# gam0022/hanamaru-renderer

Hardware: AMD Instinct MI355X
Metric: Mpaths/sec at 1920x1080x1024spp (rtcamp6 scene); achieved GB/s in BVH traversal (higher is better)
Workload: dtype f32

## Files before the change

### hanamaru-renderer_amd/csrc/device_scene.h

```cpp
#pragma once
#include <math.h>
#include <stdint.h>

#if defined(__HIPCC__)
#define HD __host__ __device__ __forceinline__
#else
#define HD inline
#endif

namespace hr {

struct alignas(16) f4 { float x, y, z, w; };

struct alignas(16) Node {
    float nearx, neary, farx, fary;
    float nearz, farz;
    uint32_t a;
    uint32_t b;
};
HD void node_set_box(Node &n, const float *mn, const float *mx, int octant) {
    n.nearx = (octant & 1) ? mx[0] : mn[0]; n.farx = (octant & 1) ? mn[0] : mx[0];
    n.neary = (octant & 2) ? mx[1] : mn[1]; n.fary = (octant & 2) ? mn[1] : mx[1];
    n.nearz = (octant & 4) ? mx[2] : mn[2]; n.farz = (octant & 4) ? mn[2] : mx[2];
}
static const uint32_t NODE_END = 0x7fffffffu;
static const uint32_t LEAF_FLAG = 0x80000000u;
static const uint32_t LEAF_FIRST_BITS = 24u, LEAF_MAX_COUNT = 15u;
static const uint32_t MAX_PRIMS_PER_TYPE = 1u << LEAF_FIRST_BITS;
HD bool node_word_is_leaf(uint32_t a) { return a >= LEAF_FLAG; }
HD uint32_t leaf_word(uint32_t type, uint32_t count, uint32_t first) { return LEAF_FLAG | (type << 28) | (count << LEAF_FIRST_BITS) | first; }
HD uint32_t leaf_type(uint32_t w) { return (w >> 28) & 3u; }
HD uint32_t leaf_count(uint32_t w) { return (w >> LEAF_FIRST_BITS) & LEAF_MAX_COUNT; }
HD uint32_t leaf_first(uint32_t w) { return w & (MAX_PRIMS_PER_TYPE - 1u); }

struct alignas(16) QNode {
    uint32_t xy_near;
    uint32_t xy_far;
    uint32_t z_nf;
    uint32_t link;
};
HD uint32_t qnode_offset(int octant, uint32_t records_per_copy, uint32_t index) { return ((uint32_t)octant * records_per_copy + index) * 16u; }
HD uint32_t qnode_link(int octant, uint32_t records_per_copy, uint32_t successor_index) {
    return successor_index == NODE_END ? NODE_END : qnode_offset(octant, records_per_copy, successor_index);
}
HD void qframe_from_box(const float *root_mn, const float *root_mx, float *qmin, float *qstep) {
    for (int a = 0; a < 3; a++) {
        double ext = (double)root_mx[a] - (double)root_mn[a];
        if (!(ext > 1e-6)) ext = 1e-6;
        double gmin = (double)root_mn[a] - 1e-6 * ext;
        float fmin_ = (float)gmin;
        fmin_ -= (fmin_ < 0 ? -fmin_ : fmin_) * 1e-6f + 1e-30f;
        qmin[a] = fmin_;
        qstep[a] = (float)(ext * (1.0 + 4e-6) / 65532.0) * (1.0f + 1e-6f);
    }
}
HD uint32_t q_low(float v, float qmin, float qstep) {
    double q = floor(((double)v - (double)qmin) / (double)qstep - 0.05);
    return (uint32_t)(q < 0.0 ? 0.0 : (q > 65535.0 ? 65535.0 : q));
}
HD uint32_t q_high(float v, float qmin, float qstep) {
    double q = ceil(((double)v - (double)qmin) / (double)qstep + 0.05);
    return (uint32_t)(q < 0.0 ? 0.0 : (q > 65535.0 ? 65535.0 : q));
}
HD QNode qnode_make(const float *mn, const float *mx, int octant, const float *qmin, const float *qstep, uint32_t link) {
    uint32_t nearq[3], farq[3];
    for (int a = 0; a < 3; a++) {
        uint32_t lo = q_low(mn[a], qmin[a], qstep[a]), hi = q_high(mx[a], qmin[a], qstep[a]);
        nearq[a] = ((octant >> a) & 1) ? hi : lo;
        farq[a] = ((octant >> a) & 1) ? lo : hi;
    }
    QNode q;
    q.xy_near = nearq[0] | (nearq[1] << 16);
    q.xy_far = farq[0] | (farq[1] << 16);
    q.z_nf = nearq[2] | (farq[2] << 16);
    q.link = link;
    return q;
}
HD QNode qnode_sentinel(int octant) {
    QNode q;
    uint32_t nearq[3], farq[3];
    for (int a = 0; a < 3; a++) { nearq[a] = ((octant >> a) & 1) ? 0u : 65535u; farq[a] = ((octant >> a) & 1) ? 65535u : 0u; }
    q.xy_near = nearq[0] | (nearq[1] << 16);
    q.xy_far = farq[0] | (farq[1] << 16);
    q.z_nf = nearq[2] | (farq[2] << 16);
    q.link = NODE_END;
    return q;
}


struct alignas(16) Tri {
    float v0[3]; float e1x;
    float e1y, e1z, e2x, e2y;
    float e2z; int32_t element; uint32_t face; float pad1;
};

struct alignas(16) TriT {
    float n[3]; float ax;
    float ay, az, bx, by;
    float bz; float v0[3];
};
struct alignas(16) TriS { float n[3]; int32_t element; };
struct alignas(16) TriX { double n[3], v0[3]; };
HD void tri_derive(const Tri &t, TriT &tt, TriS &ts) {
    const double e1[3] = {t.e1x, t.e1y, t.e1z}, e2[3] = {t.e2x, t.e2y, t.e2z};
    const double n[3] = {e1[1] * e2[2] - e1[2] * e2[1], e1[2] * e2[0] - e1[0] * e2[2], e1[0] * e2[1] - e1[1] * e2[0]};
    const double nn = n[0] * n[0] + n[1] * n[1] + n[2] * n[2];
    const double inn = nn > 0.0 ? 1.0 / nn : 0.0, il = nn > 0.0 ? 1.0 / sqrt(nn) : 0.0;
    const double a[3] = {(e2[1] * n[2] - e2[2] * n[1]) * inn, (e2[2] * n[0] - e2[0] * n[2]) * inn, (e2[0] * n[1] - e2[1] * n[0]) * inn};
    const double b[3] = {(n[1] * e1[2] - n[2] * e1[1]) * inn, (n[2] * e1[0] - n[0] * e1[2]) * inn, (n[0] * e1[1] - n[1] * e1[0]) * inn};
    for (int k = 0; k < 3; k++) { tt.n[k] = (float)(n[k] * il); tt.v0[k] = t.v0[k]; ts.n[k] = (float)(n[k] * il); }
    tt.ax = (float)a[0]; tt.ay = (float)a[1]; tt.az = (float)a[2];
    tt.bx = (float)b[0]; tt.by = (float)b[1]; tt.bz = (float)b[2];
    ts.element = t.element;
}

struct alignas(16) Material {
    int32_t surface; float param; int32_t albedo_img, emission_img;
    float albedo[3]; int32_t roughness_img;
    float emission[3]; float roughness;
    int32_t nee_albedo_zero; int32_t pad[3];
};

struct ImageRef { uint32_t offset, width, height, pad; };

struct Emitter { float c[3]; float r; int32_t element; int32_t pad[3]; };

struct CameraF {
    float eye[3], right[3], up[3], forward[3], phr[3], phu[3];
    float lens_radius, focus_distance;
    int32_t lens_shape;
};

struct CameraD {
    double eye[3], right[3], up[3], forward[3], phr[3], phu[3];
    double lens_radius, focus_distance;
};

struct Scene {
    const QNode *qnodes;
    float qmin[3], qstep[3];
    const Node *nodes;
    const TriT *tris; const TriS *tri_shade;
    const uint32_t *tri_face;
    const f4 *spheres; const int32_t *sphere_elem;
    const f4 *sphere_lo;
    const f4 *cuboids;
    const f4 *cuboid_lo;
    const TriX *tri_exact;
    const Material *materials;
    const uint32_t *texels;
    const ImageRef *images;
    const Emitter *emitters;
    uint32_t num_nodes, num_tris, num_spheres, num_cuboids, num_elements, num_emitters;
    int32_t sky_image[6];
    float sky_intensity[3];
    const uint32_t *sky_quads;
    uint32_t sky_w, sky_h;
    CameraF cam;
    const CameraD *camd;
};

struct GovDev {
    unsigned long long t0[2][2], t1[2][2];
    unsigned long long prev_t0, prev_t1;
    uint32_t lvl[2][2];
    int32_t level;
    int32_t fixed;
    float known[5];
    uint32_t decisions, moves;
    uint32_t budget;
    uint32_t bud[2];
    uint32_t budget_lo, budget_hi, budget_step;
    uint32_t budget_moves;
    float thr_down, thr_up;
};
HD uint32_t gov_trace_mask(int32_t level) { return level >= 4 ? 0x1fu : level == 3 ? 0xfu : 0u; }
HD uint32_t gov_budget_next(uint32_t B, float ratio, uint32_t lo, uint32_t hi, uint32_t step, float down = 0.88f, float up = 0.97f) {
    if (!step) return B;
    if (ratio > up && B) return B + step > hi ? 0u : B + step;
    if (ratio < down) return !B ? hi : (B >= lo + step ? B - step : B);
    return B;
}
HD uint32_t gov_producer_prio(int32_t level, uint32_t init_prio) { return level <= 0 ? (init_prio | init_prio << 2) : level == 1 ? init_prio : 0u; }

struct RenderParams {
    uint32_t width, height;
    uint32_t tiles_x, tiles_y;
    uint32_t sampling_begin, stride, num_k;
    uint32_t adv_den;
    uint32_t leaf_den;
    uint32_t pad[3];
    uint32_t trace_boost;
    uint32_t node_unroll;
    uint32_t kchunk;
    uint32_t ovf_cap;
    uint32_t rr_start;
    uint32_t gov_slot;
    uint32_t nee_cull_off;
    uint32_t tail_div;
    uint32_t wg_budget;
    GovDev *gov;
    uint64_t rec_lo_off;
    uint32_t org_x, org_y, reg_w, reg_h;
    const uint32_t *tile_list;
    uint32_t tile_count;
};
HD uint32_t rp_reg_w(const RenderParams &rp) { return rp.reg_w ? rp.reg_w : rp.width; }
HD uint32_t rp_reg_h(const RenderParams &rp) { return rp.reg_h ? rp.reg_h : rp.height; }
HD bool rp_in_region(const RenderParams &rp, uint32_t px, uint32_t py) { return px < rp_reg_w(rp) && py < rp_reg_h(rp); }

HD void tile_lane_pixel(const RenderParams &rp, uint32_t tile, uint32_t j, uint32_t &px, uint32_t &py, uint32_t &sub) {
    uint32_t tx = tile % rp.tiles_x, ty = tile / rp.tiles_x;
    uint32_t pix = j >> 2;
    sub = j & 3u;
    px = tx * 4u + (pix & 3u);
    py = ty * 4u + (pix >> 2);
}
HD void tile_lane_frame_pixel(const RenderParams &rp, uint32_t tile, uint32_t j, uint32_t &px, uint32_t &py, uint32_t &sub) {
    tile_lane_pixel(rp, tile, j, px, py, sub);
    px += rp.org_x;
    py += rp.org_y;
}

static const int ISAAC_TAIL = 64;
static const int REC_FLOATS = 32;
static const int REC_DRAWS = 28;
static const int REC_HEAD = 28;
static const int LENS_FAST = 5;
static const int DRAWS_PER_PATH = 20;
static const uint32_t REC_ITEM_FLOATS = 64u * REC_FLOATS;
static const int SEG_B1 = 11, SEG_B2 = 21, SEG_NBLK = 11;
static const int SEGP_NBLK = 8, SEGP_PNBLK = 12, SEGP_PRE = 4, SEGP_XCOLS = 32, SEGP_AHEAD_END = 24;
HD bool segp_wants(uint32_t col, int block) {
    return block == 0 || block == 24 || (col < (uint32_t)SEGP_XCOLS ? block == 12 : block == 8 || block == 16);
}
HD uint32_t segp_slot(uint32_t col, int block) {
    if (col < (uint32_t)SEGP_XCOLS) return block == 0 ? col : block == 12 ? 32u + col : 64u + col;
    return 96u + (uint32_t)(block >> 3) * 8u + (col - (uint32_t)SEGP_XCOLS);
}
HD void segp_run(uint32_t slot, uint32_t &col, uint32_t &first, uint32_t &nblk) {
    if (slot < 64u) { col = slot & 31u; first = (slot >> 5) * (uint32_t)SEGP_PNBLK; nblk = (uint32_t)SEGP_PNBLK; }
    else if (slot < 96u) { col = slot - 64u; first = 24u; nblk = (uint32_t)SEGP_NBLK; }
    else { col = (uint32_t)SEGP_XCOLS + ((slot - 96u) & 7u); first = ((slot - 96u) >> 3) * (uint32_t)SEGP_NBLK; nblk = (uint32_t)SEGP_NBLK; }
}
HD uint32_t rec_slot(uint32_t lane_base, uint32_t slot) { return lane_base + (slot >> 2) * 256u + (slot & 3u); }

struct Counters {
    unsigned long long paths, rays, node_tests, tri_tests, sphere_tests, cuboid_tests, rng_overflow, shadow_culled;
    unsigned long long shade_calls, shade_lanes, box_passes, box_lanes, leaf_calls, leaf_lanes, outer_iters, pad2;
    unsigned long long phase_cycles[4];
    unsigned long long seed_phase[8];
};

}
```

### hanamaru-renderer_amd/csrc/hr_api.hip

```cpp
#include <hip/hip_runtime.h>

#include <cmath>
#include <cstdarg>
#include <cstdio>
#include <cstring>
#include <map>
#include <atomic>
#include <mutex>
#include <string>
#include <vector>

#include "bvh_build.h"
#include "device_scene.h"
#include "flatten.h"
#include "gpu_bvh.h"
#include "hanamaru_hip.h"
#include "hanamaru_hip_debug.h"
#include "hr_comm.h"
#include "isaac_core.h"
#include "post_core.h"
#include "pt_core.h"

using namespace hr;


static thread_local std::string g_err;
static int fail(int code, const char *fmt, ...) {
    char buf[1024];
    va_list ap;
    va_start(ap, fmt);
    vsnprintf(buf, sizeof buf, fmt, ap);
    va_end(ap);
    g_err = buf;
    return code;
}
#define HIP_TRY(expr)                                                                                         \
    do {                                                                                                      \
        hipError_t e_ = (expr);                                                                               \
        if (e_ != hipSuccess) return fail(HR_ERR_DEVICE, "%s failed: %s (%s:%d)", #expr, hipGetErrorString(e_), __FILE__, __LINE__); \
    } while (0)
#define HIP_TRY_AS(who, expr)                                                                                 \
    do {                                                                                                      \
        hipError_t e_ = (expr);                                                                               \
        if (e_ != hipSuccess) return fail(HR_ERR_DEVICE, "%s: %s", who, hipGetErrorString(e_));               \
    } while (0)
template <class T>
static int free_device(T *&p) {
    if (p) { HIP_TRY(hipFree(p)); p = nullptr; }
    return HR_OK;
}
struct CallScratch {
    std::vector<void *> blocks;
    CallScratch() = default;
    CallScratch(const CallScratch &) = delete;
    CallScratch &operator=(const CallScratch &) = delete;
    ~CallScratch() { for (void *q : blocks) (void)hipFree(q); }
    hipError_t alloc(void **out, size_t bytes) {
        const hipError_t e = hipMalloc(out, bytes);
        if (e == hipSuccess) blocks.push_back(*out);
        return e;
    }
};

#include "seed_kernels.h"
#include "trace_kernel.h"
#include "wf_kernels.h"
#include "post_kernels.h"
#include "kernel_variants.h"


struct EventPair { hipEvent_t a, b; };

enum : uint32_t { SRC_ACCUM = 1, SRC_MOMENTS = 2, SRC_COUNTS = 4, SRC_BUCKETS = 8, SRC_GUIDES = 16, SRC_SCENE = 32, SRC_TARGET = 64, SRC_NEW_D = 128 };
enum ImageId { GUIDE_IMAGE, D_IMAGE, R_IMAGE, RESTORED_IMAGE, SELECTED_IMAGE, N_IMAGES };

struct hr_ctx {
    int device = 0;
    int num_cus = 256;
    hipStream_t stream = nullptr, own_stream = nullptr, seed_stream = nullptr;
    std::vector<void *> scene_allocs;
    Scene dsc{};
    bool have_scene = false;
    uint64_t st_nodes = 0, st_tris = 0, st_spheres = 0, st_cuboids = 0;
    uint32_t num_images = 0;
    uint32_t W = 0, H = 0;
    uint32_t RX = 0, RY = 0, RW = 0, RH = 0;
    float *accum_own = nullptr, *accum = nullptr;
    float *post_tmp = nullptr;
    uint8_t *d_rgb8 = nullptr;
    bool moments_on = false;
    double *moments = nullptr, *noise_img = nullptr;
    uint64_t moments_n = 0;
    bool counts_on = false;
    uint32_t *counts = nullptr;
    float *guides = nullptr, *denoised = nullptr;
    uint32_t made_of[N_IMAGES] = {};
    uint32_t guide_bounces = 0;
    bool robust_on = false;
    uint32_t robust_k = 0;
    bool bucket_by_sampling = false;
    double *buckets = nullptr;
    uint64_t buckets_n = 0;
    float *robust = nullptr;
    uint8_t *robust_trim = nullptr;
    float *restored = nullptr;
    float *selected = nullptr;
    uint8_t *selected_levels = nullptr;
    double *robust_noise_img = nullptr;
    uint8_t *robust_noise_trim = nullptr;
    bool mask_on = false;
    std::vector<uint8_t> mask;
    uint32_t mask_active = 0;
    uint64_t mask_pixels = 0;
    uint32_t *d_tile_list = nullptr, *d_tile_flags = nullptr;
    uint32_t *d_select_out = nullptr;
    void *select_tmp = nullptr;
    size_t select_tmp_bytes = 0;
    hrcomm::Comm comm = nullptr;
    int comm_world = 0, comm_rank = 0;
    int comm_path = HR_COMM_NONE;
    uint64_t comm_group = 0;
    uint64_t allreduces = 0;
    std::vector<hr_ctx *> same_device_peers;
    float *accum_total = nullptr;
    bool total_valid = false;
    float *recs[2] = {nullptr, nullptr};
    uint32_t *ovf = nullptr;
    uint32_t ovf_cap = 0;
    u64 *ovf_win = nullptr;
    size_t draws_cap = 0;
    uint64_t rec_lo_off = 0;
    int draw_residuals = 1;
    u64 *ring = nullptr;
    int seed_split = 16;
    uint32_t init_prio = 1;
    hipEvent_t seed_done[2] = {nullptr, nullptr}, trace_done[2] = {nullptr, nullptr};
    bool seed_pending[2] = {false, false}, trace_pending[2] = {false, false};
    uint64_t batch_counter = 0;
    Counters *d_counters = nullptr;
    uint32_t *d_tile_counter = nullptr;
    bool counters = false;
    uint32_t batch = 0;
    uint32_t adv_den = 2, leaf_den = 2;
    int min_waves = 5;
    uint32_t trace_wgs = 6;
    uint32_t tail_div = 16;
    uint32_t trace_grid = 0, trace_budget = 0;
    uint32_t node_unroll = 2;
    uint32_t kchunk = 0;
    int trace_boost = -1;
    GovDev *gov = nullptr;
    bool quant_nodes = true;
    int max_leaf = 4;
    double split_ratio = -1.0;
    int bvh_builder = -1;
    int builder_in_use = 0;
    double bvh_build_ms = 0;
    uint64_t max_tail_bytes = 20ull << 30;
    int seed_mode = 2;
    int seed_prof = 0;
    int seed_prerun = 1;
    uint32_t seed_prio = 3;
    uint32_t nee_cull = 7;
    uint32_t rr_start = 0;
    uint32_t ploc_top = hr::lbvh::PLOC_TOP_CLUSTERS;
    int trace_mode = 0;
    int trace_mode_opt = -1;
    int precise_opt = -1;
    bool precise = false;
    bool wf_has_prec = false;
    WfQueues wf{};
    void *wf_block = nullptr;
    uint32_t wf_adv_den = 2, wf_trav_wgs = 8, wf_shade_wgs = 8;
    int debug_skip = 0;
    std::vector<EventPair> seed_events, trace_events, post_events, debug_events;
    double seed_ms = 0, trace_ms = 0, post_ms = 0, debug_ms = 0;
    uint64_t seed_launches = 0, trace_launches = 0, debug_launches = 0;
    uint64_t paths_rendered = 0;
    std::vector<std::pair<uint64_t, hipEvent_t>> markers;
    uint64_t next_ticket = 1;
};

static std::mutex g_bound_mu;
static std::map<const void *, std::pair<const hr_ctx *, size_t>> g_bound;
static void unbind_accumulator(hr_ctx *c) {
    std::lock_guard<std::mutex> lk(g_bound_mu);
    for (auto it = g_bound.begin(); it != g_bound.end();) it = it->second.first == c ? g_bound.erase(it) : std::next(it);
}
static void free_scene(hr_ctx *c) {
    for (void *p : c->scene_allocs) (void)hipFree(p);
    c->scene_allocs.clear();
    c->have_scene = false;
}
template <class T>
static int upload(hr_ctx *c, const std::vector<T> &v, const T **out) {
    void *d = nullptr;
    size_t bytes = std::max<size_t>(v.size() * sizeof(T), 16);
    HIP_TRY(hipMalloc(&d, bytes));
    c->scene_allocs.push_back(d);
    if (!v.empty()) HIP_TRY(hipMemcpy(d, v.data(), v.size() * sizeof(T), hipMemcpyHostToDevice));
    *out = reinterpret_cast<const T *>(d);
    return HR_OK;
}
static const int GOV_LEVELS = 5;
__global__ void governor_kernel(GovDev *g, uint32_t slot) {
    typedef unsigned long long u64t;
    const uint32_t other = slot ^ 1u;
    const u64t none = ~0ull;
    const u64t s0 = g->t0[0][slot], s1 = g->t1[0][slot], r0 = g->t0[1][slot], r1 = g->t1[1][slot];
    const bool have = s0 != none && s1 > s0 && r0 != none && r1 > r0;
    if (have && g->fixed < 0) {
        const u64t p0 = g->prev_t0, p1 = g->prev_t1;
        const u64t n0 = __hip_atomic_load(&g->t0[0][other], __ATOMIC_RELAXED, __HIP_MEMORY_SCOPE_AGENT), n1 = __hip_atomic_load(&g->t1[0][other], __ATOMIC_RELAXED, __HIP_MEMORY_SCOPE_AGENT);
        float ov_seed = 0.0f, ov_trace = 0.0f;
        if (p1 > p0) {
            const u64t lo = p0 > s0 ? p0 : s0, hi = p1 < s1 ? p1 : s1;
            if (hi > lo) ov_seed = (float)(hi - lo) / (float)(s1 - s0);
        }
        if (n0 != none && n0 < r1) {
            const u64t lo = n0 > r0 ? n0 : r0, hi = (n1 > n0 && n1 < r1) ? n1 : r1;
            if (hi > lo) ov_trace = (float)(hi - lo) / (float)(r1 - r0);
        }
        const int L = (int)g->lvl[0][slot];
        const float seed_t = (float)(s1 - s0), trace_t = (float)(r1 - r0), m = seed_t > trace_t ? seed_t : trace_t;
        const bool beside = ov_trace > 0.7f || trace_t > 1.25f * seed_t;
        const uint32_t B = g->bud[slot] ? g->bud[slot] - 1u : ~0u;
        const bool spare = trace_t < 0.7f * seed_t && ov_trace > 0.7f;
        if ((ov_seed > 0.7f || spare) && beside && L == (int)g->lvl[1][slot] && L >= 0 && L < GOV_LEVELS) {
            g->decisions++;
            bool budget_moved = false;
            if (L == 0 && g->level == 0 && B == g->budget && g->budget_step) {
                const uint32_t nb = gov_budget_next(B, trace_t / seed_t, g->budget_lo, g->budget_hi, g->budget_step, g->thr_down, g->thr_up);
                if (nb != B) {
                    budget_moved = true;
                    g->budget_moves++;
                    __hip_atomic_store(&g->budget, nb, __ATOMIC_RELAXED, __HIP_MEMORY_SCOPE_AGENT);
                    for (int k = 0; k < GOV_LEVELS; k++) g->known[k] = 0;
                }
            }
            if (!budget_moved && B == 0 && g->budget == 0) {
                g->known[L] = g->known[L] > 0 ? 0.5f * (g->known[L] + m) : m;
                if (L == g->level) {
                    int next = L;
                    if (trace_t > 1.015f * seed_t && L < GOV_LEVELS - 1 && g->known[L + 1] == 0) next = L + 1;
                    else if (seed_t > 1.015f * trace_t && L > 0 && g->known[L - 1] == 0) next = L - 1;
                    else
                        for (int k = 0; k < GOV_LEVELS; k++)
                            if (g->known[k] > 0 && g->known[k] < 0.995f * g->known[next]) next = k;
                    if (next != L) { g->moves++; __hip_atomic_store(&g->level, next, __ATOMIC_RELAXED, __HIP_MEMORY_SCOPE_AGENT); }
                }
            }
        }
    }
    if (r0 != none && r1 > r0) { g->prev_t0 = r0; g->prev_t1 = r1; }
    for (int k = 0; k < 2; k++) { g->t0[k][slot] = none; g->t1[k][slot] = 0; }
    g->bud[slot] = 0;
    if (g->fixed >= 0) __hip_atomic_store(&g->level, g->fixed, __ATOMIC_RELAXED, __HIP_MEMORY_SCOPE_AGENT);
}
static void resolve_modes(hr_ctx *c) {
    const bool has_scene = c->have_scene;
    const uint32_t tris = has_scene ? c->dsc.num_tris : 0u;
    c->precise = c->precise_opt == 1 || (c->precise_opt < 0 && has_scene && tris == 0u && !c->rr_start);
    c->trace_mode = c->trace_mode_opt >= 0 ? c->trace_mode_opt : (c->precise && tris > 0u ? 1 : 0);
}
static int govern_reset(hr_ctx *c) {
    resolve_modes(c);
    if (!c->gov) return HR_OK;
    GovDev h;
    memset(&h, 0, sizeof h);
    for (int k = 0; k < 2; k++)
        for (int sl = 0; sl < 2; sl++) h.t0[k][sl] = ~0ull;
    h.fixed = c->trace_boost;
    h.level = c->trace_boost >= 0 ? c->trace_boost : 0;
    if (c->trace_boost < 0) { h.budget_step = (uint32_t)c->num_cus / 4u; h.budget_lo = (uint32_t)c->num_cus * 5u / 2u; h.budget_hi = (uint32_t)c->num_cus * 7u / 2u; }
    h.thr_down = 0.88f; h.thr_up = 0.97f;
    if (c->trace_mode == 1 && !c->rr_start && c->trace_boost < 0) {
        h.budget_step = (uint32_t)c->num_cus / 2u; h.budget_lo = (uint32_t)c->num_cus * 3u; h.budget_hi = (uint32_t)c->num_cus * 7u;
        h.thr_down = 0.96f; h.thr_up = 1.02f;
    }
    HIP_TRY(hipMemcpy(c->gov, &h, sizeof h, hipMemcpyHostToDevice));
    return HR_OK;
}
static void changed(hr_ctx *c, uint32_t sources) {
    if (sources & SRC_ACCUM) {
        c->total_valid = false;
        for (hr_ctx *p : c->same_device_peers) p->total_valid = false;
    }
    for (uint32_t &made_of : c->made_of) if (made_of & sources) made_of = 0;
}
static int drain_events(hr_ctx *c) {
    auto sum = [](std::vector<EventPair> &ev, double &acc) -> hipError_t {
        hipError_t first = hipSuccess;
        for (auto &e : ev) {
            float ms = 0;
            hipError_t r = hipEventElapsedTime(&ms, e.a, e.b);
            if (r == hipSuccess) acc += ms;
            else if (first == hipSuccess) first = r;
            (void)hipEventDestroy(e.a);
            (void)hipEventDestroy(e.b);
        }
        ev.clear();
        return first;
    };
    HIP_TRY(sum(c->seed_events, c->seed_ms));
    HIP_TRY(sum(c->trace_events, c->trace_ms));
    HIP_TRY(sum(c->post_events, c->post_ms));
    HIP_TRY(sum(c->debug_events, c->debug_ms));
    return HR_OK;
}
static void retire_finished_launches(hr_ctx *c) {
    size_t n = 0;
    const size_t limit = std::min(c->seed_events.size(), c->trace_events.size());
    while (n < limit && hipEventQuery(c->seed_events[n].b) == hipSuccess && hipEventQuery(c->trace_events[n].b) == hipSuccess) n++;
    if (n > 2) n -= 2; else return;
    for (size_t i = 0; i < n; i++) {
        float sm = 0, tm = 0;
        if (hipEventElapsedTime(&sm, c->seed_events[i].a, c->seed_events[i].b) == hipSuccess) c->seed_ms += sm;
        if (hipEventElapsedTime(&tm, c->trace_events[i].a, c->trace_events[i].b) == hipSuccess) c->trace_ms += tm;
        (void)hipEventDestroy(c->seed_events[i].a); (void)hipEventDestroy(c->seed_events[i].b);
        (void)hipEventDestroy(c->trace_events[i].a); (void)hipEventDestroy(c->trace_events[i].b);
    }
    c->seed_events.erase(c->seed_events.begin(), c->seed_events.begin() + (long)n);
    c->trace_events.erase(c->trace_events.begin(), c->trace_events.begin() + (long)n);
}
static int sync_all(hr_ctx *c) {
    HIP_TRY(hipStreamSynchronize(c->seed_stream));
    HIP_TRY(hipStreamSynchronize(c->stream));
    c->trace_pending[0] = c->trace_pending[1] = false;
    c->seed_pending[0] = c->seed_pending[1] = false;
    for (auto &m : c->markers) (void)hipEventDestroy(m.second);
    c->markers.clear();
    return drain_events(c);
}
static void drop_pair(EventPair &ev) {
    if (ev.a) (void)hipEventDestroy(ev.a);
    if (ev.b) (void)hipEventDestroy(ev.b);
    ev = EventPair{nullptr, nullptr};
}
static hipError_t timed_begin(EventPair &ev, hipStream_t st) {
    ev = EventPair{nullptr, nullptr};
    hipError_t e = hipEventCreate(&ev.a);
    if (e == hipSuccess) e = hipEventCreate(&ev.b);
    if (e == hipSuccess) e = hipEventRecord(ev.a, st);
    if (e != hipSuccess) drop_pair(ev);
    return e;
}
static hipError_t timed_end(hipError_t launched, EventPair &ev, hipStream_t st, std::vector<EventPair> &list, uint64_t *launches = nullptr) {
    hipError_t e = launched;
    if (e == hipSuccess && ev.a) e = hipEventRecord(ev.b, st);
    if (e != hipSuccess || !ev.a) { drop_pair(ev); return e; }
    list.push_back(ev);
    if (launches) ++*launches;
    return hipSuccess;
}
struct CallEvents : EventPair {
    CallEvents() : EventPair{nullptr, nullptr} {}
    CallEvents(const CallEvents &) = delete;
    CallEvents &operator=(const CallEvents &) = delete;
    ~CallEvents() { drop_pair(*this); }
};

static void reset_same_device_peers(hr_ctx *c) {
    for (hr_ctx *p : c->same_device_peers) if (p != c) { p->same_device_peers.clear(); p->comm_world = 0; p->total_valid = false; p->comm_path = HR_COMM_NONE; p->allreduces = 0; }
}
static int free_mask_buffers(hr_ctx *c) {
    c->select_tmp_bytes = 0;
    for (uint32_t **p : {&c->d_tile_list, &c->d_tile_flags, &c->d_select_out}) { int rc = free_device(*p); if (rc) return rc; }
    return free_device(c->select_tmp);
}

enum PlaneLife { WITH_TARGET, WITH_OPTION, ON_FIRST_USE };
struct Plane {
    void **(*slot)(hr_ctx *);
    size_t elem;
    uint32_t comps;
    PlaneLife life;
    bool at_alloc, at_clear;
    const char *option = nullptr;
    bool hr_ctx::*on = nullptr;
    uint64_t hr_ctx::*n = nullptr;
    uint32_t hr_ctx::*per = nullptr;
};
#define PLANE_SLOT(member) [](hr_ctx *c) -> void ** { return (void **)&c->member; }
static const Plane ACCUM_OWN{PLANE_SLOT(accum_own), sizeof(float), 3, WITH_TARGET, true, true};
static const Plane POST_TMP{PLANE_SLOT(post_tmp), sizeof(float), 3, WITH_TARGET, false, false};
static const Plane RGB8{PLANE_SLOT(d_rgb8), sizeof(uint8_t), 3, WITH_TARGET, false, false};
static const Plane ACCUM_TOTAL{PLANE_SLOT(accum_total), sizeof(float), 3, ON_FIRST_USE, false, false};
static const Plane MOMENTS{PLANE_SLOT(moments), sizeof(double), 6, WITH_OPTION, true, true, "moments", &hr_ctx::moments_on, &hr_ctx::moments_n};
static const Plane NOISE_IMG{PLANE_SLOT(noise_img), sizeof(double), 1, ON_FIRST_USE, false, false};
static const Plane COUNTS{PLANE_SLOT(counts), sizeof(uint32_t), 1, WITH_OPTION, true, true, "sample_counts", &hr_ctx::counts_on};
static const Plane GUIDES{PLANE_SLOT(guides), sizeof(float), 8, ON_FIRST_USE, false, false};
static const Plane DENOISED{PLANE_SLOT(denoised), sizeof(float), 3, ON_FIRST_USE, false, false};
static const Plane BUCKETS{PLANE_SLOT(buckets), sizeof(double), 3, WITH_OPTION, true, true, "robust_buckets", &hr_ctx::robust_on, &hr_ctx::buckets_n, &hr_ctx::robust_k};
static const Plane ROBUST{PLANE_SLOT(robust), sizeof(float), 3, ON_FIRST_USE, false, false};
static const Plane ROBUST_TRIM{PLANE_SLOT(robust_trim), sizeof(uint8_t), 1, ON_FIRST_USE, false, false};
static const Plane ROBUST_NOISE_IMG{PLANE_SLOT(robust_noise_img), sizeof(double), 1, ON_FIRST_USE, false, false};
static const Plane ROBUST_NOISE_TRIM{PLANE_SLOT(robust_noise_trim), sizeof(uint8_t), 1, ON_FIRST_USE, false, false};
static const Plane RESTORED{PLANE_SLOT(restored), sizeof(float), 3, ON_FIRST_USE, false, false};
static const Plane SELECTED{PLANE_SLOT(selected), sizeof(float), 3, ON_FIRST_USE, false, false};
static const Plane SELECTED_LEVELS{PLANE_SLOT(selected_levels), sizeof(uint8_t), 1, ON_FIRST_USE, false, false};
#undef PLANE_SLOT
static const Plane *const PLANES[] = {&ACCUM_OWN, &POST_TMP, &RGB8, &ACCUM_TOTAL, &MOMENTS, &NOISE_IMG, &COUNTS, &GUIDES, &DENOISED, &BUCKETS, &ROBUST, &ROBUST_TRIM, &ROBUST_NOISE_IMG, &ROBUST_NOISE_TRIM, &RESTORED, &SELECTED, &SELECTED_LEVELS};

static size_t region_pixels(const hr_ctx *c) { return (size_t)c->RW * c->RH; }
static size_t plane_elems(const hr_ctx *c, const Plane &p) { return region_pixels(c) * p.comps * (p.per ? c->*p.per : 1u); }
static size_t plane_bytes(const hr_ctx *c, const Plane &p) { return plane_elems(c, p) * p.elem; }
static int plane_free(hr_ctx *c, const Plane &p) {
    if (p.n) c->*p.n = 0;
    return free_device(*p.slot(c));
}
static int plane_zero(hr_ctx *c, const Plane &p, hipStream_t st = nullptr, void *dev = nullptr) {
    if (!dev && !(dev = *p.slot(c))) return HR_OK;
    HIP_TRY(hipMemsetAsync(dev, 0, plane_bytes(c, p), st));
    if (!st) HIP_TRY(hipStreamSynchronize(nullptr));
    if (p.n) c->*p.n = 0;
    return HR_OK;
}
static int plane_alloc(hr_ctx *c, const Plane &p) {
    int rc = plane_free(c, p);
    if (rc) return rc;
    HIP_TRY(hipMalloc(p.slot(c), plane_bytes(c, p)));
    return p.at_alloc ? plane_zero(c, p) : HR_OK;
}
static int plane_read(hr_ctx *c, const Plane &p, const void *dev, void *host) {
    int rc = hr_synchronize(c);
    if (rc) return rc;
    HIP_TRY(hipMemcpy(host, dev, plane_bytes(c, p), hipMemcpyDeviceToHost));
    return HR_OK;
}
static int plane_write(hr_ctx *c, const Plane &p, void *dev, const void *host) {
    HIP_TRY(hipSetDevice(c->device));
    int rc = sync_all(c);
    if (rc) return rc;
    changed(c, dev == c->guides ? SRC_GUIDES : (dev == c->accum ? SRC_ACCUM : 0u) | SRC_MOMENTS | SRC_COUNTS | SRC_BUCKETS);
    HIP_TRY(hipMemcpy(dev, host, plane_bytes(c, p), hipMemcpyHostToDevice));
    return HR_OK;
}
static int plane_ready(hr_ctx *c, const Plane &p, const char *who) {
    if (!c) return fail(HR_ERR_INVALID, "%s: null ctx", who);
    if (!(c->*p.on) || !*p.slot(c)) return fail(HR_ERR_INVALID, "%s: option %s is off", who, p.option);
    return HR_OK;
}
static int option_plane_read(hr_ctx *c, const Plane &p, const char *who, void *host) {
    int rc = plane_ready(c, p, who);
    if (!rc && !host) rc = fail(HR_ERR_INVALID, "%s: null argument", who);
    return rc ? rc : plane_read(c, p, *p.slot(c), host);
}
static int option_plane_write(hr_ctx *c, const Plane &p, const char *who, const void *host) {
    int rc = plane_ready(c, p, who);
    if (!rc && !host) rc = fail(HR_ERR_INVALID, "%s: null argument", who);
    return rc ? rc : plane_write(c, p, *p.slot(c), host);
}

struct Image {
    const Plane *plane, *second;
    uint32_t stale_with;
    const Plane *option;
    const char *none;
};
static const Image IMAGES[N_IMAGES] = {
    {&GUIDES, nullptr, SRC_GUIDES | SRC_SCENE | SRC_TARGET, nullptr, "no guide planes (hr_render_guides or hr_write_guides first)"},
    {&DENOISED, nullptr, SRC_ACCUM | SRC_COUNTS | SRC_GUIDES | SRC_SCENE | SRC_TARGET | SRC_NEW_D, nullptr, "no denoised image (hr_denoise first; anything that changes its inputs invalidates it)"},
    {&ROBUST, &ROBUST_TRIM, SRC_COUNTS | SRC_BUCKETS | SRC_TARGET, &BUCKETS, "no robust image (hr_robust first; anything that changes its inputs invalidates it)"},
    {&RESTORED, nullptr, SRC_ACCUM | SRC_COUNTS | SRC_BUCKETS | SRC_GUIDES | SRC_SCENE | SRC_TARGET, nullptr, "no restored image (hr_robust_restore first; anything that changes its inputs invalidates it)"},
    {&SELECTED, &SELECTED_LEVELS, SRC_ACCUM | SRC_MOMENTS | SRC_COUNTS | SRC_BUCKETS | SRC_GUIDES | SRC_SCENE | SRC_TARGET, &BUCKETS,
     "no selected image (hr_denoise_select first; anything that changes its inputs invalidates it)"},
};
static bool image_valid(const hr_ctx *c, ImageId id) { return c->made_of[id] != 0; }
static void image_made(hr_ctx *c, ImageId id, uint32_t decided = 0) { c->made_of[id] = IMAGES[id].stale_with | decided; }
static int image_ready(hr_ctx *c, ImageId id, const char *who, const void *host) {
    const Image &im = IMAGES[id];
    int rc;
    if (im.option && (rc = plane_ready(c, *im.option, who))) return rc;
    if (!c || !host) return fail(HR_ERR_INVALID, "%s: null argument", who);
    if (!*im.plane->slot(c) || (im.second && !*im.second->slot(c)) || !image_valid(c, id)) return fail(HR_ERR_INVALID, "%s: %s", who, im.none);
    return HR_OK;
}
static int image_read(hr_ctx *c, ImageId id, const char *who, void *host, bool second = false) {
    const Plane &p = second ? *IMAGES[id].second : *IMAGES[id].plane;
    int rc = image_ready(c, id, who, host);
    return rc ? rc : plane_read(c, p, *p.slot(c), host);
}
static int guides_or_render(hr_ctx *c) { return image_valid(c, GUIDE_IMAGE) ? HR_OK : hr_render_guides(c); }
static int no_instantiation(const char *who, const char *kernel, uint32_t K) {
    return fail(HR_ERR_UNSUPPORTED, "%s: no %s instantiation for %u buckets (kernel_variants.h)", who, kernel, K);
// ... 375 lines not shown

int hr_bind_accumulator(hr_ctx *c, float *device_rgb) {
    if (!c) return fail(HR_ERR_INVALID, "hr_bind_accumulator: null ctx");
    if (!c->W) return fail(HR_ERR_NO_TARGET, "hr_bind_accumulator: hr_set_resolution not called");
    HIP_TRY(hipSetDevice(c->device));
    const size_t bytes = plane_bytes(c, ACCUM_OWN);
    if (device_rgb) {
        hipPointerAttribute_t at;
        if (hipPointerGetAttributes(&at, device_rgb) != hipSuccess || at.type != hipMemoryTypeDevice) {
            (void)hipGetLastError();
            return fail(HR_ERR_INVALID, "hr_bind_accumulator: %p is not device memory", (void *)device_rgb);
        }
        if (at.device != c->device) return fail(HR_ERR_INVALID, "hr_bind_accumulator: the buffer lives on device %d, the context on device %d", at.device, c->device);
        if ((uintptr_t)device_rgb % sizeof(float)) return fail(HR_ERR_INVALID, "hr_bind_accumulator: the buffer is not aligned for floats");
        void *base = nullptr;
        size_t size = 0;
        if (hipMemGetAddressRange((hipDeviceptr_t *)&base, &size, (hipDeviceptr_t)device_rgb) == hipSuccess) {
            if ((const char *)device_rgb + bytes > (const char *)base + size)
                return fail(HR_ERR_INVALID, "hr_bind_accumulator: the buffer is too small (%zu bytes from this address to the end of its allocation, %u x %u x 3 floats = %zu needed)",
                            (size_t)((const char *)base + size - (const char *)device_rgb), c->RW, c->RH, bytes);
        } else (void)hipGetLastError();
    }
    int rc = sync_all(c);
    if (rc) return rc;
    {
        std::lock_guard<std::mutex> lk(g_bound_mu);
        if (device_rgb)
            for (const auto &kv : g_bound) {
                const char *a = (const char *)kv.first, *b = (const char *)device_rgb;
                if (kv.second.first != c && a < b + bytes && b < a + kv.second.second)
                    return fail(HR_ERR_INVALID, "hr_bind_accumulator: this buffer is already bound to another context (one context per accumulator: the launch's radiance is added with plain loads and stores)");
            }
        for (auto it = g_bound.begin(); it != g_bound.end();) it = it->second.first == c ? g_bound.erase(it) : std::next(it);
        if (device_rgb) g_bound[device_rgb] = std::make_pair((const hr_ctx *)c, bytes);
    }
    c->accum = device_rgb ? device_rgb : c->accum_own;
    changed(c, SRC_ACCUM | SRC_MOMENTS | SRC_COUNTS | SRC_BUCKETS);
    return HR_OK;
}
void *hr_accumulator_device_ptr(hr_ctx *c) { return c ? c->accum : nullptr; }

int hr_set_stream(hr_ctx *c, void *s) {
    if (!c) return fail(HR_ERR_INVALID, "hr_set_stream: null ctx");
    HIP_TRY(hipSetDevice(c->device));
    int rc = sync_all(c);
    if (rc) return rc;
    c->stream = s ? (hipStream_t)s : c->own_stream;
    return HR_OK;
}

int hr_clear(hr_ctx *c) {
    if (!c) return fail(HR_ERR_INVALID, "hr_clear: null ctx");
    if (!c->accum) return fail(HR_ERR_NO_TARGET, "hr_clear: no accumulator (call hr_set_resolution)");
    HIP_TRY(hipSetDevice(c->device));
    int rc = sync_all(c);
    if (rc) return rc;
    changed(c, SRC_ACCUM | SRC_MOMENTS | SRC_COUNTS | SRC_BUCKETS);
    for (const Plane *p : PLANES)
        if (p->at_clear && (rc = plane_zero(c, *p, c->stream, p == &ACCUM_OWN ? c->accum : nullptr))) return rc;
    HIP_TRY(hipMemsetAsync(c->d_counters, 0, sizeof(Counters), c->stream));
    HIP_TRY(hipStreamSynchronize(c->stream));
    c->seed_ms = c->trace_ms = c->post_ms = c->debug_ms = 0;
    c->seed_launches = c->trace_launches = c->debug_launches = 0;
    c->paths_rendered = 0;
    return HR_OK;
}

static bool draws_twin(const hr_ctx *c) { return c->precise && c->seed_mode == 2 && c->draw_residuals; }
static uint64_t rec_lo_off(const hr_ctx *c) { return draws_twin(c) ? c->rec_lo_off : 0; }
static int ensure_draws(hr_ctx *c, size_t items) {
    const bool twin = draws_twin(c);
    if (items <= c->draws_cap && (!twin || c->rec_lo_off)) return HR_OK;
    int rc = sync_all(c);
    if (rc) return rc;
    items = std::max(items, c->draws_cap);
    c->draws_cap = 0;
    c->rec_lo_off = 0;
    const size_t floats = (items + SEED_SPARE_ITEMS) * REC_ITEM_FLOATS;
    for (int i = 0; i < 2; i++) {
        if (c->recs[i]) { HIP_TRY(hipFree(c->recs[i])); c->recs[i] = nullptr; }
        HIP_TRY(hipMalloc((void **)&c->recs[i], floats * (twin ? 2 : 1) * sizeof(float)));
    }
    c->draws_cap = items;
    c->rec_lo_off = twin ? floats : 0;
    return HR_OK;
}

static int ensure_ovf(hr_ctx *c, uint64_t paths_per_launch) {
    const uint64_t groups = (paths_per_launch + SEED_COLS - 1) / SEED_COLS;
    const uint64_t waves = 2 * std::min<uint64_t>(std::max<uint64_t>(groups, 1), (uint64_t)c->num_cus);
    const double expected = 4.7e-4 * (double)paths_per_launch / (double)waves;
    const uint64_t want = std::max<uint64_t>(SEED_OVF_MIN, ((uint64_t)(8.0 * expected) + 64 + 255) / 256 * 256);
    if (want <= c->ovf_cap) return HR_OK;
    int rc = sync_all(c);
    if (rc) return rc;
    if (c->ovf) { HIP_TRY(hipFree(c->ovf)); c->ovf = nullptr; }
    c->ovf_cap = 0;
    HIP_TRY(hipMalloc((void **)&c->ovf, (size_t)c->num_cus * 2 * want * sizeof(uint32_t)));
    c->ovf_cap = (uint32_t)want;
    return HR_OK;
}

static int ensure_wf(hr_ctx *c, uint64_t paths) {
    const uint64_t sub_paths = ((paths / 64u + WF_SUBQ - 1u) / WF_SUBQ) * 64u, sub_rays = sub_paths * (1ull + c->dsc.num_emitters);
    if (sub_paths <= c->wf.cap_paths && sub_rays <= c->wf.cap_rays && c->wf_block && (c->wf_has_prec || !c->precise)) return HR_OK;
    if (sub_rays * WF_SUBQ >= 0xffffffffull) return fail(HR_ERR_UNSUPPORTED, "split pipeline: %llu ray slots per launch exceed the 32-bit queue index (reduce option batch)", (unsigned long long)(sub_rays * WF_SUBQ));
    int rc = sync_all(c);
    if (rc) return rc;
    if (c->wf_block) { HIP_TRY(hipFree(c->wf_block)); c->wf_block = nullptr; }
    c->wf.cap_paths = c->wf.cap_rays = 0;
    const uint64_t rays = sub_rays * WF_SUBQ, pths = sub_paths * WF_SUBQ;
    const size_t ray_q = (size_t)rays * sizeof(f4), st_q = (size_t)pths * sizeof(f4), cnt = (WF_STEPS + 2) * WF_SUBQ * sizeof(WfCounts);
    const size_t total = cnt + 4 * ray_q + (size_t)rays * sizeof(WfHitRec) + (c->precise ? 10 : 6) * st_q;
    hipError_t e = hipMalloc(&c->wf_block, total);
    if (e != hipSuccess) { c->wf_block = nullptr; return fail(HR_ERR_DEVICE, "split pipeline: %.1f GiB of queues: %s", (double)total / (1ull << 30), hipGetErrorString(e)); }
    char *b = (char *)c->wf_block;
    c->wf.counts = (WfCounts *)b; b += cnt;
    for (int i = 0; i < 2; i++) { c->wf.ray_a[i] = (f4 *)b; b += ray_q; c->wf.ray_b[i] = (f4 *)b; b += ray_q; }
    c->wf.hits = (WfHitRec *)b; b += (size_t)rays * sizeof(WfHitRec);
    for (int i = 0; i < 2; i++) { c->wf.st_a[i] = (f4 *)b; b += st_q; c->wf.st_b[i] = (f4 *)b; b += st_q; c->wf.st_c[i] = (f4 *)b; b += st_q; }
    for (int i = 0; i < 2; i++) { c->wf.st_d[i] = c->wf.st_e[i] = c->wf.st_f[i] = nullptr; c->wf.tag[i] = nullptr; }
    if (c->precise) for (int i = 0; i < 2; i++) { c->wf.st_d[i] = (f4 *)b; b += st_q; c->wf.st_e[i] = (f4 *)b; b += st_q; }
    c->wf_has_prec = c->precise;
    c->wf.cap_paths = (uint32_t)sub_paths; c->wf.cap_rays = (uint32_t)sub_rays;
    return HR_OK;
}
static int launch_split(hr_ctx *c, const RenderParams &rp, int slot, std::vector<hipEvent_t> *marks = nullptr, uint32_t *plog = nullptr, const WfQueues *queues = nullptr) {
    const WfQueues wq = queues ? *queues : c->wf;
    hipStream_t st = c->stream;
    auto mark = [&]() -> hipError_t { if (!marks) return hipSuccess; hipEvent_t e; hipError_t r = hipEventCreate(&e); if (r != hipSuccess) return r; marks->push_back(e); return hipEventRecord(e, st); };
    const bool log = plog != nullptr;
    const WfStartFn start = select_wf_start_kernel(c->precise, rp.tile_list != nullptr);
    const WfTraverseFn traverse = select_wf_traverse_kernel(c->counters, c->dsc.qnodes != nullptr, log);
    const WfShadeFn shade = select_wf_shade_kernel(c->counters, c->precise, log);
    if (!start || !traverse || !shade) return fail(HR_ERR_UNSUPPORTED, "split pipeline: no kernel instantiation for these options (kernel_variants.h)");
    HIP_TRY(hipMemsetAsync(wq.counts, 0, (WF_STEPS + 2) * WF_SUBQ * sizeof(WfCounts), st));
    HIP_TRY(mark());
    auto grid_of = [&](uint32_t wgs_per_cu) { return dim3(std::max<uint32_t>(16u, (uint32_t)c->num_cus * wgs_per_cu / 16u * 16u)); };
    hipLaunchKernelGGL(start, grid_of(8u), dim3(256), 0, st, c->dsc, rp, c->recs[slot], wq);
    HIP_TRY(mark());
    RenderParams rt = rp;
    rt.adv_den = c->wf_adv_den;
    const dim3 gt = grid_of(c->wf_trav_wgs), gs = grid_of(c->wf_shade_wgs), b(256);
    for (uint32_t step = 1; step <= WF_STEPS; step++) {
        hipLaunchKernelGGL(traverse, gt, b, 0, st, c->dsc, rt, wq, step, c->d_counters);
        HIP_TRY(mark());
        hipLaunchKernelGGL(shade, gs, b, 0, st, c->dsc, rp, c->recs[slot], wq, step, c->d_counters, plog);
        HIP_TRY(mark());
    }
    HIP_TRY(hipGetLastError());
    return HR_OK;
}

static int launch_seed(hr_ctx *c, const RenderParams &rp, int slot, hipStream_t st) {
    const bool list = rp.tile_list != nullptr;
    uint64_t paths = (uint64_t)(list ? rp.tile_count : rp.tiles_x * rp.tiles_y) * rp.num_k * 64u;
    uint32_t grid = (uint32_t)std::min<uint64_t>((paths + SEED_COLS - 1) / SEED_COLS, (uint64_t)c->num_cus);
    const SeedVariant *v = select_seed_kernel(c->seed_mode, c->seed_split, c->seed_prof, rp.rec_lo_off != 0, list, c->seed_prerun != 0);
    if (!v) return fail(HR_ERR_UNSUPPORTED, "no seed kernel instantiation for seed_mode %d, seed_split %d, seed_prof %d%s (kernel_variants.h)", c->seed_mode, c->seed_split, c->seed_prof, list ? " under a tile mask" : "");
    const bool skip = (c->debug_skip & 2) != 0;
    if (!skip && v->ring && !c->ring) HIP_TRY(hipMalloc((void **)&c->ring, (size_t)c->num_cus * SEED_RING_WORDS_MAX * sizeof(u64)));
    EventPair ev;
    HIP_TRY(timed_begin(ev, st));
    hipError_t e = hipSuccess;
    if (!skip) {
        RenderParams krp = rp;
        int lens_shape = c->dsc.cam.lens_shape;
        void *args[7] = {&krp, &lens_shape, &c->ring, &c->recs[slot], &c->ovf, &c->ovf_win, &c->d_counters};
        if (!v->ring) std::copy(args + 3, args + 7, args + 2);
        e = hipLaunchKernel(v->fn, dim3(grid), dim3(v->threads), args, SEED_LDS_BYTES, st);
    }
    HIP_TRY(timed_end(e, ev, st, c->seed_events, &c->seed_launches));
    return HR_OK;
}

static void target_params(const hr_ctx *c, RenderParams &rp) {
    rp.width = c->W; rp.height = c->H;
    rp.org_x = c->RX; rp.org_y = c->RY; rp.reg_w = c->RW; rp.reg_h = c->RH;
    rp.tiles_x = (c->RW + 3) / 4; rp.tiles_y = (c->RH + 3) / 4;
}
static void knob_params(const hr_ctx *c, RenderParams &rp) {
    rp.adv_den = c->adv_den; rp.leaf_den = c->leaf_den;
    rp.node_unroll = c->node_unroll; rp.kchunk = c->kchunk;
    rp.nee_cull_off = ~c->nee_cull & 7u;
}
static uint32_t render_batch(const hr_ctx *c, uint32_t tiles, bool split) {
    uint64_t batch = c->batch;
    if (!batch) {
        const uint64_t per_sampling_paths = (uint64_t)tiles * 64u;
        batch = std::min<uint64_t>(64, std::max<uint64_t>(4, (33177600ull + per_sampling_paths - 1) / per_sampling_paths));
    }
    const uint64_t per_sampling = (uint64_t)tiles * REC_ITEM_FLOATS * sizeof(float) * (draws_twin(c) ? 2 : 1);
    batch = std::min(batch, std::max<uint64_t>(1, c->max_tail_bytes / std::max<uint64_t>(1, per_sampling)));
    if (split) {
        const uint64_t per_path = (1ull + c->dsc.num_emitters) * (4 * sizeof(f4) + sizeof(WfHitRec)) + (c->precise ? 10 : 6) * sizeof(f4);
        batch = std::min(batch, std::max<uint64_t>(1, c->max_tail_bytes / std::max<uint64_t>(1, (uint64_t)tiles * 64u * per_path)));
    }
    return (uint32_t)batch;
}
enum TraceSide { TRACE_NONE, TRACE_IN_FORCE, TRACE_SPLIT };
struct LaunchPlan {
    RenderParams rp;
    uint32_t tiles;
    uint32_t batch;
    bool split;
};
static int plan_launch(hr_ctx *c, uint32_t begin, uint32_t stride, uint32_t batch, TraceSide side, LaunchPlan &p) {
    p = LaunchPlan{};
    RenderParams &rp = p.rp;
    target_params(c, rp);
    knob_params(c, rp);
    rp.sampling_begin = begin; rp.stride = stride; rp.num_k = batch;
    rp.pad[0] = c->seed_prio;
    p.tiles = rp.tiles_x * rp.tiles_y;
    if (c->mask_on) { rp.tile_list = c->d_tile_list; rp.tile_count = c->mask_active; p.tiles = c->mask_active; }
    p.split = side == TRACE_SPLIT || (side == TRACE_IN_FORCE && c->trace_mode == 1 && !c->rr_start);
    p.batch = batch ? batch : render_batch(c, p.tiles, p.split);
    int rc = ensure_draws(c, (size_t)p.tiles * p.batch);
    if (rc) return rc;
    rp.rec_lo_off = rec_lo_off(c);
    if ((rc = ensure_ovf(c, (uint64_t)p.tiles * 64u * p.batch))) return rc;
    if (p.split && (rc = ensure_wf(c, (uint64_t)p.tiles * 64u * p.batch))) return rc;
    rp.ovf_cap = c->ovf_cap;
    return HR_OK;
}
static uint32_t trace_grid_size(const hr_ctx *c, uint32_t tiles, uint32_t nk, uint32_t fixed_grid) {
    const uint32_t kch = c->kchunk ? c->kchunk : TRACE_KCHUNK;
    const uint64_t units = (uint64_t)tiles * ((nk + kch - 1) / kch);
    return (uint32_t)std::min<uint64_t>(fixed_grid ? fixed_grid : (uint64_t)c->num_cus * c->trace_wgs, (units + TRACE_WAVES - 1) / TRACE_WAVES);
}

int hr_render(hr_ctx *c, uint32_t s_begin, uint32_t s_end, uint32_t stride) {
    if (!c || !stride) return fail(HR_ERR_INVALID, "hr_render: bad argument");
    if (!c->have_scene) return fail(HR_ERR_NO_SCENE, "hr_render: no scene uploaded");
    if (!c->accum || !c->W) return fail(HR_ERR_NO_TARGET, "hr_render: hr_set_resolution not called");
    if (s_end <= s_begin) return HR_OK;
    HIP_TRY(hipSetDevice(c->device));
    changed(c, SRC_ACCUM | SRC_MOMENTS | SRC_COUNTS | SRC_BUCKETS);
    if (c->precise_opt == 1 && c->rr_start) return fail(HR_ERR_UNSUPPORTED, "hr_render: russian_roulette and precise_shading exclude each other (the roulette estimator has no f64 instantiation)");
    const uint32_t total_k = (s_end - s_begin + stride - 1) / stride;
    const bool list = c->mask_on;
    if (list) {
        const char *what = c->counters ? "option counters" : c->rr_start ? "option russian_roulette" : c->min_waves != 5 ? "debug option min_waves" :
                           c->seed_mode != 2 ? "a seed_mode other than 2" : c->seed_prof ? "debug option seed_prof" : nullptr;
        if (what) return fail(HR_ERR_UNSUPPORTED, "hr_render: %s has no kernel form for a tile mask (hr_set_tile_mask(NULL) removes the mask)", what);
        if (!c->mask_active) {
            if (c->moments) c->moments_n += total_k;
            if (c->buckets) c->buckets_n += total_k;
            return HR_OK;
        }
    }
    LaunchPlan plan;
    int rc = plan_launch(c, s_begin, stride, 0, TRACE_IN_FORCE, plan);
    if (rc) return rc;
    RenderParams &rp = plan.rp;
    const uint32_t tiles = plan.tiles, batch = plan.batch;
    rp.rr_start = c->rr_start;
    rp.tail_div = c->tail_div;
    rp.pad[2] = (uint32_t)c->debug_skip;
    rp.wg_budget = c->trace_budget;
    const TraceFn trace = select_trace_kernel(c->counters, c->dsc.qnodes != nullptr, c->rr_start != 0, c->precise, c->min_waves, false, list);
    if (!trace) return fail(HR_ERR_UNSUPPORTED, "hr_render: no trace kernel instantiation for these options%s (kernel_variants.h)", list ? " under a tile mask" : "");
    const AccumulateFn accumulate = select_accumulate_kernel(c->moments != nullptr, c->counts != nullptr, list);
    if (!accumulate) return fail(HR_ERR_UNSUPPORTED, "hr_render: no accumulate kernel instantiation for these options (kernel_variants.h)");
    const BucketFn bucket = c->buckets ? select_bucket_kernel(c->counts != nullptr, list, c->bucket_by_sampling) : nullptr;
    if (c->buckets && !bucket) return fail(HR_ERR_UNSUPPORTED, "hr_render: no bucket kernel instantiation for these options (kernel_variants.h)");
    for (uint32_t done = 0; done < total_k; done += batch) {
        uint32_t nk = std::min(batch, total_k - done);
        rp.sampling_begin = s_begin + done * stride;
        rp.num_k = nk;
        int slot = (int)(c->batch_counter & 1);
        c->batch_counter++;
        rp.gov = c->gov; rp.gov_slot = (uint32_t)slot;
        rp.trace_boost = 0;
        rp.pad[1] = c->init_prio;
        hipStream_t sstream = c->seed_stream;
        if (c->trace_pending[slot]) HIP_TRY(hipStreamWaitEvent(sstream, c->trace_done[slot], 0));
        if ((rc = launch_seed(c, rp, slot, sstream))) return rc;
        HIP_TRY(hipEventRecord(c->seed_done[slot], sstream));
        c->seed_pending[slot] = true;
        HIP_TRY(hipStreamWaitEvent(c->stream, c->seed_done[slot], 0));
        EventPair ev;
        HIP_TRY(timed_begin(ev, c->stream));
        HIP_TRY(hipMemsetAsync(c->d_tile_counter + slot, 0, sizeof(uint32_t), c->stream));
        if (c->debug_skip & 16) {
        } else if (plan.split) {
            if ((rc = launch_split(c, rp, slot))) return rc;
        } else
            hipLaunchKernelGGL(trace, dim3(trace_grid_size(c, tiles, nk, c->trace_grid)), dim3(64 * TRACE_WAVES), 0, c->stream, c->dsc, rp, c->recs[slot], c->d_counters,
                               c->d_tile_counter + slot, (uint32_t *)nullptr);
        HIP_TRY(timed_end(hipGetLastError(), ev, c->stream, c->trace_events, &c->trace_launches));
        if (!(c->debug_skip & 16)) {
            if (bucket) {
                const unsigned long long start = c->bucket_by_sampling ? ((unsigned long long)rp.sampling_begin + c->robust_k - 1u) % c->robust_k : (unsigned long long)c->buckets_n;
                hipLaunchKernelGGL(bucket, dim3((tiles + 3) / 4), dim3(256), 0, c->stream, rp, c->recs[slot], c->buckets, c->counts, c->robust_k, start);
                HIP_TRY(hipGetLastError());
                c->buckets_n += nk;
            }
            hipLaunchKernelGGL(accumulate, dim3((tiles + 3) / 4), dim3(256), 0, c->stream, rp, c->recs[slot], c->accum, c->moments, c->counts);
            HIP_TRY(hipGetLastError());
            if (c->moments) c->moments_n += nk;
        }
        hipLaunchKernelGGL(governor_kernel, dim3(1), dim3(1), 0, c->stream, c->gov, (uint32_t)slot);
        HIP_TRY(hipGetLastError());
        HIP_TRY(hipEventRecord(c->trace_done[slot], c->stream));
        c->trace_pending[slot] = true;
        c->paths_rendered += (list ? c->mask_pixels : (uint64_t)region_pixels(c)) * 4 * nk;
        if (c->trace_events.size() >= 64 && c->seed_events.size() == c->trace_events.size()) retire_finished_launches(c);
        if (c->trace_events.size() > 4096) {
            if ((rc = sync_all(c))) return rc;
        }
    }
    return HR_OK;
}

template <class Fn, class... Args>
static int launch_tile_pass(hr_ctx *c, Fn fn, Args... args) {
    RenderParams rp{};
    target_params(c, rp);
    knob_params(c, rp);
    const uint32_t tiles = rp.tiles_x * rp.tiles_y;
    EventPair ev;
    HIP_TRY(timed_begin(ev, c->stream));
    hipLaunchKernelGGL(fn, dim3((tiles + TRACE_WAVES - 1) / TRACE_WAVES), dim3(64 * TRACE_WAVES), 0, c->stream, c->dsc, rp, args...);
    HIP_TRY(timed_end(hipGetLastError(), ev, c->stream, c->debug_events, &c->debug_launches));
    return HR_OK;
}

int hr_render_debug(hr_ctx *c, int mode) {
    if (!c || mode < 0 || mode > 3) return fail(HR_ERR_INVALID, "hr_render_debug: mode must be 0..3");
    int rc;
    if ((rc = debug_refusal(c, "hr_render_debug", A_SCENE)) || (rc = debug_refusal(c, "hr_render_debug", A_TARGET))) return rc;
    if (c->moments_on) return fail(HR_ERR_UNSUPPORTED, "hr_render_debug: not with option moments on (a debug sampling goes into the accumulator without per-sampling values)");
    if ((rc = debug_refusal(c, "hr_render_debug", NO_MASK))) return rc;
    if (c->counts_on) return fail(HR_ERR_UNSUPPORTED, "hr_render_debug: not with option sample_counts on (a debug sampling goes into the accumulator without being counted)");
    if (c->robust_on) return fail(HR_ERR_UNSUPPORTED, "hr_render_debug: not with option robust_buckets on (a debug sampling goes into the accumulator without per-sampling values)");
    HIP_TRY(hipSetDevice(c->device));
    changed(c, SRC_ACCUM);
    const DebugRenderFn fn = select_debug_render_kernel(c->counters, c->dsc.qnodes != nullptr);
    if (!fn) return fail(HR_ERR_UNSUPPORTED, "hr_render_debug: no kernel instantiation for these options (kernel_variants.h)");
    return launch_tile_pass(c, fn, mode, c->accum, c->d_counters);
}

int hr_synchronize(hr_ctx *c) {
    if (!c) return fail(HR_ERR_INVALID, "hr_synchronize: null ctx");
    HIP_TRY(hipSetDevice(c->device));
    int rc = sync_all(c);
    if (rc) return rc;
    Counters h;
    HIP_TRY(hipMemcpy(&h, c->d_counters, sizeof h, hipMemcpyDeviceToHost));
    if (h.rng_overflow) return fail(HR_ERR_RNG_WINDOW, "%llu paths needed more than %d ISAAC-64 outputs for the lens rejection loop (or the fix-up queue overflowed)", h.rng_overflow, ISAAC_TAIL);
    return HR_OK;
}

int hr_mark(hr_ctx *c, uint64_t *ticket) {
    if (!c || !ticket) return fail(HR_ERR_INVALID, "hr_mark: null argument");
    HIP_TRY(hipSetDevice(c->device));
    hipEvent_t ev = nullptr;
    HIP_TRY(hipEventCreateWithFlags(&ev, hipEventDisableTiming));
    hipError_t e = hipEventRecord(ev, c->stream);
    if (e != hipSuccess) { (void)hipEventDestroy(ev); return fail(HR_ERR_DEVICE, "hr_mark: %s", hipGetErrorString(e)); }
    *ticket = c->next_ticket++;
    c->markers.emplace_back(*ticket, ev);
    return HR_OK;
}
int hr_wait(hr_ctx *c, uint64_t ticket) {
    if (!c) return fail(HR_ERR_INVALID, "hr_wait: null ctx");
    HIP_TRY(hipSetDevice(c->device));
    size_t n = 0;
    while (n < c->markers.size() && c->markers[n].first <= ticket) n++;
    if (!n) return HR_OK;
    hipError_t e = hipEventSynchronize(c->markers[n - 1].second);
    for (size_t i = 0; i < n; i++) (void)hipEventDestroy(c->markers[i].second);
    c->markers.erase(c->markers.begin(), c->markers.begin() + (long)n);
    if (e != hipSuccess) return fail(HR_ERR_DEVICE, "hr_wait: %s", hipGetErrorString(e));
    return HR_OK;
}

int hr_read_accumulator(hr_ctx *c, float *host) {
    if (!c || !host) return fail(HR_ERR_INVALID, "hr_read_accumulator: null argument");
    if (!c->accum) return fail(HR_ERR_NO_TARGET, "hr_read_accumulator: no accumulator");
    return plane_read(c, ACCUM_OWN, c->total_valid ? c->accum_total : c->accum, host);
}
int hr_write_accumulator(hr_ctx *c, const float *host) {
    if (!c || !host) return fail(HR_ERR_INVALID, "hr_write_accumulator: null argument");
    if (!c->accum) return fail(HR_ERR_NO_TARGET, "hr_write_accumulator: no accumulator");
    return plane_write(c, ACCUM_OWN, c->accum, host);
}

#define NCCL_TRY(expr)                                                                                                    \
    do {                                                                                                                  \
        int r_ = (expr);                                                                                                  \
        if (r_ != 0) return fail(HR_ERR_DEVICE, "%s failed: %s", #expr, hrcomm::api().GetErrorString ? hrcomm::api().GetErrorString(r_) : "?"); \
    } while (0)

int hr_comm_get_unique_id(void *id_out) {
    if (!id_out) return fail(HR_ERR_INVALID, "hr_comm_get_unique_id: null argument");
    if (!hrcomm::load()) return fail(HR_ERR_UNSUPPORTED, "%s", hrcomm::api().error.c_str());
    hrcomm::UniqueId id;
    NCCL_TRY(hrcomm::api().GetUniqueId(&id));
    memcpy(id_out, &id, sizeof id);
    return HR_OK;
}
// ... 1017 lines not shown
};
static const OptionRow DEBUG_OPTIONS[] = {
    {"adv_den", &hr_ctx::adv_den, 1, 64, 0, "adv_den must be in [1,64]", 0},
    {"leaf_den", &hr_ctx::leaf_den, 1, 64, 0, "leaf_den must be in [1,64]", 0},
    {"min_waves", &hr_ctx::min_waves, 4, 6, 0, "min_waves must be in [4,6]", 0},
    {"kchunk", &hr_ctx::kchunk, 0, 64, 0, "kchunk must be in [1,64], or 0 for the default", 0},
    {"node_unroll", &hr_ctx::node_unroll, 1, 2, 1, "node_unroll must be 1 or 2", 0},
    {"tail_div", &hr_ctx::tail_div, 0, 2147483648.0, 0, "tail_div must be in [0,2^31] (0 = no finer tail)", 0},
    {"trace_grid", &hr_ctx::trace_grid, 0, 2147483648.0, 0, "trace_grid must be in [0,2^31] (0 = trace_wgs per CU)", 0},
    {"trace_budget", &hr_ctx::trace_budget, 0, 2147483648.0, 0, "trace_budget must be in [0,2^31] (0 = every workgroup stays)", 0},
    {"trace_wgs", &hr_ctx::trace_wgs, 1, 8, 0, "trace_wgs must be in [1,8]", 0},
    {"seed_prio", &hr_ctx::seed_prio, 0, 3, 0, "seed_prio must be in [0,3]", 0},
    {"init_prio", &hr_ctx::init_prio, 0, 3, 0, "init_prio must be in [0,3]", 0},
    {"seed_split", &hr_ctx::seed_split, 8, 28, 4, "seed_split must be 8, 12, 16, 20, 24 or 28", 0},
    {"seed_prof", &hr_ctx::seed_prof, 1, 0, 0, "", 0},
    {"seed_prerun", &hr_ctx::seed_prerun, 0, 1, 1, "seed_prerun must be 1 (pre-run window of the three-run seed kernel) or 0 (its three equal runs)", OPT_SYNC},
    {"ploc_top", &hr_ctx::ploc_top, 1, 1 << 16, 0, "ploc_top must be in [1,65536]", 0},
    {"trace_mode", &hr_ctx::trace_mode_opt, -1, 1, 1, "trace_mode must be -1 (automatic), 0 (megakernel) or 1 (split: traversal kernel + shading kernel)", OPT_SYNC | OPT_GOVERN},
    {"draw_residuals", &hr_ctx::draw_residuals, 0, 1, 1, "draw_residuals must be 0 or 1", 0},
    {"wf_adv_den", &hr_ctx::wf_adv_den, 0, 64, 0, "wf_adv_den must be in [0,64]", 0},
    {"wf_trav_wgs", &hr_ctx::wf_trav_wgs, 1, 16, 0, "wf_trav_wgs must be in [1,16]", 0},
    {"wf_shade_wgs", &hr_ctx::wf_shade_wgs, 1, 16, 0, "wf_shade_wgs must be in [1,16]", 0},
    {"debug_skip", &hr_ctx::debug_skip, 1, 0, 0, "", 0},
};
static int apply_option(hr_ctx *c, const OptionRow &r, double value) {
    if (r.lo <= r.hi) {
        bool ok = value >= r.lo && value <= r.hi;
        if (ok && r.step > 0) ok = std::fmod(value - r.lo, r.step) == 0.0;
        if (!ok) return fail(HR_ERR_INVALID, "%s", r.error);
    }
    if (r.flags & OPT_SYNC) { int rc = sync_all(c); if (rc) return rc; }
    if (r.field.b) c->*r.field.b = value != 0.0;
    else if (r.field.u) c->*r.field.u = (uint32_t)value;
    else c->*r.field.i = (int)value;
    return r.flags & OPT_GOVERN ? govern_reset(c) : HR_OK;
}

static int set_plane_option(hr_ctx *c, double value, const Plane &p, const Plane &other, int (*off_first)(hr_ctx *)) {
    if (value != 0 && value != 1) return fail(HR_ERR_INVALID, "%s must be 0 or 1", p.option);
    if (value == 1 && !c->W) return fail(HR_ERR_NO_TARGET, "%s: hr_set_resolution not called", p.option);
    int rc = sync_all(c);
    if (rc) return rc;
    if (value == 0 || !(c->*p.on)) changed(c, SRC_MOMENTS | SRC_COUNTS);
    if (value == 0) {
        c->*p.on = false;
        if ((rc = off_first(c))) return rc;
        return plane_free(c, p);
    }
    if (c->*p.on) return HR_OK;
    if ((rc = plane_alloc(c, p))) { (void)plane_free(c, p); return rc; }
    c->*p.on = true;
    return plane_zero(c, other);
}

static int set_robust_buckets(hr_ctx *c, double value) {
    if (value != 0 && !robust_valid_k(value)) return fail(HR_ERR_INVALID, "robust_buckets must be 0 (off) or an odd number of buckets in [3,15]");
    if (value != 0 && !c->W) return fail(HR_ERR_NO_TARGET, "robust_buckets: hr_set_resolution not called");
    if (c->robust_on && (uint32_t)value == c->robust_k) return HR_OK;
    changed(c, SRC_BUCKETS);
    int rc = sync_all(c);
    if (rc) return rc;
    c->robust_on = false;
    c->robust_k = 0;
    if ((rc = plane_free(c, BUCKETS)) || (rc = plane_free(c, ROBUST)) || (rc = plane_free(c, ROBUST_TRIM)) || (rc = plane_free(c, ROBUST_NOISE_IMG)) || (rc = plane_free(c, ROBUST_NOISE_TRIM)) || (rc = plane_free(c, RESTORED))) return rc;
    if (value == 0) return HR_OK;
    c->robust_k = (uint32_t)value;
    if ((rc = plane_alloc(c, BUCKETS))) { (void)plane_free(c, BUCKETS); c->robust_k = 0; return rc; }
    c->robust_on = true;
    if (c->counts_on) { changed(c, SRC_COUNTS | SRC_MOMENTS); if ((rc = plane_zero(c, COUNTS)) || (rc = plane_zero(c, MOMENTS))) return rc; }
    return HR_OK;
}

static bool set_sharding_option(hr_ctx *c, const std::string &key, double value, int &rc) {
    if (key != "bucket_by_sampling") return false;
    rc = HR_OK;
    if (value != 0 && value != 1) { rc = fail(HR_ERR_INVALID, "bucket_by_sampling must be 0 (a pixel's j-th sampling in bucket j mod K) or 1 (sampling s in bucket (s - 1) mod K)"); return true; }
    if ((value == 1) == c->bucket_by_sampling) return true;
    if ((rc = sync_all(c))) return true;
    c->bucket_by_sampling = value == 1;
    if (!c->robust_on) return true;
    changed(c, SRC_BUCKETS);
    if ((rc = plane_zero(c, BUCKETS))) return true;
    if (c->counts_on) { changed(c, SRC_COUNTS | SRC_MOMENTS); if ((rc = plane_zero(c, COUNTS))) return true; rc = plane_zero(c, MOMENTS); }
    return true;
}

static const char *const RR_EXCLUDES_PRECISE = "russian_roulette and precise_shading 1 exclude each other (the roulette estimator has no f64 instantiation)";
int hr_set_option(hr_ctx *c, const char *key, double value) {
    if (!c || !key) return fail(HR_ERR_INVALID, "hr_set_option: null argument");
    HIP_TRY(hipSetDevice(c->device));
    std::string k = key;
    if (k == "precise_shading" && value == 1 && c->rr_start) return fail(HR_ERR_UNSUPPORTED, "%s", RR_EXCLUDES_PRECISE);
    { int rc; if (set_sharding_option(c, k, value, rc)) return rc; }
    if (const OptionRow *row = find_row(PRODUCT_OPTIONS, [&](const OptionRow &r) { return k == r.key; })) return apply_option(c, *row, value);
    if (k == "moments") {
        const bool was_on = c->moments_on;
        const int rc = set_plane_option(c, value, MOMENTS, COUNTS, [](hr_ctx *x) { return plane_free(x, NOISE_IMG); });
        return !rc && value == 1 && !was_on && c->counts_on ? plane_zero(c, BUCKETS) : rc;
    }
    if (k == "sample_counts") {
        const bool was_on = c->counts_on;
        const int rc = set_plane_option(c, value, COUNTS, MOMENTS, remove_mask);
        return !rc && value == 1 && !was_on ? plane_zero(c, BUCKETS) : rc;
    }
    if (k == "robust_buckets") return set_robust_buckets(c, value);
    if (k == "guide_bounces") {
        if (!(value >= 0 && value <= 8) || value != std::floor(value)) return fail(HR_ERR_INVALID, "guide_bounces must be a whole number in [0,8]");
        if ((uint32_t)value == c->guide_bounces) return HR_OK;
        c->guide_bounces = (uint32_t)value;
        changed(c, SRC_GUIDES);
        return HR_OK;
    }
    if (k == "max_tail_gib") {
        if (value < 1 || value > 128) return fail(HR_ERR_INVALID, "max_tail_gib must be in [1,128]");
        c->max_tail_bytes = (uint64_t)value << 30;
        return HR_OK;
    }
    if (k == "split_ratio") {
        if ((value < 0 && value != -1) || value > 1000) return fail(HR_ERR_INVALID, "split_ratio must be -1 (automatic), 0 (off) or in (0,1000]");
        c->split_ratio = value;
        return HR_OK;
    }
    if (k == "rng_window") {
        if ((int)value != ISAAC_TAIL) return fail(HR_ERR_UNSUPPORTED, "rng_window is fixed at %d in this build", ISAAC_TAIL);
        return HR_OK;
    }
    if (k == "russian_roulette") {
        if (value != 0 && (value < 2 || value > 9)) return fail(HR_ERR_INVALID, "russian_roulette must be 0 (off) or the first iteration that plays, in [2,9]");
        if (value != 0 && c->precise_opt == 1) return fail(HR_ERR_UNSUPPORTED, "%s", RR_EXCLUDES_PRECISE);
        int rc = sync_all(c);
        if (rc) return rc;
        c->rr_start = (uint32_t)value;
        return govern_reset(c);
    }
    return fail(HR_ERR_INVALID, "unknown option '%s' (measurement knobs live behind hr_set_debug_option)", key);
}

int hr_set_debug_option(hr_ctx *c, const char *key, double value) {
    if (!c || !key) return fail(HR_ERR_INVALID, "hr_set_debug_option: null argument");
    HIP_TRY(hipSetDevice(c->device));
    std::string k = key;
    if (const OptionRow *row = find_row(DEBUG_OPTIONS, [&](const OptionRow &r) { return k == r.key; })) return apply_option(c, *row, value);
    if (k == "seed_mode") {
        if (value != 0 && value != 1 && value != 2 && value != 3 && value != 4) return fail(HR_ERR_INVALID, "seed_mode must be 4 (five-wave four-run kernel), 3 (phase-shifted four-run kernel), 2 (three-run kernel), 1 (producer / consumer kernel with a state ring) or 0 (fused kernel)");
#if !defined(HR_EXPERIMENTS)
        if (value >= 3) return fail(HR_ERR_UNSUPPORTED, "seed_mode %d is a measured experiment (slower than the default): build with `make EXPERIMENTS=1` to have it", (int)value);
#endif
        int rc = sync_all(c);
        if (rc) return rc;
        c->seed_mode = (int)value;
        return HR_OK;
    }
    if (k == "nee_cull") { c->nee_cull = (uint32_t)value & 7u; return HR_OK; }
    return fail(HR_ERR_INVALID, "unknown debug option '%s'", key);
}

int hr_debug_draws(hr_ctx *c, uint32_t sampling, uint32_t first_path, uint32_t num_paths, uint32_t window, uint64_t *host_out) {
    if (!c || !host_out || !num_paths) return fail(HR_ERR_INVALID, "hr_debug_draws: bad argument");
    int rc = debug_refusal(c, "hr_debug_draws", NO_REGION | NO_MASK | A_TARGET);
    if (rc) return rc;
    if (window == 0 || window > (uint32_t)ISAAC_TAIL) return fail(HR_ERR_INVALID, "window must be in [1,%d]", ISAAC_TAIL);
    if ((uint64_t)first_path + num_paths > (uint64_t)c->W * c->H * 4) return fail(HR_ERR_INVALID, "path range outside the image");
    HIP_TRY(hipSetDevice(c->device));
    CallScratch scratch;
    u64 *d = nullptr;
    HIP_TRY(scratch.alloc((void **)&d, (size_t)num_paths * window * 8));
    hipLaunchKernelGGL(seed_debug_kernel, dim3((num_paths + 63) / 64), dim3(64), 256 * 64 * 8, c->stream, c->W, c->H, sampling, first_path, num_paths,
                       (int)window, d);
    HIP_TRY_AS("hr_debug_draws", hipGetLastError());
    HIP_TRY_AS("hr_debug_draws", hipStreamSynchronize(c->stream));
    HIP_TRY_AS("hr_debug_draws", hipMemcpy(host_out, d, (size_t)num_paths * window * 8, hipMemcpyDeviceToHost));
    return HR_OK;
}

static int path_draws_out(hr_ctx *c, uint32_t sampling, float *host_out, bool residuals, const char *who) {
    if (!c || !host_out) return fail(HR_ERR_INVALID, "%s: bad argument", who);
    int rc = debug_refusal(c, who, NO_REGION | NO_MASK | A_TARGET);
    if (rc) return rc;
    if (!c->have_scene) return fail(HR_ERR_NO_SCENE, "%s: no scene (lens shape needed)", who);
    if (residuals && !draws_twin(c)) return fail(HR_ERR_UNSUPPORTED, "%s: no residuals are written (needs precise shading in force, seed_mode 2, draw_residuals 1)", who);
    HIP_TRY(hipSetDevice(c->device));
    if ((rc = sync_all(c))) return rc;
    LaunchPlan plan;
    if ((rc = plan_launch(c, sampling, 1, 1, TRACE_NONE, plan))) return rc;
    RenderParams &rp = plan.rp;
    const uint32_t tiles = plan.tiles;
    if (!residuals) rp.rec_lo_off = 0;
    rp.pad[0] = 0;
    if ((rc = launch_seed(c, rp, 0, c->stream))) return rc;
    std::vector<float> h((size_t)tiles * REC_ITEM_FLOATS), lo;
    HIP_TRY(hipStreamSynchronize(c->stream));
    HIP_TRY(hipMemcpy(h.data(), c->recs[0], h.size() * sizeof(float), hipMemcpyDeviceToHost));
    if (residuals) {
        lo.resize(h.size());
        HIP_TRY(hipMemcpy(lo.data(), c->recs[0] + rp.rec_lo_off, lo.size() * sizeof(float), hipMemcpyDeviceToHost));
    }
    for (uint32_t t = 0; t < tiles; t++)
        for (uint32_t j = 0; j < 64; j++) {
            uint32_t tx = t % rp.tiles_x, ty = t / rp.tiles_x, pix = j >> 2, sub = j & 3;
            uint32_t px = tx * 4 + (pix & 3), py = ty * 4 + (pix >> 2);
            if (px >= c->W || py >= c->H) continue;
            const float *rec = &h[(size_t)t * REC_ITEM_FLOATS];
            const uint32_t lb = j * 4u;
            uint32_t a = float_as_uint(rec[rec_slot(lb, REC_HEAD)]);
            float *o = &host_out[(((size_t)py * c->W + px) * 4 + sub) * DRAWS_PER_PATH];
            if (residuals) {
                const float *rl = &lo[(size_t)t * REC_ITEM_FLOATS];
                for (uint32_t d = 0; d < (uint32_t)DRAWS_PER_PATH; d++) o[d] = rl[rec_slot(lb, 2 * a + d)];
                continue;
            }
            o[0] = rec[rec_slot(lb, REC_HEAD + 1)];
            o[1] = rec[rec_slot(lb, REC_HEAD + 2)];
            for (uint32_t d = 2; d < (uint32_t)DRAWS_PER_PATH; d++) o[d] = rec[rec_slot(lb, 2 * a + d)];
        }
    return drain_events(c);
}
int hr_debug_path_draws(hr_ctx *c, uint32_t sampling, float *host_out) { return path_draws_out(c, sampling, host_out, false, "hr_debug_path_draws"); }
int hr_debug_path_draw_residuals(hr_ctx *c, uint32_t sampling, float *host_out) { return path_draws_out(c, sampling, host_out, true, "hr_debug_path_draw_residuals"); }

int hr_debug_path_log(hr_ctx *c, uint32_t sampling, uint32_t *host_out) {
    if (!c || !host_out) return fail(HR_ERR_INVALID, "hr_debug_path_log: bad argument");
    int rc = debug_refusal(c, "hr_debug_path_log", NO_REGION | NO_MASK | A_TARGET | A_SCENE);
    if (rc) return rc;
    HIP_TRY(hipSetDevice(c->device));
    if ((rc = sync_all(c))) return rc;
    LaunchPlan plan;
    if ((rc = plan_launch(c, sampling, 1, 1, TRACE_IN_FORCE, plan))) return rc;
    const RenderParams &rp = plan.rp;
    const bool split = plan.split;
    const TraceFn trace = select_trace_kernel(c->counters, c->dsc.qnodes != nullptr, c->rr_start != 0, c->precise, c->min_waves, true);
    if (!split && !trace) return fail(HR_ERR_UNSUPPORTED, "hr_debug_path_log: no trace kernel instantiation for these options (kernel_variants.h)");
    if ((rc = launch_seed(c, rp, 0, c->stream))) return rc;
    const size_t words = (size_t)c->W * c->H * 4u * 8u;
    CallScratch scratch;
    uint32_t *d_log = nullptr;
    HIP_TRY(scratch.alloc((void **)&d_log, words * sizeof(uint32_t)));
    HIP_TRY_AS("hr_debug_path_log", hipMemsetAsync(d_log, 0, words * sizeof(uint32_t), c->stream));
    if (split) {
        WfQueues wq = c->wf;
        const size_t st_q = (size_t)wq.cap_paths * WF_SUBQ * sizeof(f4), tg_q = (size_t)wq.cap_rays * WF_SUBQ * sizeof(uint32_t);
        char *b = nullptr;
        HIP_TRY_AS("hr_debug_path_log", scratch.alloc((void **)&b, 2 * st_q + 2 * tg_q));
        for (int i = 0; i < 2; i++) { wq.st_f[i] = (f4 *)b; b += st_q; }
        for (int i = 0; i < 2; i++) { wq.tag[i] = (uint32_t *)b; b += tg_q; }
        if ((rc = launch_split(c, rp, 0, nullptr, d_log, &wq))) return rc;
    } else {
        HIP_TRY_AS("hr_debug_path_log", hipMemsetAsync(c->d_tile_counter, 0, sizeof(uint32_t), c->stream));
        hipLaunchKernelGGL(trace, dim3(trace_grid_size(c, plan.tiles, 1, 0)), dim3(64 * TRACE_WAVES), 0, c->stream, c->dsc, rp, c->recs[0], c->d_counters, c->d_tile_counter, d_log);
        HIP_TRY_AS("hr_debug_path_log", hipGetLastError());
    }
    HIP_TRY_AS("hr_debug_path_log", hipStreamSynchronize(c->stream));
    HIP_TRY_AS("hr_debug_path_log", hipMemcpy(host_out, d_log, words * sizeof(uint32_t), hipMemcpyDeviceToHost));
    return drain_events(c);
}

int hr_debug_wf_profile(hr_ctx *c, uint32_t sampling, uint32_t num_k, double *ms_out, uint32_t *counts_out) {
    if (!c || !ms_out || !counts_out || !num_k) return fail(HR_ERR_INVALID, "hr_debug_wf_profile: bad argument");
    int rc = debug_refusal(c, "hr_debug_wf_profile", NO_REGION | NO_MASK | A_TARGET | A_SCENE);
    if (rc) return rc;
    HIP_TRY(hipSetDevice(c->device));
    if ((rc = sync_all(c))) return rc;
    LaunchPlan plan;
    if ((rc = plan_launch(c, sampling, 1, num_k, TRACE_SPLIT, plan))) return rc;
    RenderParams &rp = plan.rp;
    rp.kchunk = 0;
    if ((rc = launch_seed(c, rp, 0, c->stream))) return rc;
    std::vector<hipEvent_t> marks;
    rc = launch_split(c, rp, 0, &marks);
    hipError_t e = hipStreamSynchronize(c->stream);
    if (!rc && e == hipSuccess && marks.size() == 2u + 2u * WF_STEPS) {
        for (size_t i = 0; i + 1 < marks.size(); i++) { float ms = 0; (void)hipEventElapsedTime(&ms, marks[i], marks[i + 1]); ms_out[i] = ms; }
        std::vector<WfCounts> h((WF_STEPS + 2) * WF_SUBQ);
        e = hipMemcpy(h.data(), c->wf.counts, h.size() * sizeof(WfCounts), hipMemcpyDeviceToHost);
        for (uint32_t s = 0; s <= WF_STEPS; s++) {
            counts_out[2 * s] = counts_out[2 * s + 1] = 0;
            for (uint32_t k = 0; k < WF_SUBQ; k++) { counts_out[2 * s] += wf_rays(h[s * WF_SUBQ + k]); counts_out[2 * s + 1] += wf_paths(h[s * WF_SUBQ + k]); }
        }
    }
    for (hipEvent_t ev : marks) (void)hipEventDestroy(ev);
    if (rc) return rc;
    if (e != hipSuccess) return fail(HR_ERR_DEVICE, "hr_debug_wf_profile: %s", hipGetErrorString(e));
    return drain_events(c);
}

int hr_debug_intersect(hr_ctx *c, uint32_t n, const float *rays, float *out, int32_t *out_element) {
    if (!c || !rays || !out || !out_element || !n) return fail(HR_ERR_INVALID, "hr_debug_intersect: bad argument");
    int rc = debug_refusal(c, "hr_debug_intersect", NO_REGION | NO_MASK | A_SCENE);
    if (rc) return rc;
    HIP_TRY(hipSetDevice(c->device));
    CallScratch scratch;
    float *d_rays = nullptr, *d_out = nullptr;
    int32_t *d_el = nullptr;
    HIP_TRY_AS("hr_debug_intersect", scratch.alloc((void **)&d_rays, (size_t)n * 6 * 4));
    HIP_TRY_AS("hr_debug_intersect", scratch.alloc((void **)&d_out, (size_t)n * 8 * 4));
    HIP_TRY_AS("hr_debug_intersect", scratch.alloc((void **)&d_el, (size_t)n * 4));
    HIP_TRY_AS("hr_debug_intersect", hipMemcpy(d_rays, rays, (size_t)n * 6 * 4, hipMemcpyHostToDevice));
    hipLaunchKernelGGL(intersect_debug_kernel, dim3((n + 63) / 64), dim3(64), 0, c->stream, c->dsc, n, d_rays, d_out, d_el);
    HIP_TRY_AS("hr_debug_intersect", hipGetLastError());
    HIP_TRY_AS("hr_debug_intersect", hipStreamSynchronize(c->stream));
    HIP_TRY_AS("hr_debug_intersect", hipMemcpy(out, d_out, (size_t)n * 8 * 4, hipMemcpyDeviceToHost));
    HIP_TRY_AS("hr_debug_intersect", hipMemcpy(out_element, d_el, (size_t)n * 4, hipMemcpyDeviceToHost));
    return HR_OK;
}

int hr_debug_trace(hr_ctx *c, uint32_t n, const float *rays, const float *shadow_len, float *out, int32_t *out_element) {
    if (!c || !rays || !out || !out_element || !n) return fail(HR_ERR_INVALID, "hr_debug_trace: bad argument");
// ... 103 lines not shown
```

### hanamaru-renderer_amd/csrc/isaac_core.h

```cpp
#pragma once
#include "device_scene.h"

namespace hr {

typedef unsigned long long u64;

#if defined(__HIPCC__)
#define HR_NOUNROLL _Pragma("unroll 1")
#define HR_UNROLL _Pragma("unroll")
#else
#define HR_NOUNROLL
#define HR_UNROLL
#endif

#define HR_ISAAC_MIX(a, b, c, d, e, f, g, h) \
    a -= e; f ^= h >> 9;  h += a;            \
    b -= f; g ^= a << 9;  a += b;            \
    c -= g; h ^= b >> 23; b += c;            \
    d -= h; a ^= c << 15; c += d;            \
    e -= a; b ^= d >> 14; d += e;            \
    f -= b; c ^= e << 20; e += f;            \
    g -= c; d ^= f >> 17; f += g;            \
    h -= d; e ^= g << 14; g += h;

#if defined(__HIP_DEVICE_COMPILE__)
#include "isaac_mix_gfx950.h"
#define HR_ISAAC_MIXB_1(a, b, c, d, e, f, g, h) HR_ISAAC_MIX_R1(a, b, c, d, e, f, g, h)
#define HR_ISAAC_MIXB_2(a, b, c, d, e, f, g, h) HR_ISAAC_MIX_R2(a, b, c, d, e, f, g, h)
#else
#define HR_ISAAC_MIXB_1(a, b, c, d, e, f, g, h) HR_ISAAC_MIX(a, b, c, d, e, f, g, h)
#define HR_ISAAC_MIXB_2(a, b, c, d, e, f, g, h) HR_ISAAC_MIX(a, b, c, d, e, f, g, h)
#endif
#define HR_ISAAC_MIX_1(a, b, c, d, e, f, g, h) HR_ISAAC_MIX(a, b, c, d, e, f, g, h)
#define HR_ISAAC_MIX_2(a, b, c, d, e, f, g, h) HR_ISAAC_MIX(a, b, c, d, e, f, g, h)

struct IsaacWarm { u64 r[8]; };
HD IsaacWarm isaac_warm() {
    u64 a, b, c, d, e, f, g, h;
    a = b = c = d = e = f = g = h = 0x9e3779b97f4a7c13ULL;
    for (int i = 0; i < 4; i++) { HR_ISAAC_MIX(a, b, c, d, e, f, g, h) }
    IsaacWarm w;
    w.r[0] = a; w.r[1] = b; w.r[2] = c; w.r[3] = d; w.r[4] = e; w.r[5] = f; w.r[6] = g; w.r[7] = h;
    return w;
}

HD double isaac_to_f64(u64 v) {
    union { u64 u; double d; } cv;
    cv.u = 0x3FF0000000000000ULL | (v & 0x000FFFFFFFFFFFFFULL);
    return cv.d - 1.0;
}

template <class Out>
HD void isaac_init_final(Out &out, const IsaacWarm &w, u64 s0, u64 s1, u64 s2, u64 s3) {
    u64 A = w.r[0] + s0, B = w.r[1] + s1, C = w.r[2] + s2, D = w.r[3] + s3, E = w.r[4], F = w.r[5], G = w.r[6], H = w.r[7];
    HR_NOUNROLL
    for (int i = 0; i < 32; i++) { HR_ISAAC_MIX_2(A, B, C, D, E, F, G, H) }
    u64 a = w.r[0] + s0, b = w.r[1] + s1, c = w.r[2] + s2, d = w.r[3] + s3, e = w.r[4], f = w.r[5], g = w.r[6], h = w.r[7];
    HR_NOUNROLL
    for (int i = 0; i < 256; i += 8) {
        HR_ISAAC_MIX_1(a, b, c, d, e, f, g, h)
        A += a; B += b; C += c; D += d; E += e; F += f; G += g; H += h;
        HR_ISAAC_MIX_2(A, B, C, D, E, F, G, H)
        out.st8(i, A, B, C, D, E, F, G, H);
    }
}

template <int SPLIT, class Out>
HD void isaac_init_front(Out &out, const IsaacWarm &w, u64 s0, u64 s1, u64 s2, u64 s3) {
    u64 A = w.r[0] + s0, B = w.r[1] + s1, C = w.r[2] + s2, D = w.r[3] + s3, E = w.r[4], F = w.r[5], G = w.r[6], H = w.r[7];
    HR_NOUNROLL
    for (int i = 0; i < 32; i++) { HR_ISAAC_MIX_2(A, B, C, D, E, F, G, H) }
    u64 a = w.r[0] + s0, b = w.r[1] + s1, c = w.r[2] + s2, d = w.r[3] + s3, e = w.r[4], f = w.r[5], g = w.r[6], h = w.r[7];
    HR_NOUNROLL
    for (int i = 0; i < 8 * SPLIT; i += 8) {
        HR_ISAAC_MIX_1(a, b, c, d, e, f, g, h)
        A += a; B += b; C += c; D += d; E += e; F += f; G += g; H += h;
        HR_ISAAC_MIX_2(A, B, C, D, E, F, G, H)
        out.st8(i, A, B, C, D, E, F, G, H);
    }
    out.end2(0, a, b); out.end2(2, c, d); out.end2(4, e, f); out.end2(6, g, h);
    out.end2(8, A, B); out.end2(10, C, D); out.end2(12, E, F); out.end2(14, G, H);
}
template <int SPLIT, class Mem>
HD void isaac_init_back(Mem &mem, const u64 *st16) {
    u64 a = st16[0], b = st16[1], c = st16[2], d = st16[3], e = st16[4], f = st16[5], g = st16[6], h = st16[7];
    u64 A = st16[8], B = st16[9], C = st16[10], D = st16[11], E = st16[12], F = st16[13], G = st16[14], H = st16[15];
    HR_NOUNROLL
    for (int i = 8 * SPLIT; i < 256; i += 8) {
        HR_ISAAC_MIXB_1(a, b, c, d, e, f, g, h)
        A += a; B += b; C += c; D += d; E += e; F += f; G += g; H += h;
        HR_ISAAC_MIXB_2(A, B, C, D, E, F, G, H)
        mem.st(i, A); mem.st(i + 1, B); mem.st(i + 2, C); mem.st(i + 3, D);
        mem.st(i + 4, E); mem.st(i + 5, F); mem.st(i + 6, G); mem.st(i + 7, H);
    }
}

template <int B1, int B2, class Out>
HD void isaac_init_ahead(Out &out, const IsaacWarm &w, u64 s0, u64 s1, u64 s2, u64 s3) {
    static_assert(0 < B1 && B1 < B2 && B2 < 32, "segment boundaries");
    u64 A = w.r[0] + s0, B = w.r[1] + s1, C = w.r[2] + s2, D = w.r[3] + s3, E = w.r[4], F = w.r[5], G = w.r[6], H = w.r[7];
    HR_NOUNROLL
    for (int i = 0; i < 32; i++) { HR_ISAAC_MIX_2(A, B, C, D, E, F, G, H) }
    u64 a = w.r[0] + s0, b = w.r[1] + s1, c = w.r[2] + s2, d = w.r[3] + s3, e = w.r[4], f = w.r[5], g = w.r[6], h = w.r[7];
    out.state(0, a, b, c, d, e, f, g, h, A, B, C, D, E, F, G, H);
    HR_NOUNROLL
    for (int i = 0; i < B1; i++) {
        HR_ISAAC_MIX_1(a, b, c, d, e, f, g, h)
        A += a; B += b; C += c; D += d; E += e; F += f; G += g; H += h;
        HR_ISAAC_MIX_2(A, B, C, D, E, F, G, H)
    }
    out.state(1, a, b, c, d, e, f, g, h, A, B, C, D, E, F, G, H);
    HR_NOUNROLL
    for (int i = B1; i < B2; i++) {
        HR_ISAAC_MIX_1(a, b, c, d, e, f, g, h)
        A += a; B += b; C += c; D += d; E += e; F += f; G += g; H += h;
        HR_ISAAC_MIX_2(A, B, C, D, E, F, G, H)
    }
    out.state(2, a, b, c, d, e, f, g, h, A, B, C, D, E, F, G, H);
}
template <int NBLK, class Mem>
HD void isaac_init_run(Mem &mem, const u64 *st16) {
    u64 a = st16[0], b = st16[1], c = st16[2], d = st16[3], e = st16[4], f = st16[5], g = st16[6], h = st16[7];
    u64 A = st16[8], B = st16[9], C = st16[10], D = st16[11], E = st16[12], F = st16[13], G = st16[14], H = st16[15];
    HR_NOUNROLL
    for (int i = 0; i < 8 * NBLK; i += 8) {
        HR_ISAAC_MIXB_1(a, b, c, d, e, f, g, h)
        A += a; B += b; C += c; D += d; E += e; F += f; G += g; H += h;
        HR_ISAAC_MIXB_2(A, B, C, D, E, F, G, H)
        mem.st(i, A); mem.st(i + 1, B); mem.st(i + 2, C); mem.st(i + 3, D);
        mem.st(i + 4, E); mem.st(i + 5, F); mem.st(i + 6, G); mem.st(i + 7, H);
    }
}

template <class Out>
HD void isaac_init_ahead_pre(Out &out, const IsaacWarm &w, u64 s0, u64 s1, u64 s2, u64 s3) {
    u64 A = w.r[0] + s0, B = w.r[1] + s1, C = w.r[2] + s2, D = w.r[3] + s3, E = w.r[4], F = w.r[5], G = w.r[6], H = w.r[7];
    HR_NOUNROLL
    for (int i = 0; i < 32; i++) { HR_ISAAC_MIX_2(A, B, C, D, E, F, G, H) }
    u64 a = w.r[0] + s0, b = w.r[1] + s1, c = w.r[2] + s2, d = w.r[3] + s3, e = w.r[4], f = w.r[5], g = w.r[6], h = w.r[7];
    out.state(0, a, b, c, d, e, f, g, h, A, B, C, D, E, F, G, H);
#define HR_AHEAD_TO(from, to)                                                  \
    HR_NOUNROLL                                                                \
    for (int i = from; i < to; i++) {                                          \
        HR_ISAAC_MIX_1(a, b, c, d, e, f, g, h)                                 \
        A += a; B += b; C += c; D += d; E += e; F += f; G += g; H += h;        \
        HR_ISAAC_MIX_2(A, B, C, D, E, F, G, H)                                 \
    }                                                                          \
    if (out.wants(to)) out.state(to, a, b, c, d, e, f, g, h, A, B, C, D, E, F, G, H);
    HR_AHEAD_TO(0, 8)
    HR_AHEAD_TO(8, 12)
    HR_AHEAD_TO(12, 16)
    HR_AHEAD_TO(16, 24)
#undef HR_AHEAD_TO
}
template <int P>
HD void isaac_init_prerun(u64 *st16, u64 (*kept)[8]) {
    u64 a = st16[0], b = st16[1], c = st16[2], d = st16[3], e = st16[4], f = st16[5], g = st16[6], h = st16[7];
    u64 A = st16[8], B = st16[9], C = st16[10], D = st16[11], E = st16[12], F = st16[13], G = st16[14], H = st16[15];
    HR_UNROLL
    for (int p = 0; p < P; p++) {
        HR_ISAAC_MIX_1(a, b, c, d, e, f, g, h)
        A += a; B += b; C += c; D += d; E += e; F += f; G += g; H += h;
        HR_ISAAC_MIX_2(A, B, C, D, E, F, G, H)
        kept[p][0] = A; kept[p][1] = B; kept[p][2] = C; kept[p][3] = D; kept[p][4] = E; kept[p][5] = F; kept[p][6] = G; kept[p][7] = H;
    }
    st16[0] = a; st16[1] = b; st16[2] = c; st16[3] = d; st16[4] = e; st16[5] = f; st16[6] = g; st16[7] = h;
    st16[8] = A; st16[9] = B; st16[10] = C; st16[11] = D; st16[12] = E; st16[13] = F; st16[14] = G; st16[15] = H;
}

struct AheadRegs { u64 a, b, c, d, e, f, g, h, A, B, C, D, E, F, G, H; };
#define HR_AHEAD_BLOCK(r)                                                                           \
    HR_ISAAC_MIX_1(r.a, r.b, r.c, r.d, r.e, r.f, r.g, r.h)                                          \
    r.A += r.a; r.B += r.b; r.C += r.c; r.D += r.d; r.E += r.e; r.F += r.f; r.G += r.g; r.H += r.h; \
    HR_ISAAC_MIX_2(r.A, r.B, r.C, r.D, r.E, r.F, r.G, r.H)
template <int P1BLK, class Out>
HD void isaac_ahead_part1(Out &out, const IsaacWarm &w, u64 s0, u64 s1, u64 s2, u64 s3, AheadRegs &r) {
    r.A = w.r[0] + s0; r.B = w.r[1] + s1; r.C = w.r[2] + s2; r.D = w.r[3] + s3; r.E = w.r[4]; r.F = w.r[5]; r.G = w.r[6]; r.H = w.r[7];
    HR_NOUNROLL
    for (int i = 0; i < 32; i++) { HR_ISAAC_MIX_2(r.A, r.B, r.C, r.D, r.E, r.F, r.G, r.H) }
    r.a = w.r[0] + s0; r.b = w.r[1] + s1; r.c = w.r[2] + s2; r.d = w.r[3] + s3; r.e = w.r[4]; r.f = w.r[5]; r.g = w.r[6]; r.h = w.r[7];
    out.state(0, r.a, r.b, r.c, r.d, r.e, r.f, r.g, r.h, r.A, r.B, r.C, r.D, r.E, r.F, r.G, r.H);
    HR_NOUNROLL
    for (int i = 0; i < P1BLK; i++) { HR_AHEAD_BLOCK(r) }
}
template <int NRUN, int NBLK, int P1BLK, class Out>
HD void isaac_ahead_part2(Out &out, AheadRegs &r) {
    static_assert(NRUN * NBLK == 32 && P1BLK > 0 && P1BLK < NBLK, "runs tile the sweep; part 1 ends inside the first run");
    HR_NOUNROLL
    for (int i = P1BLK; i < NBLK; i++) { HR_AHEAD_BLOCK(r) }
    out.state(1, r.a, r.b, r.c, r.d, r.e, r.f, r.g, r.h, r.A, r.B, r.C, r.D, r.E, r.F, r.G, r.H);
    HR_NOUNROLL
    for (int k = 2; k < NRUN; k++) {
        HR_NOUNROLL
        for (int i = 0; i < NBLK; i++) { HR_AHEAD_BLOCK(r) }
        out.state(k, r.a, r.b, r.c, r.d, r.e, r.f, r.g, r.h, r.A, r.B, r.C, r.D, r.E, r.F, r.G, r.H);
    }
}

template <int TAILN, class Mem, class Tail>
HD void isaac_round(Mem &mem, Tail &tail);

template <int TAILN, class Mem, class Tail>
HD void isaac_seed_round(Mem &mem, const IsaacWarm &w, u64 s0, u64 s1, u64 s2, u64 s3, Tail &tail) {
    u64 a = w.r[0], b = w.r[1], c = w.r[2], d = w.r[3], e = w.r[4], f = w.r[5], g = w.r[6], h = w.r[7];
    a += s0; b += s1; c += s2; d += s3;
    HR_NOUNROLL
    for (int i = 0; i < 256; i += 8) {
        HR_ISAAC_MIX_1(a, b, c, d, e, f, g, h)
        mem.st(i, a); mem.st(i + 1, b); mem.st(i + 2, c); mem.st(i + 3, d);
        mem.st(i + 4, e); mem.st(i + 5, f); mem.st(i + 6, g); mem.st(i + 7, h);
    }
    HR_NOUNROLL
    for (int i = 0; i < 256; i += 8) {
        a += mem.ld(i); b += mem.ld(i + 1); c += mem.ld(i + 2); d += mem.ld(i + 3);
        e += mem.ld(i + 4); f += mem.ld(i + 5); g += mem.ld(i + 6); h += mem.ld(i + 7);
        HR_ISAAC_MIX_1(a, b, c, d, e, f, g, h)
        mem.st(i, a); mem.st(i + 1, b); mem.st(i + 2, c); mem.st(i + 3, d);
        mem.st(i + 4, e); mem.st(i + 5, f); mem.st(i + 6, g); mem.st(i + 7, h);
    }
    isaac_round<TAILN>(mem, tail);
}

#if defined(__HIP_DEVICE_COMPILE__)
#define HR_OPAQUE64(v) asm volatile("" : "+v"(v))
#define HR_OPAQUE32(p) asm volatile("" : "+v"(p))
#define HR_SCHED_FENCE() __builtin_amdgcn_sched_barrier(0)
#else
#define HR_OPAQUE64(v)
#define HR_OPAQUE32(p)
#define HR_SCHED_FENCE()
#endif

template <int TAILN, int NG, class Mem, class Tail>
HD void isaac_round_n(Mem *mem, Tail *tail) {
    static_assert(TAILN % 4 == 0 && TAILN >= 8 && TAILN <= 124, "tail steps");
    u64 aa[NG], x[NG], xn[NG], xnn[NG], m2v[NG], g1[NG], T[NG], g2[NG], xprev[NG];
    uint32_t p1[NG];
    HR_UNROLL for (int g = 0; g < NG; g++) {
        x[g] = mem[g].ld(0); xn[g] = mem[g].ld(1); xnn[g] = mem[g].ld(2); m2v[g] = mem[g].ld(128);
        g1[g] = mem[g].ld((int)((x[g] >> 3) & 255));
        aa[g] = ~(u64)0 + m2v[g];
        m2v[g] = mem[g].ld(129);
        T[g] = g1[g] + aa[g] + 1; g2[g] = 0; xprev[g] = 0;
        p1[g] = mem[g].off((int)((xn[g] >> 3) & 255));
    }
#define HR_ISAAC_STEP(N, MIXEXPR_NEXT, XN3_IDX, M2N_IDX, TAIL, TAILPREV)                                               \
    {                                                                                                                  \
        HR_UNROLL for (int g = 0; g < NG; g++) HR_OPAQUE32(p1[g]);                                                            \
        HR_SCHED_FENCE();                                                                                              \
        u64 g2n[NG];                                                                                                   \
        HR_UNROLL for (int g = 0; g < NG; g++) {                                                                       \
            u64 y = T[g] + g2[g];                                        \
            mem[g].st(N, y);                                                                                           \
            g1[g] = mem[g].ldo(p1[g]);                     \
            g2n[g] = mem[g].ld((int)((y >> 11) & 255));                                                                \
        }                                                                                                              \
        HR_SCHED_FENCE();                                                                                              \
        HR_UNROLL for (int g = 0; g < NG; g++) {                                                                       \
            if (TAILPREV) tail[g].put((N) - 1, g2[g] + xprev[g]);                                                      \
            g2[g] = g2n[g];                                                                                            \
            p1[g] = mem[g].off((int)((xnn[g] >> 3) & 255));                                                            \
            u64 xn3 = mem[g].ld(XN3_IDX);                                                                              \
            u64 m2n = mem[g].ld(M2N_IDX);                                                                              \
            const u64 A_ = aa[g];                                                                                      \
            aa[g] = (MIXEXPR_NEXT) + m2v[g];                                                              \
            T[g] = g1[g] + (aa[g] + x[g]);                                      \
            HR_OPAQUE64(T[g]);                                                                                         \
            xprev[g] = x[g]; x[g] = xn[g]; xn[g] = xnn[g]; xnn[g] = xn3; m2v[g] = m2n;                                 \
        }                                                                                                              \
    }
    HR_ISAAC_STEP(0, A_ ^ (A_ >> 5), 3, 130, false, false)
    HR_ISAAC_STEP(1, A_ ^ (A_ << 12), 4, 131, false, false)
    HR_ISAAC_STEP(2, A_ ^ (A_ >> 33), 5, 132, false, false)
    HR_ISAAC_STEP(3, ~(A_ ^ (A_ << 21)), 6, 133, false, false)
    HR_NOUNROLL
    for (int n = 4; n < 124; n += 4) {
        HR_ISAAC_STEP(n, A_ ^ (A_ >> 5), n + 3, n + 130, false, false)
        HR_ISAAC_STEP(n + 1, A_ ^ (A_ << 12), n + 4, n + 131, false, false)
        HR_ISAAC_STEP(n + 2, A_ ^ (A_ >> 33), n + 5, n + 132, false, false)
        HR_ISAAC_STEP(n + 3, ~(A_ ^ (A_ << 21)), n + 6, n + 133, false, false)
    }
    HR_ISAAC_STEP(124, A_ ^ (A_ >> 5), 127, 254, false, false)
    HR_ISAAC_STEP(125, A_ ^ (A_ << 12), 128, 255, false, false)
    HR_ISAAC_STEP(126, A_ ^ (A_ >> 33), 129, 0, false, false)
    HR_ISAAC_STEP(127, ~(A_ ^ (A_ << 21)), 130, 1, false, false)
    HR_NOUNROLL
    for (int n = 128; n < 256 - TAILN; n += 4) {
        HR_ISAAC_STEP(n, A_ ^ (A_ >> 5), n + 3, n - 126, false, false)
        HR_ISAAC_STEP(n + 1, A_ ^ (A_ << 12), n + 4, n - 125, false, false)
        HR_ISAAC_STEP(n + 2, A_ ^ (A_ >> 33), n + 5, n - 124, false, false)
        HR_ISAAC_STEP(n + 3, ~(A_ ^ (A_ << 21)), n + 6, n - 123, false, false)
    }
    HR_ISAAC_STEP(256 - TAILN, A_ ^ (A_ >> 5), 256 - TAILN + 3, 256 - TAILN - 126, true, false)
    HR_ISAAC_STEP(256 - TAILN + 1, A_ ^ (A_ << 12), 256 - TAILN + 4, 256 - TAILN - 125, true, true)
    HR_ISAAC_STEP(256 - TAILN + 2, A_ ^ (A_ >> 33), 256 - TAILN + 5, 256 - TAILN - 124, true, true)
    HR_ISAAC_STEP(256 - TAILN + 3, ~(A_ ^ (A_ << 21)), 256 - TAILN + 6, 256 - TAILN - 123, true, true)
    HR_NOUNROLL
    for (int n = 256 - TAILN + 4; n < 252; n += 4) {
        HR_ISAAC_STEP(n, A_ ^ (A_ >> 5), n + 3, n - 126, true, true)
        HR_ISAAC_STEP(n + 1, A_ ^ (A_ << 12), n + 4, n - 125, true, true)
        HR_ISAAC_STEP(n + 2, A_ ^ (A_ >> 33), n + 5, n - 124, true, true)
        HR_ISAAC_STEP(n + 3, ~(A_ ^ (A_ << 21)), n + 6, n - 123, true, true)
    }
    HR_ISAAC_STEP(252, A_ ^ (A_ >> 5), 255, 126, true, true)
    HR_ISAAC_STEP(253, A_ ^ (A_ << 12), 255, 127, true, true)
    HR_ISAAC_STEP(254, A_ ^ (A_ >> 33), 255, 127, true, true)
    HR_ISAAC_STEP(255, ~(A_ ^ (A_ << 21)), 255, 127, true, true)
    HR_UNROLL for (int g = 0; g < NG; g++) tail[g].put(255, g2[g] + xprev[g]);
#undef HR_ISAAC_STEP
}
struct NoRoundSync {
    static constexpr bool ON = false;
    static constexpr int N1 = 0, K1 = 0, N2 = 0, K2 = 0;
    HD void mid() const {}
};
template <class Mem, class Tail, class Sync = NoRoundSync>
HD void isaac_round_deep28(Mem &mem, Tail &tail, const Sync &sync = Sync()) {
    constexpr int TAILN = 28;
    u64 aa, x0, x1, x2, x3, m1, m2, g1, T, g2, xprev;
    uint32_t p1;
    x0 = mem.ld(0); x1 = mem.ld(1); x2 = mem.ld(2); x3 = mem.ld(3);
    g1 = mem.ld((int)((x0 >> 3) & 255));
    aa = ~(u64)0 + mem.ld(128);
    m1 = mem.ld(129); m2 = mem.ld(130);
    T = g1 + aa + 1; g2 = 0; xprev = 0;
    p1 = mem.off((int)((x1 >> 3) & 255));
#define DSTEP(N, R, MIXEXPR_NEXT, X4_IDX, M3_IDX, TAIL, TAILPREV)                                   \
    {                                                                                               \
        HR_OPAQUE32(p1);                                                                            \
        HR_SCHED_FENCE();                                                                           \
        u64 y = T + g2;                                                                             \
        mem.st((N) + (R), y);                                                                       \
        g1 = mem.ldo(p1);                                                                           \
        u64 g2n = mem.ld((int)((y >> 11) & 255));                                                   \
        HR_SCHED_FENCE();                                                                           \
        if (TAILPREV) tail.put((N) - 1, g2 + xprev);                                                \
        g2 = g2n;                                                                                   \
        p1 = mem.off((int)((x2 >> 3) & 255));                                                       \
        u64 x4 = mem.ld((X4_IDX) + (R));                                                            \
        u64 m3 = mem.ld(M3_IDX);                                                                    \
        const u64 A_ = aa;                                                                          \
        aa = (MIXEXPR_NEXT) + m1;                                                                   \
        T = g1 + (aa + x0);                                                                         \
        HR_OPAQUE64(T);                                                                             \
        xprev = x0; x0 = x1; x1 = x2; x2 = x3; x3 = x4; m1 = m2; m2 = m3;                           \
    }
#define DSTEP4(n, R, MO, TAIL, TP0)                                            \
    DSTEP((n), R, A_ ^ (A_ >> 5), (n) + 4, (n) + (MO), TAIL, TP0)              \
    DSTEP((n) + 1, R, A_ ^ (A_ << 12), (n) + 5, (n) + 1 + (MO), TAIL, TAIL)    \
    DSTEP((n) + 2, R, A_ ^ (A_ >> 33), (n) + 6, (n) + 2 + (MO), TAIL, TAIL)    \
    DSTEP((n) + 3, R, ~(A_ ^ (A_ << 21)), (n) + 7, (n) + 3 + (MO), TAIL, TAIL)
#define DSTEP20(n, R, MO, TAIL) DSTEP4(n, R, MO, TAIL, TAIL) DSTEP4((n) + 4, R, MO, TAIL, TAIL) DSTEP4((n) + 8, R, MO, TAIL, TAIL) DSTEP4((n) + 12, R, MO, TAIL, TAIL) DSTEP4((n) + 16, R, MO, TAIL, TAIL)
#define DHOOK(n, NN, KK, k) if (Sync::ON && Sync::KK == (k) && (n) == Sync::NN) sync.mid();
#define DSTEP20S(n, R, MO, NN, KK) DSTEP4(n, R, MO, false, false) DHOOK(n, NN, KK, 1) DSTEP4((n) + 4, R, MO, false, false) DHOOK(n, NN, KK, 2) DSTEP4((n) + 8, R, MO, false, false) DHOOK(n, NN, KK, 3) DSTEP4((n) + 12, R, MO, false, false) DHOOK(n, NN, KK, 4) DSTEP4((n) + 16, R, MO, false, false)
    DSTEP4(0, 0, 131, false, false)
    HR_NOUNROLL
    for (int n = 4; n < 124; n += 20) { DSTEP20S(n, 0, 131, N1, K1) }
    DSTEP(124, 0, A_ ^ (A_ >> 5), 128, 255, false, false)
    DSTEP(125, 0, A_ ^ (A_ << 12), 129, 0, false, false)
    DSTEP(126, 0, A_ ^ (A_ >> 33), 130, 1, false, false)
    DSTEP(127, 0, ~(A_ ^ (A_ << 21)), 131, 2, false, false)
    HR_NOUNROLL
    for (int n = 128; n < 256 - TAILN; n += 20) { DSTEP20S(n, 0, -125, N2, K2) }
    int tb = 128;
    HR_OPAQUE32(tb);
#define DTAILR (tb - 128)
    DSTEP4(256 - TAILN, DTAILR, -125, true, false)
    DSTEP20(256 - TAILN + 4, DTAILR, -125, true)
    DSTEP(252, DTAILR, A_ ^ (A_ >> 5), 255, 127, true, true)
    DSTEP(253, DTAILR, A_ ^ (A_ << 12), 255, 127, true, true)
    DSTEP(254, DTAILR, A_ ^ (A_ >> 33), 255, 127, true, true)
    DSTEP(255, DTAILR, ~(A_ ^ (A_ << 21)), 255, 127, true, true)
    tail.put(255, g2 + xprev);
    static_assert(256 - TAILN + 28 == 256, "the tail is 4 + 20 + 4 steps");
#undef DTAILR
#undef DSTEP
#undef DSTEP4
#undef DSTEP20
#undef DSTEP20S
#undef DHOOK
}
template <int TAILN, class Mem, class Tail>
HD void isaac_round(Mem &mem, Tail &tail) {
    if constexpr (TAILN == 28) isaac_round_deep28(mem, tail);
// ... 85 lines not shown
```

### hanamaru-renderer_amd/csrc/kernel_variants.h

```cpp
#pragma once

#define HR_VARIANT(kernel, ...) {__VA_ARGS__, kernel<__VA_ARGS__>}
template <class Row, size_t N, class Match>
static const Row *find_row(const Row (&table)[N], Match match) {
    for (const Row &r : table)
        if (match(r)) return &r;
    return nullptr;
}
template <class Row>
static auto fn_of(const Row *r) -> decltype(r->fn) { return r ? r->fn : nullptr; }

typedef void (*TraceFn)(Scene, RenderParams, float *, Counters *, uint32_t *, uint32_t *);
struct TraceVariant { bool cnt; int minw; bool qn, rr, log, prec, list; TraceFn fn; };
static const TraceVariant TRACE_VARIANTS[] = {
    HR_VARIANT(trace_kernel, false, 5, true, false, false, false, false), HR_VARIANT(trace_kernel, false, 5, false, false, false, false, false),
    HR_VARIANT(trace_kernel, false, 4, true, false, false, false, false), HR_VARIANT(trace_kernel, false, 6, true, false, false, false, false),
    HR_VARIANT(trace_kernel, true, 3, true, false, false, false, false), HR_VARIANT(trace_kernel, true, 3, false, false, false, false, false),
    HR_VARIANT(trace_kernel, false, 5, true, true, false, false, false), HR_VARIANT(trace_kernel, false, 5, false, true, false, false, false),
    HR_VARIANT(trace_kernel, true, 3, true, true, false, false, false), HR_VARIANT(trace_kernel, true, 3, false, true, false, false, false),
    HR_VARIANT(trace_kernel, false, 4, true, false, false, true, false), HR_VARIANT(trace_kernel, false, 4, false, false, false, true, false),
    HR_VARIANT(trace_kernel, false, 5, true, false, false, true, false), HR_VARIANT(trace_kernel, false, 3, true, false, false, true, false),
    HR_VARIANT(trace_kernel, true, 3, true, false, false, true, false), HR_VARIANT(trace_kernel, true, 3, false, false, false, true, false),
    HR_VARIANT(trace_kernel, false, 3, true, false, true, false, false), HR_VARIANT(trace_kernel, false, 3, false, false, true, false, false),
    HR_VARIANT(trace_kernel, false, 3, true, false, true, true, false), HR_VARIANT(trace_kernel, false, 3, false, false, true, true, false),
    HR_VARIANT(trace_kernel, false, 5, true, false, false, false, true), HR_VARIANT(trace_kernel, false, 5, false, false, false, false, true),
    HR_VARIANT(trace_kernel, false, 4, true, false, false, true, true), HR_VARIANT(trace_kernel, false, 4, false, false, false, true, true),
};
static TraceFn select_trace_kernel(bool counters, bool qn, bool rr, bool precise, int min_waves, bool log, bool list = false) {
    bool cnt = counters, prec = precise;
    int minw;
    if (log) { cnt = false; rr = false; minw = 3; }
    else if (rr) { prec = false; minw = cnt ? 3 : 5; }
    else if (cnt) minw = 3;
    else if (prec) minw = !qn ? 4 : min_waves == 6 ? 5 : min_waves == 4 ? 3 : 4;
    else minw = !qn ? 5 : min_waves == 4 ? 4 : min_waves == 6 ? 6 : 5;
    if (list && (cnt || rr || log || min_waves != 5)) return nullptr;
    return fn_of(find_row(TRACE_VARIANTS, [&](const TraceVariant &r) { return r.cnt == cnt && r.minw == minw && r.qn == qn && r.rr == rr && r.log == log && r.prec == prec && r.list == list; }));
}

typedef void (*WfStartFn)(Scene, RenderParams, float *, WfQueues);
struct WfStartVariant { bool prec, list; WfStartFn fn; };
static const WfStartVariant WF_START_VARIANTS[] = {HR_VARIANT(wf_start_kernel, false, false), HR_VARIANT(wf_start_kernel, true, false),
                                                   HR_VARIANT(wf_start_kernel, false, true), HR_VARIANT(wf_start_kernel, true, true)};
static WfStartFn select_wf_start_kernel(bool precise, bool list = false) {
    return fn_of(find_row(WF_START_VARIANTS, [&](const WfStartVariant &r) { return r.prec == precise && r.list == list; }));
}

typedef void (*WfTraverseFn)(Scene, RenderParams, WfQueues, uint32_t, Counters *);
struct WfTraverseVariant { bool cnt, qn; WfTraverseFn fn; };
static const WfTraverseVariant WF_TRAVERSE_VARIANTS[] = {HR_VARIANT(wf_traverse_kernel, false, true), HR_VARIANT(wf_traverse_kernel, false, false),
                                                         HR_VARIANT(wf_traverse_kernel, true, true), HR_VARIANT(wf_traverse_kernel, true, false)};
typedef void (*WfShadeFn)(Scene, RenderParams, float *, WfQueues, uint32_t, Counters *, uint32_t *);
struct WfShadeVariant { bool cnt, prec, log; WfShadeFn fn; };
static const WfShadeVariant WF_SHADE_VARIANTS[] = {HR_VARIANT(wf_shade_kernel, false, false, false), HR_VARIANT(wf_shade_kernel, false, true, false),
                                                   HR_VARIANT(wf_shade_kernel, true, false, false),  HR_VARIANT(wf_shade_kernel, true, true, false),
                                                   HR_VARIANT(wf_shade_kernel, false, false, true),  HR_VARIANT(wf_shade_kernel, false, true, true)};
static WfTraverseFn select_wf_traverse_kernel(bool counters, bool qn, bool log) {
    const bool cnt = counters && !log;
    return fn_of(find_row(WF_TRAVERSE_VARIANTS, [&](const WfTraverseVariant &r) { return r.cnt == cnt && r.qn == qn; }));
}
static WfShadeFn select_wf_shade_kernel(bool counters, bool precise, bool log) {
    const bool cnt = counters && !log;
    return fn_of(find_row(WF_SHADE_VARIANTS, [&](const WfShadeVariant &r) { return r.cnt == cnt && r.prec == precise && r.log == log; }));
}

typedef void (*DebugRenderFn)(Scene, RenderParams, int, float *, Counters *);
struct DebugRenderVariant { bool cnt, qn; DebugRenderFn fn; };
static const DebugRenderVariant DEBUG_RENDER_VARIANTS[] = {HR_VARIANT(debug_render_kernel, false, true), HR_VARIANT(debug_render_kernel, false, false),
                                                           HR_VARIANT(debug_render_kernel, true, true), HR_VARIANT(debug_render_kernel, true, false)};
static DebugRenderFn select_debug_render_kernel(bool counters, bool qn) {
    return fn_of(find_row(DEBUG_RENDER_VARIANTS, [&](const DebugRenderVariant &r) { return r.cnt == counters && r.qn == qn; }));
}
typedef void (*GuideRenderFn)(Scene, RenderParams, float *);
struct GuideRenderVariant { bool qn; GuideRenderFn fn; };
static const GuideRenderVariant GUIDE_RENDER_VARIANTS[] = {HR_VARIANT(guide_render_kernel, true), HR_VARIANT(guide_render_kernel, false)};
static GuideRenderFn select_guide_render_kernel(bool qn) {
    return fn_of(find_row(GUIDE_RENDER_VARIANTS, [&](const GuideRenderVariant &r) { return r.qn == qn; }));
}
typedef void (*GuideChainFn)(Scene, RenderParams, uint32_t, float *);
struct GuideChainVariant { bool qn; GuideChainFn fn; };
static const GuideChainVariant GUIDE_CHAIN_VARIANTS[] = {HR_VARIANT(guide_chain_kernel, true), HR_VARIANT(guide_chain_kernel, false)};
static GuideChainFn select_guide_chain_kernel(bool qn) {
    return fn_of(find_row(GUIDE_CHAIN_VARIANTS, [&](const GuideChainVariant &r) { return r.qn == qn; }));
}
typedef void (*GuideLensFn)(Scene, RenderParams, uint32_t, uint32_t, float *);
struct GuideLensVariant { bool qn; GuideLensFn fn; };
static const GuideLensVariant GUIDE_LENS_VARIANTS[] = {HR_VARIANT(guide_lens_kernel, true), HR_VARIANT(guide_lens_kernel, false)};
static GuideLensFn select_guide_lens_kernel(bool qn) {
    return fn_of(find_row(GUIDE_LENS_VARIANTS, [&](const GuideLensVariant &r) { return r.qn == qn; }));
}
typedef void (*TraceDebugFn)(Scene, RenderParams, uint32_t, const float *, const float *, float *, int32_t *, Counters *);
struct TraceDebugVariant { bool qn, cnt; TraceDebugFn fn; };
static const TraceDebugVariant TRACE_DEBUG_VARIANTS[] = {HR_VARIANT(trace_debug_kernel, true, false), HR_VARIANT(trace_debug_kernel, false, false),
                                                         HR_VARIANT(trace_debug_kernel, true, true), HR_VARIANT(trace_debug_kernel, false, true)};
static TraceDebugFn select_trace_debug_kernel(bool counters, bool qn) {
    return fn_of(find_row(TRACE_DEBUG_VARIANTS, [&](const TraceDebugVariant &r) { return r.cnt == counters && r.qn == qn; }));
}

struct SeedVariant { int mode, split, prof; bool lo; const void *fn; uint32_t threads; bool ring; bool list = false; bool pre = false; };
static const SeedVariant SEED_VARIANTS[] = {
    {0, 0, 0, false, (const void *)seed_isaac64_kernel, 64 * SEED_WAVES, false},
    {1, 8, 0, false, (const void *)seed_pc_kernel<8>, 256, true},
    {1, 12, 0, false, (const void *)seed_pc_kernel<12>, 256, true},
    {1, 16, 0, false, (const void *)seed_pc_kernel<16>, 256, true},
    {1, 20, 0, false, (const void *)seed_pc_kernel<20>, 256, true},
    {1, 24, 0, false, (const void *)seed_pc_kernel<24>, 256, true},
    {1, 28, 0, false, (const void *)seed_pc_kernel<28>, 256, true},
    {1, 16, 1, false, (const void *)seed_pc_kernel<16, true>, 256, true},
    {1, 20, 1, false, (const void *)seed_pc_kernel<20, true>, 256, true},
    {2, 0, 0, false, (const void *)seed_seg_kernel<false, false>, 256, true},
    {2, 0, 1, false, (const void *)seed_seg_kernel<true, false>, 256, true},
    {2, 0, 0, true, (const void *)seed_seg_kernel<false, true>, 256, true},
    {2, 0, 1, true, (const void *)seed_seg_kernel<true, true>, 256, true},
    {2, 0, 0, false, (const void *)seed_seg_kernel<false, false, true>, 256, true, true},
    {2, 0, 0, true, (const void *)seed_seg_kernel<false, true, true>, 256, true, true},
    {2, 0, 2, false, (const void *)seed_seg_kernel<2, false>, 256, true},
    {2, 0, 0, false, (const void *)seed_seg_kernel<false, false, false, true>, 256, true, false, true},
    {2, 0, 1, false, (const void *)seed_seg_kernel<true, false, false, true>, 256, true, false, true},
    {2, 0, 0, true, (const void *)seed_seg_kernel<false, true, false, true>, 256, true, false, true},
    {2, 0, 1, true, (const void *)seed_seg_kernel<true, true, false, true>, 256, true, false, true},
    {2, 0, 0, false, (const void *)seed_seg_kernel<false, false, true, true>, 256, true, true, true},
    {2, 0, 0, true, (const void *)seed_seg_kernel<false, true, true, true>, 256, true, true, true},
    {2, 0, 2, false, (const void *)seed_seg_kernel<2, false, false, true>, 256, true, false, true},
#if defined(HR_EXPERIMENTS)
    {3, 0, 0, false, (const void *)seed_ps_kernel<0>, 256, true},
    {3, 0, 1, false, (const void *)seed_ps_kernel<1>, 256, true},
    {3, 0, 2, false, (const void *)seed_ps_kernel<2>, 256, true},
    {3, 0, 3, false, (const void *)seed_ps_kernel<3>, 256, true},
    {4, 0, 0, false, (const void *)seed_w5_kernel<false>, 320, true},
    {4, 0, 1, false, (const void *)seed_w5_kernel<true>, 320, true},
#endif
};
static const SeedVariant *select_seed_kernel(int seed_mode, int seed_split, int seed_prof, bool twin, bool list = false, bool prerun = false) {
    int split = 0, prof = seed_prof ? 1 : 0;
    bool lo = false, pre = false;
    if (seed_mode == 2) { lo = twin; pre = prerun; if (seed_prof == 2) prof = 2; }
    else if (seed_mode == 1) split = prof ? (seed_split == 20 ? 20 : 16) : seed_split;
    else if (seed_mode == 3) prof = seed_prof >= 1 && seed_prof <= 3 ? seed_prof : 0;
    else if (seed_mode == 0) prof = 0;
    return find_row(SEED_VARIANTS, [&](const SeedVariant &r) { return r.mode == seed_mode && r.split == split && r.prof == prof && r.lo == lo && r.list == list && r.pre == pre; });
}

typedef void (*AccumulateFn)(RenderParams, const float *, float *, double *, uint32_t *);
struct AccumulateVariant { bool mom, cnts, list; AccumulateFn fn; };
static const AccumulateVariant ACCUMULATE_VARIANTS[] = {HR_VARIANT(accumulate_kernel, false, false, false), HR_VARIANT(accumulate_kernel, true, false, false),
                                                        HR_VARIANT(accumulate_kernel, false, true, false),  HR_VARIANT(accumulate_kernel, true, true, false),
                                                        HR_VARIANT(accumulate_kernel, false, true, true),   HR_VARIANT(accumulate_kernel, true, true, true)};
static AccumulateFn select_accumulate_kernel(bool moments, bool counts, bool list) {
    return fn_of(find_row(ACCUMULATE_VARIANTS, [&](const AccumulateVariant &r) { return r.mom == moments && r.cnts == counts && r.list == list; }));
}

typedef void (*BucketFn)(RenderParams, const float *, double *, const uint32_t *, uint32_t, unsigned long long);
struct BucketVariant {
    bool cnts, list, bys;
    BucketFn fn;
    constexpr BucketVariant(bool c, bool l, BucketFn f) : cnts(c), list(l), bys(false), fn(f) {}
    constexpr BucketVariant(bool c, bool l, bool b, BucketFn f) : cnts(c), list(l), bys(b), fn(f) {}
};
static const BucketVariant BUCKET_VARIANTS[] = {HR_VARIANT(bucket_kernel, false, false), HR_VARIANT(bucket_kernel, true, false), HR_VARIANT(bucket_kernel, true, true),
                                                HR_VARIANT(bucket_kernel, false, false, true), HR_VARIANT(bucket_kernel, true, false, true), HR_VARIANT(bucket_kernel, true, true, true)};
static BucketFn select_bucket_kernel(bool counts, bool list, bool by_sampling) {
    return fn_of(find_row(BUCKET_VARIANTS, [&](const BucketVariant &r) { return r.cnts == counts && r.list == list && r.bys == by_sampling; }));
}

typedef void (*RobustNoiseFn)(const double *, const uint32_t *, unsigned long long, size_t, double, double, double *, uint8_t *, double *);
struct RobustNoiseVariant { uint32_t k; bool stage; RobustNoiseFn fn; uint32_t lds() const { return stage ? 256u * 3u * k * (uint32_t)sizeof(double) : 0u; } };
static const RobustNoiseVariant ROBUST_NOISE_VARIANTS[] = {
    HR_VARIANT(robust_noise_kernel, 3, true),   HR_VARIANT(robust_noise_kernel, 5, true),   HR_VARIANT(robust_noise_kernel, 7, true),  HR_VARIANT(robust_noise_kernel, 9, true),
    HR_VARIANT(robust_noise_kernel, 11, true),  HR_VARIANT(robust_noise_kernel, 13, true),  HR_VARIANT(robust_noise_kernel, 15, true),
    HR_VARIANT(robust_noise_kernel, 3, false),  HR_VARIANT(robust_noise_kernel, 5, false),  HR_VARIANT(robust_noise_kernel, 7, false), HR_VARIANT(robust_noise_kernel, 9, false),
    HR_VARIANT(robust_noise_kernel, 11, false), HR_VARIANT(robust_noise_kernel, 13, false), HR_VARIANT(robust_noise_kernel, 15, false),
};
#if defined(HR_ROBUST_NOISE_PER_LANE)
static const bool ROBUST_NOISE_STAGED = false;
#else
static const bool ROBUST_NOISE_STAGED = true;
#endif
static const RobustNoiseVariant *select_robust_noise_kernel(uint32_t k, bool stage) {
    return find_row(ROBUST_NOISE_VARIANTS, [&](const RobustNoiseVariant &r) { return r.k == k && r.stage == stage; });
}

template <class Fn>
struct KRow { uint32_t k; Fn fn; uint32_t lds() const { return 256u * 3u * k * (uint32_t)sizeof(double); } };
typedef void (*RobustFn)(const double *, const uint32_t *, unsigned long long, float *, uint8_t *, size_t);
typedef KRow<RobustFn> RobustVariant;
static const RobustVariant ROBUST_VARIANTS[] = {
    HR_VARIANT(robust_kernel, 3),  HR_VARIANT(robust_kernel, 5),  HR_VARIANT(robust_kernel, 7),  HR_VARIANT(robust_kernel, 9),
    HR_VARIANT(robust_kernel, 11), HR_VARIANT(robust_kernel, 13), HR_VARIANT(robust_kernel, 15),
};
static const RobustVariant *select_robust_kernel(uint32_t k) {
    return find_row(ROBUST_VARIANTS, [&](const RobustVariant &r) { return r.k == k; });
}
typedef void (*RobustDenoiseInitFn)(const double *, const uint32_t *, unsigned long long, const float *, double *, size_t, int);
typedef KRow<RobustDenoiseInitFn> RobustDenoiseInitVariant;
static const RobustDenoiseInitVariant ROBUST_DENOISE_INIT_VARIANTS[] = {
    HR_VARIANT(robust_denoise_init_kernel, 3),  HR_VARIANT(robust_denoise_init_kernel, 5),  HR_VARIANT(robust_denoise_init_kernel, 7),
    HR_VARIANT(robust_denoise_init_kernel, 9),  HR_VARIANT(robust_denoise_init_kernel, 11), HR_VARIANT(robust_denoise_init_kernel, 13),
    HR_VARIANT(robust_denoise_init_kernel, 15),
};
static const RobustDenoiseInitVariant *select_robust_denoise_init_kernel(uint32_t k) {
    return find_row(ROBUST_DENOISE_INIT_VARIANTS, [&](const RobustDenoiseInitVariant &r) { return r.k == k; });
}

typedef void (*RestoreInitFn)(const double *, const uint32_t *, unsigned long long, double *, size_t);
typedef KRow<RestoreInitFn> RestoreInitVariant;
static const RestoreInitVariant RESTORE_INIT_VARIANTS[] = {
    HR_VARIANT(restore_init_kernel, 3),  HR_VARIANT(restore_init_kernel, 5),  HR_VARIANT(restore_init_kernel, 7),  HR_VARIANT(restore_init_kernel, 9),
    HR_VARIANT(restore_init_kernel, 11), HR_VARIANT(restore_init_kernel, 13), HR_VARIANT(restore_init_kernel, 15),
};
static const RestoreInitVariant *select_restore_init_kernel(uint32_t k) {
    return find_row(RESTORE_INIT_VARIANTS, [&](const RestoreInitVariant &r) { return r.k == k; });
}

typedef void (*SelectInitFn)(const double *, const uint32_t *, uint32_t, const float *, const double *, const float *, double *, double *, size_t, int);
typedef KRow<SelectInitFn> SelectInitVariant;
static const SelectInitVariant SELECT_INIT_VARIANTS[] = {
    HR_VARIANT(select_init_kernel, 3),  HR_VARIANT(select_init_kernel, 5),  HR_VARIANT(select_init_kernel, 7),  HR_VARIANT(select_init_kernel, 9),
    HR_VARIANT(select_init_kernel, 11), HR_VARIANT(select_init_kernel, 13), HR_VARIANT(select_init_kernel, 15),
};
static const SelectInitVariant *select_select_init_kernel(uint32_t k) {
    return find_row(SELECT_INIT_VARIANTS, [&](const SelectInitVariant &r) { return r.k == k; });
}
```

### hanamaru-renderer_amd/csrc/seed_kernels.h

```cpp
#pragma once
#include <hip/hip_runtime.h>

#include "adapt_core.h"
#include "device_scene.h"
#include "isaac_core.h"

using namespace hr;


__device__ __forceinline__ uint32_t lds_addr(const void *p) { return (uint32_t)(size_t)(const __attribute__((address_space(3))) void *)p; }
__device__ __forceinline__ u64 lds_load64(uint32_t a) { return *(const __attribute__((address_space(3))) u64 *)(size_t)a; }

static const int SEED_COLS = 80;
static const int SEED_WAVES = 2, SEED_LANES = SEED_COLS / SEED_WAVES;
__device__ __forceinline__ uint32_t seed_gov_begin(const RenderParams &rp, bool stamp) {
    if (!rp.gov) return rp.pad[1];
    const int32_t lvl = __hip_atomic_load(&rp.gov->level, __ATOMIC_RELAXED, __HIP_MEMORY_SCOPE_AGENT);
    if (stamp) {
        atomicMin(&rp.gov->t0[0][rp.gov_slot], (unsigned long long)__builtin_amdgcn_s_memrealtime());
        if (blockIdx.x == 0) rp.gov->lvl[0][rp.gov_slot] = (uint32_t)lvl;
    }
    return gov_producer_prio(lvl, rp.pad[1] & 3u);
}
__device__ __forceinline__ void seed_gov_end(const RenderParams &rp, bool stamp) {
// ... 226 lines not shown
        __syncthreads();
        HR_STAMP(3);
        if (it < n_groups) load_regs(r.G0 + it);
        RecStore rs(recs, pid);
        RecordTail<RecStore> lt(rs, lens_shape);
        if (lane < (uint32_t)SEED_LANES) {
            isaac_round<REC_DRAWS>(m, lt);
            lt.finish();
        }
        HR_STAMP(4);
        ovf_note(lane < (uint32_t)SEED_LANES && valid && lt.overflow(), pid, ovf_list, ovf_count, rp.ovf_cap);
        HR_STAMP(5);
        if (PROF) pc[7]++;
        __syncthreads();
        HR_STAMP(6);
    }
#undef HR_STAMP
    if (PROF && lane == 0)
        for (int i = 0; i < 8; i++) atomicAdd(&cnt->seed_phase[i], pc[i]);
    const bool lane_on = lane < (uint32_t)SEED_LANES;
    seed_fixup_wave(rp, lens_shape, m, colr, lane_on, ovf_list, ovf_count, win + (size_t)(blockIdx.x * 2u + half) * SEED_WIN_WORDS, recs, cnt);
}
template <int SEED_SPLIT>
__device__ __forceinline__ void seed_pc_producer(const RenderParams &rp, const PcRange &r, unsigned char *smem, uint32_t lane, uint32_t half) {
    typedef PcLayout<SEED_SPLIT> L;
    constexpr int CHUNKS = L::SHIP_ROWS * SEED_LANES * 8 / 1024;
    static_assert(CHUNKS % 2 == 0, "fill is unrolled by two");
    const IsaacWarm warm = isaac_warm();
    uint64_t frontier = r.first_path & ~63ull;
    const uint64_t n_groups = r.G1 - r.G0;
    for (uint64_t it = 0; it <= n_groups; it++) {
        if (it > 0) {
            if (!(rp.pad[2] & 8u)) {
                const uint64_t g = r.G0 + it - 1;
                const u64 *src = r.ring_wg + (g & (SEED_RING_GROUPS - 1)) * L::GROUP_WORDS + half * L::HALF_WORDS;
                const unsigned char *gsrc = reinterpret_cast<const unsigned char *>(src) + lane * 16u;
                unsigned char *ldst = smem + (size_t)half * SEED_LDS_HALF_BYTES;
#pragma unroll 5
                for (int q = 0; q < CHUNKS; q += 2, gsrc += 2048, ldst += 2048) {
                    const void __attribute__((address_space(1))) *gp = (const void __attribute__((address_space(1))) *)gsrc;
                    void __attribute__((address_space(3))) *lp = (void __attribute__((address_space(3))) *)ldst;
                    __builtin_amdgcn_global_load_lds(gp, lp, 16, 0, 2);
                    __builtin_amdgcn_global_load_lds(gp, lp, 16, 1024, 2);
                }
                __builtin_amdgcn_s_waitcnt(0);
            }
            __syncthreads();
        }
        const uint64_t need = (r.G0 + it + 2) * SEED_COLS;
        uint32_t n = 0;
        while (frontier < need && frontier < r.end_path) {
            if ((n & 1u) == half) {
                const uint64_t pid0 = frontier + lane;
                const bool on = pid0 >= r.first_path && pid0 < r.end_path && !(rp.pad[2] & 4u);
                const uint64_t ppid = pid0 >= r.first_path && pid0 < r.end_path ? pid0 : r.end_path - 1;
                const uint32_t item = (uint32_t)(ppid >> 6), j = (uint32_t)(ppid & 63u);
                uint32_t tile = item / rp.num_k, k = item - tile * rp.num_k;
                uint32_t px, py, sub;
                tile_lane_frame_pixel(rp, tile, j, px, py, sub);
                bool pvalid = px < rp.width && py < rp.height;
                u64 s, t;
                path_seed_words(rp.width, rp.height, pvalid ? px : 0u, pvalid ? py : 0u, sub, s, t);
                const uint64_t g = ppid / SEED_COLS;
                const uint32_t c80 = (uint32_t)(ppid - g * SEED_COLS);
                RingState<SEED_SPLIT> out(r.ring_wg + (g & (SEED_RING_GROUPS - 1)) * L::GROUP_WORDS + (c80 >= (uint32_t)SEED_LANES ? L::HALF_WORDS : 0), c80 % SEED_LANES, lane);
                if (on) isaac_init_front<SEED_SPLIT>(out, warm, 8700304ULL, (u64)(rp.sampling_begin + k * rp.stride), s, t);
            }
            frontier += 64;
            n++;
        }
        __builtin_amdgcn_s_waitcnt(0);
        __syncthreads();
    }
}
template <int SEED_SPLIT, bool PROF = false>
__global__ __launch_bounds__(256) void seed_pc_kernel(RenderParams rp, int lens_shape, u64 *__restrict__ ring, float *__restrict__ recs,
                                                      uint32_t *__restrict__ ovf, u64 *__restrict__ win, Counters *cnt) {
    extern __shared__ __align__(16) unsigned char smem[];
    const uint32_t lane = threadIdx.x & 63u, wave = threadIdx.x >> 6, half = wave & 1u;
    const bool consumer = wave < 2u;
    const uint32_t pprio = consumer ? 0u : seed_gov_begin(rp, wave == 2u && lane == 0u);
    const uint32_t prio = consumer ? rp.pad[0] : pprio & 3u;
    switch (prio) {
        case 0: break;
        case 1: __builtin_amdgcn_s_setprio(1); break;
        case 2: __builtin_amdgcn_s_setprio(2); break;
        default: __builtin_amdgcn_s_setprio(3); break;
    }
    PcRange r;
    r.paths = (uint64_t)rp.tiles_x * rp.tiles_y * rp.num_k * 64u;
    const uint64_t groups = (r.paths + SEED_COLS - 1) / SEED_COLS;
    r.G0 = groups * blockIdx.x / gridDim.x; r.G1 = groups * (blockIdx.x + 1) / gridDim.x;
    r.first_path = r.G0 * SEED_COLS; r.end_path = r.G1 * SEED_COLS < r.paths ? r.G1 * SEED_COLS : r.paths;
    r.ring_wg = ring + (size_t)blockIdx.x * SEED_RING_WORDS_MAX;
    if (consumer) seed_pc_consumer<SEED_SPLIT, PROF>(rp, lens_shape, r, smem, lane, half, recs, ovf, win, cnt);
    else {
        seed_pc_producer<SEED_SPLIT>(rp, r, smem, lane, half);
        seed_gov_end(rp, wave == 2u && lane == 0u);
    }
}

struct SegLayout {
    static const size_t STATE_WORDS = (size_t)16 * SEED_LANES;
    static const size_t HALF_WORDS = 3 * STATE_WORDS;
    static const size_t GROUP_WORDS = 2 * HALF_WORDS;
};
static_assert(SEED_RING_GROUPS * SegLayout::GROUP_WORDS <= SEED_RING_WORDS_MAX, "the ring allocation of the producer / consumer kernel holds it");
struct SegStateOut {
    u64 *base;
    __device__ __forceinline__ void state(int k, u64 a, u64 b, u64 c, u64 d, u64 e, u64 f, u64 g, u64 h, u64 A, u64 B, u64 C, u64 D, u64 E, u64 F, u64 G, u64 H) {
        typedef u64 u64x2 __attribute__((ext_vector_type(2)));
        u64x2 *dst = reinterpret_cast<u64x2 *>(base + (size_t)k * SegLayout::STATE_WORDS);
        const u64x2 q[8] = {{a, b}, {c, d}, {e, f}, {g, h}, {A, B}, {C, D}, {E, F}, {G, H}};
#pragma unroll
        for (int j = 0; j < 8; j++) asm volatile("global_store_dwordx4 %0, %1, off sc1\n\ts_nop 1" : : "v"(dst + j * SEED_LANES), "v"(q[j]) : "memory");
    }
};
struct SegLane {
    uint32_t col, run;
    bool on;
};
__device__ __forceinline__ SegLane seg_lane(bool consumer, uint32_t lane) {
    SegLane l;
    if (lane < (uint32_t)SEED_LANES) { l.col = lane; l.run = consumer ? 2u : 0u; l.on = true; }
    else if (consumer) { l.col = lane - (uint32_t)SEED_LANES; l.run = 1u; l.on = true; }
    else { l.col = lane - 16u; l.run = 1u; l.on = lane < 56u; if (!l.on) l.col = (uint32_t)SEED_LANES - 1u; }
    return l;
}
struct SegRegs {
    typedef u64 u64x2_t __attribute__((ext_vector_type(2)));
    u64x2_t v[8];
    __device__ __forceinline__ void load(const u64 *ring_wg, uint64_t g, uint32_t half, const SegLane &l) {
        const u64 *regs = ring_wg + (g & (SEED_RING_GROUPS - 1)) * SegLayout::GROUP_WORDS + half * SegLayout::HALF_WORDS + (size_t)l.run * SegLayout::STATE_WORDS + (size_t)l.col * 2u;
#pragma unroll
        for (int q = 0; q < 8; q++) v[q] = __builtin_nontemporal_load(reinterpret_cast<const u64x2_t *>(regs + q * (2 * SEED_LANES)));
    }
    __device__ __forceinline__ void run(unsigned char *lds_half, const SegLane &l) const {
        u64 st16[16];
#pragma unroll
        for (int q = 0; q < 8; q++) { st16[2 * q] = v[q].x; st16[2 * q + 1] = v[q].y; }
        const uint32_t first = l.run == 0u ? 0u : l.run == 1u ? (uint32_t)SEG_B1 : (uint32_t)SEG_B2;
        LdsHalfMem m{reinterpret_cast<u64 *>(lds_half) + l.col + (size_t)first * 8u * SEED_LANES};
        if (l.on) isaac_init_run<SEG_NBLK>(m, st16);
    }
};
struct SegpLayout {
    static const size_t WAVE_WORDS = (size_t)16 * 64;
    static const size_t HALF_WORDS = 2 * WAVE_WORDS;
    static const size_t GROUP_WORDS = 2 * HALF_WORDS;
};
static_assert(SEED_RING_GROUPS * SegpLayout::GROUP_WORDS <= SEED_RING_WORDS_MAX, "the ring allocation of the producer / consumer kernel holds it");
static_assert(2 * SEGP_XCOLS == 64 && SEGP_XCOLS + 4 * (SEED_LANES - SEGP_XCOLS) == 64, "64 producer runs and 64 consumer runs per half");
static_assert(SEGP_PNBLK == SEGP_PRE + SEGP_NBLK && 2 * SEGP_PNBLK + SEGP_NBLK == 32 && 4 * SEGP_NBLK == 32 && SEGP_AHEAD_END == 32 - SEGP_NBLK, "the runs tile the sweep");
struct SegpStateOut {
    u64 *half;
    uint32_t col;
    __device__ __forceinline__ bool wants(int block) const { return segp_wants(col, block); }
    __device__ __forceinline__ void state(int block, u64 a, u64 b, u64 c, u64 d, u64 e, u64 f, u64 g, u64 h, u64 A, u64 B, u64 C, u64 D, u64 E, u64 F, u64 G, u64 H) {
        typedef u64 u64x2 __attribute__((ext_vector_type(2)));
        const uint32_t s = segp_slot(col, block);
        u64x2 *dst = reinterpret_cast<u64x2 *>(half + (size_t)(s >> 6) * SegpLayout::WAVE_WORDS + (size_t)(s & 63u) * 2u);
        const u64x2 q[8] = {{a, b}, {c, d}, {e, f}, {g, h}, {A, B}, {C, D}, {E, F}, {G, H}};
#pragma unroll
        for (int j = 0; j < 8; j++) asm volatile("global_store_dwordx4 %0, %1, off sc1\n\ts_nop 1" : : "v"(dst + j * 64), "v"(q[j]) : "memory");
    }
};
struct SegpLane {
    uint32_t slot, col, first;
};
__device__ __forceinline__ SegpLane segp_lane(bool consumer, uint32_t lane) {
    SegpLane l;
    uint32_t nblk;
    l.slot = (consumer ? 64u : 0u) + lane;
    segp_run(l.slot, l.col, l.first, nblk);
    return l;
}
struct SegpRegs {
    typedef u64 u64x2_t __attribute__((ext_vector_type(2)));
    u64x2_t v[8];
    __device__ __forceinline__ void load(const u64 *ring_wg, uint64_t g, uint32_t half, const SegpLane &l) {
        const u64 *regs = ring_wg + (g & (SEED_RING_GROUPS - 1)) * SegpLayout::GROUP_WORDS + half * SegpLayout::HALF_WORDS + (size_t)(l.slot >> 6) * SegpLayout::WAVE_WORDS + (size_t)(l.slot & 63u) * 2u;
#pragma unroll
        for (int q = 0; q < 8; q++) v[q] = __builtin_nontemporal_load(reinterpret_cast<const u64x2_t *>(regs + q * 128));
    }
    __device__ __forceinline__ void run(unsigned char *lds_half, const SegpLane &l) const {
        u64 st16[16];
#pragma unroll
        for (int q = 0; q < 8; q++) { st16[2 * q] = v[q].x; st16[2 * q + 1] = v[q].y; }
        LdsHalfMem m{reinterpret_cast<u64 *>(lds_half) + l.col + (size_t)l.first * 8u * SEED_LANES};
        isaac_init_run<SEGP_NBLK>(m, st16);
    }
    __device__ __forceinline__ void prerun(u64 (*kept)[8]) {
        u64 st16[16];
#pragma unroll
        for (int q = 0; q < 8; q++) { st16[2 * q] = v[q].x; st16[2 * q + 1] = v[q].y; }
        isaac_init_prerun<SEGP_PRE>(st16, kept);
#pragma unroll
        for (int q = 0; q < 8; q++) { v[q].x = st16[2 * q]; v[q].y = st16[2 * q + 1]; }
    }
    __device__ __forceinline__ void finish(unsigned char *lds_half, const SegpLane &l, const u64 (*kept)[8]) const {
        LdsHalfMem k{reinterpret_cast<u64 *>(lds_half) + l.col + (size_t)l.first * 8u * SEED_LANES};
#pragma unroll
        for (int p = 0; p < SEGP_PRE; p++)
#pragma unroll
            for (int j = 0; j < 8; j++) k.st(p * 8 + j, kept[p][j]);
        u64 st16[16];
#pragma unroll
        for (int q = 0; q < 8; q++) { st16[2 * q] = v[q].x; st16[2 * q + 1] = v[q].y; }
        LdsHalfMem m{k.col + (size_t)SEGP_PRE * 8u * SEED_LANES};
        isaac_init_run<SEGP_NBLK>(m, st16);
    }
};
template <bool PRE> struct SegForm { typedef SegLane Lane; typedef SegRegs Regs; static __device__ __forceinline__ Lane lane(bool consumer, uint32_t l) { return seg_lane(consumer, l); } };
template <> struct SegForm<true> { typedef SegpLane Lane; typedef SegpRegs Regs; static __device__ __forceinline__ Lane lane(bool consumer, uint32_t l) { return segp_lane(consumer, l); } };
template <bool PROF, bool LO, bool LIST, bool PRE>
__device__ __forceinline__ void seed_seg_consumer(const RenderParams &rp, int lens_shape, const PcRange &r, unsigned char *smem, uint32_t lane, uint32_t half,
                                                  float *__restrict__ recs, uint32_t *__restrict__ ovf, u64 *__restrict__ win, Counters *cnt) {
    uint32_t *ovf_list = ovf + (size_t)(blockIdx.x * 2u + half) * rp.ovf_cap;
    uint32_t ovf_count = 0;
    unsigned long long pc[8] = {0, 0, 0, 0, 0, 0, 0, 0}, tm = 0;
#define HR_STAMP(i) do { if (PROF) { unsigned long long now_ = __builtin_readcyclecounter(); pc[i] += now_ - tm; tm = now_; } } while (0)
    const typename SegForm<PRE>::Lane sl = SegForm<PRE>::lane(true, lane);
    typename SegForm<PRE>::Regs regs;
    const uint32_t colr = lane < (uint32_t)SEED_LANES ? lane : 0u;
    unsigned char *lds_half = smem + (size_t)half * SEED_LDS_HALF_BYTES;
    LdsHalfMem m{reinterpret_cast<u64 *>(lds_half) + colr};
    const uint64_t n_groups = r.G1 - r.G0;
    if (PRE) __syncthreads();
    __syncthreads();
    for (uint64_t it = 1; it <= n_groups; it++) {
        if (PROF) tm = __builtin_readcyclecounter();
        const uint64_t g = r.G0 + it - 1;
        if (it == 1) regs.load(r.ring_wg, g, half, sl);
        const uint64_t pid = g * SEED_COLS + half * SEED_LANES + colr;
        const bool in_range = pid < r.paths;
        const uint32_t item = (uint32_t)((in_range ? pid : r.paths - 1) >> 6), j = (uint32_t)((in_range ? pid : r.paths - 1) & 63u);
        uint32_t tile = item / rp.num_k;
        uint32_t px, py, sub;
        tile_lane_frame_pixel(rp, launch_tile<LIST>(rp, tile), j, px, py, sub);
        const bool valid = in_range && px < rp.width && py < rp.height;
        HR_STAMP(0);
        if (PROF) { __builtin_amdgcn_s_waitcnt(0x0F70); HR_STAMP(1); }
        regs.run(lds_half, sl);
        HR_STAMP(2);
        __syncthreads();
        HR_STAMP(3);
        if (it < n_groups) regs.load(r.ring_wg, r.G0 + it, half, sl);
        RecStore rs(recs, pid, rp.rec_lo_off);
        RecordTail<RecStore, LO> lt(rs, lens_shape);
        if (lane < (uint32_t)SEED_LANES) {
            isaac_round<REC_DRAWS>(m, lt);
            lt.finish();
        }
        HR_STAMP(4);
        ovf_note(lane < (uint32_t)SEED_LANES && valid && lt.overflow(), pid, ovf_list, ovf_count, rp.ovf_cap);
        HR_STAMP(5);
        if (PROF) pc[7]++;
        __syncthreads();
        HR_STAMP(6);
    }
#undef HR_STAMP
    if (PROF && lane == 0)
        for (int i = 0; i < 8; i++) atomicAdd(&cnt->seed_phase[i], pc[i]);
    const bool lane_on = lane < (uint32_t)SEED_LANES;
    seed_fixup_wave<LdsHalfMem, LO, LIST>(rp, lens_shape, m, colr, lane_on, ovf_list, ovf_count, win + (size_t)(blockIdx.x * 2u + half) * SEED_WIN_WORDS, recs, cnt);
}
static const uint32_t SEG_PROF_FIT = 563u * SEGP_PRE;
template <bool LIST, bool PRE, bool PROF>
__device__ __forceinline__ void seed_seg_producer(const RenderParams &rp, const PcRange &r, unsigned char *smem, uint32_t lane, uint32_t half, const uint32_t pprio, Counters *cnt) {
    const IsaacWarm warm = isaac_warm();
    const typename SegForm<PRE>::Lane sl = SegForm<PRE>::lane(false, lane);
    typename SegForm<PRE>::Regs regs;
    u64 kept[PRE ? SEGP_PRE : 1][8];
    uint32_t pc[8] = {0, 0, 0, 0, 0, 0, 0, 0}, tm = 0, chunks = 0;
#define HR_NOW() __builtin_amdgcn_readfirstlane((uint32_t)__builtin_readcyclecounter())
#define HR_STAMP(i) do { if (PROF) { const uint32_t now_ = HR_NOW(); pc[i] = __builtin_amdgcn_readfirstlane(pc[i] + (now_ - tm)); tm = now_; } } while (0)
    unsigned char *lds_half = smem + (size_t)half * SEED_LDS_HALF_BYTES;
    const uint64_t n_groups = r.G1 - r.G0;
    uint64_t frontier = r.first_path & ~63ull;
    auto ahead = [&](uint64_t upto) {
        const uint64_t need = upto * SEED_COLS;
        for (; frontier < need && frontier < r.end_path; frontier += 64) {
            if (((frontier >> 6) & 1u) != half) continue;
            const uint64_t pid0 = frontier + lane;
            const bool on = pid0 >= r.first_path && pid0 < r.end_path && !(rp.pad[2] & 4u);
            const uint64_t ppid = pid0 >= r.first_path && pid0 < r.end_path ? pid0 : r.end_path - 1;
            const uint32_t item = (uint32_t)(ppid >> 6), j = (uint32_t)(ppid & 63u);
            uint32_t tile = item / rp.num_k, k = item - tile * rp.num_k;
            uint32_t px, py, sub;
            tile_lane_frame_pixel(rp, launch_tile<LIST>(rp, tile), j, px, py, sub);
            bool pvalid = px < rp.width && py < rp.height;
            u64 s, t;
            path_seed_words(rp.width, rp.height, pvalid ? px : 0u, pvalid ? py : 0u, sub, s, t);
            const uint64_t g = ppid / SEED_COLS;
            const uint32_t c80 = (uint32_t)(ppid - g * SEED_COLS), hh = c80 >= (uint32_t)SEED_LANES ? 1u : 0u;
            if constexpr (PRE) {
                SegpStateOut out{r.ring_wg + (g & (SEED_RING_GROUPS - 1)) * SegpLayout::GROUP_WORDS + hh * SegpLayout::HALF_WORDS, c80 - hh * (uint32_t)SEED_LANES};
                if (on) isaac_init_ahead_pre(out, warm, 8700304ULL, (u64)(rp.sampling_begin + k * rp.stride), s, t);
            } else {
                SegStateOut out{r.ring_wg + (g & (SEED_RING_GROUPS - 1)) * SegLayout::GROUP_WORDS + hh * SegLayout::HALF_WORDS + (size_t)(c80 - hh * (uint32_t)SEED_LANES) * 2u};
                if (on) isaac_init_ahead<SEG_B1, SEG_B2>(out, warm, 8700304ULL, (u64)(rp.sampling_begin + k * rp.stride), s, t);
            }
            if (PROF) chunks = __builtin_amdgcn_readfirstlane(chunks + 1u);
        }
        __builtin_amdgcn_s_waitcnt(0);
    };
    ahead(r.G0 + 2);
    if constexpr (PRE) {
        __syncthreads();
        regs.load(r.ring_wg, r.G0, half, sl);
        regs.prerun(kept);
        __syncthreads();
    } else {
        __syncthreads();
        if (n_groups >= 1) regs.load(r.ring_wg, r.G0, half, sl);
    }
    for (uint64_t it = 1; it <= n_groups; it++) {
        if (PROF) { tm = HR_NOW(); chunks = 0; }
        if constexpr (PRE) regs.finish(lds_half, sl, kept);
        else regs.run(lds_half, sl);
        HR_STAMP(0);
        __syncthreads();
        HR_STAMP(1);
        if (it < n_groups) regs.load(r.ring_wg, r.G0 + it, half, sl);
        if (((pprio >> 2) & 3u) != (pprio & 3u)) {
            const uint32_t pr = (it & 1u) ? (pprio >> 2) & 3u : pprio & 3u;
            if (pr == 0u) __builtin_amdgcn_s_setprio(0); else if (pr == 1u) __builtin_amdgcn_s_setprio(1); else if (pr == 2u) __builtin_amdgcn_s_setprio(2); else __builtin_amdgcn_s_setprio(3);
        }
        ahead(r.G0 + it + 2);
        if constexpr (PRE) regs.prerun(kept);
        HR_STAMP(2);
        __syncthreads();
        if (PROF) {
            const uint32_t now_ = HR_NOW(), wait = now_ - tm;
            tm = now_;
            const bool busy = chunks != 0;
            pc[3] = __builtin_amdgcn_readfirstlane(pc[3] + (busy ? wait : 0u));
            pc[4] = __builtin_amdgcn_readfirstlane(pc[4] + (busy ? 0u : wait));
            pc[5] = __builtin_amdgcn_readfirstlane(pc[5] + (busy ? 1u : 0u));
            pc[6] = __builtin_amdgcn_readfirstlane(pc[6] + (busy && wait < SEG_PROF_FIT ? 1u : 0u));
            pc[7] = __builtin_amdgcn_readfirstlane(pc[7] + 1u);
        }
    }
#undef HR_STAMP
#undef HR_NOW
    if (PROF && lane == 0)
        for (int i = 0; i < 8; i++) atomicAdd(&cnt->seed_phase[i], (unsigned long long)pc[i]);
}
template <int PROF = 0, bool LO = false, bool LIST = false, bool PRE = false>
__global__ __launch_bounds__(256) void seed_seg_kernel(RenderParams rp, int lens_shape, u64 *__restrict__ ring, float *__restrict__ recs,
                                                       uint32_t *__restrict__ ovf, u64 *__restrict__ win, Counters *cnt) {
    extern __shared__ __align__(16) unsigned char smem[];
    const uint32_t lane = threadIdx.x & 63u, wave = threadIdx.x >> 6, half = wave & 1u;
    const bool consumer = wave < 2u;
    const uint32_t pprio = consumer ? 0u : seed_gov_begin(rp, wave == 2u && lane == 0u);
    const uint32_t prio = consumer ? rp.pad[0] : pprio & 3u;
    switch (prio) {
        case 0: break;
        case 1: __builtin_amdgcn_s_setprio(1); break;
        case 2: __builtin_amdgcn_s_setprio(2); break;
        default: __builtin_amdgcn_s_setprio(3); break;
    }
    PcRange r;
    r.paths = (uint64_t)launch_tiles<LIST>(rp) * rp.num_k * 64u;
    const uint64_t groups = (r.paths + SEED_COLS - 1) / SEED_COLS;
    r.G0 = groups * blockIdx.x / gridDim.x; r.G1 = groups * (blockIdx.x + 1) / gridDim.x;
    r.first_path = r.G0 * SEED_COLS; r.end_path = r.G1 * SEED_COLS < r.paths ? r.G1 * SEED_COLS : r.paths;
    r.ring_wg = ring + (size_t)blockIdx.x * SEED_RING_WORDS_MAX;
    if (consumer) seed_seg_consumer<PROF == 1, LO, LIST, PRE>(rp, lens_shape, r, smem, lane, half, recs, ovf, win, cnt);
    else {
        seed_seg_producer<LIST, PRE, PROF == 2>(rp, r, smem, lane, half, pprio, cnt);
        seed_gov_end(rp, wave == 2u && lane == 0u);
    }
}

#if defined(HR_EXPERIMENTS)
static const int PS_NRUN = 4, PS_NBLK = 8, PS_P1BLK = 4;
struct PsLayout {
    static const size_t STATE_WORDS = (size_t)16 * SEED_LANES;
    static const size_t HALF_WORDS = PS_NRUN * STATE_WORDS;
    static const size_t GROUP_WORDS = 2 * HALF_WORDS;
};
static_assert(SEED_RING_GROUPS * PsLayout::GROUP_WORDS <= SEED_RING_WORDS_MAX, "the ring allocation of the producer / consumer kernel holds it");
struct PsStateOut {
    u64 *base;
    __device__ __forceinline__ void state(int k, u64 a, u64 b, u64 c, u64 d, u64 e, u64 f, u64 g, u64 h, u64 A, u64 B, u64 C, u64 D, u64 E, u64 F, u64 G, u64 H) {
        typedef u64 u64x2 __attribute__((ext_vector_type(2)));
        u64x2 *dst = reinterpret_cast<u64x2 *>(base + (size_t)k * PsLayout::STATE_WORDS);
        const u64x2 q[8] = {{a, b}, {c, d}, {e, f}, {g, h}, {A, B}, {C, D}, {E, F}, {G, H}};
#pragma unroll
        for (int j = 0; j < 8; j++) asm volatile("global_store_dwordx4 %0, %1, off sc1\n\ts_nop 1" : : "v"(dst + j * SEED_LANES), "v"(q[j]) : "memory");
    }
};
struct PsLane { uint32_t col, run; bool on; };
__device__ __forceinline__ PsLane ps_lane(uint32_t slot, uint32_t lane) {
    const uint32_t L = slot * 64u + lane;
    PsLane l;
    l.on = L < (uint32_t)(PS_NRUN * SEED_LANES);
    const uint32_t Lc = l.on ? L : 0u;
    l.run = Lc / (uint32_t)SEED_LANES; l.col = Lc - l.run * (uint32_t)SEED_LANES;
    return l;
}
struct PsRegs {
    typedef u64 u64x2_t __attribute__((ext_vector_type(2)));
    u64x2_t v[8];
    __device__ __forceinline__ void load(const u64 *ring_wg, uint64_t g, uint32_t half, const PsLane &l) {
        const u64 *regs = ring_wg + (g & (SEED_RING_GROUPS - 1)) * PsLayout::GROUP_WORDS + half * PsLayout::HALF_WORDS + (size_t)l.run * PsLayout::STATE_WORDS + (size_t)l.col * 2u;
#pragma unroll
        for (int q = 0; q < 8; q++) v[q] = __builtin_nontemporal_load(reinterpret_cast<const u64x2_t *>(regs + q * (2 * SEED_LANES)));
    }
    __device__ __forceinline__ void run(unsigned char *lds_half, const PsLane &l) const {
        u64 st16[16];
#pragma unroll
        for (int q = 0; q < 8; q++) { st16[2 * q] = v[q].x; st16[2 * q + 1] = v[q].y; }
        LdsHalfMem m{reinterpret_cast<u64 *>(lds_half) + l.col + (size_t)(l.run * (uint32_t)PS_NBLK) * 8u * SEED_LANES};
        if (l.on) isaac_init_run<PS_NBLK>(m, st16);
    }
};
template <bool PROF>
struct PsRoundSync {
    static constexpr bool ON = true;
    static constexpr int N1 = 104, K1 = 2, N2 = 148, K2 = 2;
    unsigned long long *pc, *tm; mutable int k;
    __device__ __forceinline__ void mid() const {
        if (PROF) { unsigned long long now = __builtin_readcyclecounter(); pc[3 + 2 * k] += now - *tm; *tm = now; }
        __builtin_amdgcn_s_barrier();
        if (PROF) { unsigned long long now = __builtin_readcyclecounter(); pc[4 + 2 * k] += now - *tm; *tm = now; k++; }
    }
};
template <int PROF>
__device__ __forceinline__ void seed_ps_consumer(const RenderParams &rp, int lens_shape, const PcRange &r, unsigned char *smem, uint32_t lane, uint32_t half,
                                                 float *__restrict__ recs, uint32_t *__restrict__ ovf, u64 *__restrict__ win, Counters *cnt) {
    uint32_t *ovf_list = ovf + (size_t)(blockIdx.x * 2u + half) * rp.ovf_cap;
    uint32_t ovf_count = 0;
    const PsLane sl = ps_lane(0u, lane);
    PsRegs regs;
    constexpr bool P = PROF != 0;
    unsigned long long pc[8] = {0, 0, 0, 0, 0, 0, 0, 0}, tm = 0;
#define HR_STAMP(i) do { if (P) { unsigned long long now_ = __builtin_readcyclecounter(); pc[i] += now_ - tm; tm = now_; } } while (0)
    const uint32_t colr = lane < (uint32_t)SEED_LANES ? lane : 0u;
    unsigned char *lds_half = smem + (size_t)half * SEED_LDS_HALF_BYTES;
    LdsHalfMem m{reinterpret_cast<u64 *>(lds_half) + colr};
    const uint64_t n_groups = r.G1 - r.G0;
    __syncthreads();
    if (n_groups >= 1) regs.load(r.ring_wg, r.G0, half, sl);
    if (half == 1u && n_groups >= 1) { __builtin_amdgcn_s_barrier(); __builtin_amdgcn_s_barrier(); }
    for (uint64_t it = 1; it <= n_groups; it++) {
        const uint64_t g = r.G0 + it - 1;
        const uint64_t pid = g * SEED_COLS + half * SEED_LANES + colr;
        const bool in_range = pid < r.paths;
        const uint32_t item = (uint32_t)((in_range ? pid : r.paths - 1) >> 6), j = (uint32_t)((in_range ? pid : r.paths - 1) & 63u);
        uint32_t tile = item / rp.num_k;
        uint32_t px, py, sub;
        tile_lane_frame_pixel(rp, tile, j, px, py, sub);
        const bool valid = in_range && px < rp.width && py < rp.height;
        if (P) tm = __builtin_readcyclecounter();
        __syncthreads();
        HR_STAMP(0);
        regs.run(lds_half, sl);
        HR_STAMP(1);
        __syncthreads();
        HR_STAMP(2);
        if (it < n_groups) regs.load(r.ring_wg, r.G0 + it, half, sl);
        RecStore rs(recs, pid);
        RecordTail<RecStore> lt(rs, lens_shape);
        if (lane < (uint32_t)SEED_LANES) {
            isaac_round_deep28(m, lt, PsRoundSync<P>{pc, &tm, 0});
            lt.finish();
        }
        ovf_note(lane < (uint32_t)SEED_LANES && valid && lt.overflow(), pid, ovf_list, ovf_count, rp.ovf_cap);
        HR_STAMP(7);
    }
    if (half == 0u && n_groups >= 1) { __builtin_amdgcn_s_barrier(); __builtin_amdgcn_s_barrier(); }
#undef HR_STAMP
    if (P && lane == 0 && half + 1u == (uint32_t)PROF)
        for (int i = 0; i < 8; i++) atomicAdd(&cnt->seed_phase[i], pc[i]);
    const bool lane_on = lane < (uint32_t)SEED_LANES;
    seed_fixup_wave(rp, lens_shape, m, colr, lane_on, ovf_list, ovf_count, win + (size_t)(blockIdx.x * 2u + half) * SEED_WIN_WORDS, recs, cnt);
}
template <int PROF>
__device__ __forceinline__ void seed_ps_producer(const RenderParams &rp, const PcRange &r, unsigned char *smem, uint32_t lane, uint32_t half, Counters *cnt) {
    constexpr bool P = PROF == 3;
    unsigned long long pc[8] = {0, 0, 0, 0, 0, 0, 0, 0}, tm = 0;
#define HR_STAMP(i) do { if (P) { unsigned long long now_ = __builtin_readcyclecounter(); pc[i] += now_ - tm; tm = now_; } } while (0)
    const IsaacWarm warm = isaac_warm();
    const PsLane sl = ps_lane(1u + half, lane);
    PsRegs regs;
    const uint64_t n_groups = r.G1 - r.G0;
    uint64_t frontier = r.first_path & ~63ull;
    AheadRegs job;
    PsStateOut job_out{nullptr};
    bool job_on = false, job_open = false;
    auto part1 = [&](uint64_t upto) -> bool {
        const uint64_t need = upto * SEED_COLS;
        for (; frontier < need && frontier < r.end_path; frontier += 64) {
            if (((frontier >> 6) & 1u) != half) continue;
            const uint64_t pid0 = frontier + lane;
            job_on = pid0 >= r.first_path && pid0 < r.end_path && !(rp.pad[2] & 4u);
            const uint64_t ppid = pid0 >= r.first_path && pid0 < r.end_path ? pid0 : r.end_path - 1;
            const uint32_t item = (uint32_t)(ppid >> 6), j = (uint32_t)(ppid & 63u);
            uint32_t tile = item / rp.num_k, k = item - tile * rp.num_k;
            uint32_t px, py, sub;
            tile_lane_frame_pixel(rp, tile, j, px, py, sub);
            bool pvalid = px < rp.width && py < rp.height;
            u64 s, t;
            path_seed_words(rp.width, rp.height, pvalid ? px : 0u, pvalid ? py : 0u, sub, s, t);
            const uint64_t g = ppid / SEED_COLS;
            const uint32_t c80 = (uint32_t)(ppid - g * SEED_COLS), hh = c80 >= (uint32_t)SEED_LANES ? 1u : 0u;
            job_out.base = r.ring_wg + (g & (SEED_RING_GROUPS - 1)) * PsLayout::GROUP_WORDS + hh * PsLayout::HALF_WORDS + (size_t)(c80 - hh * (uint32_t)SEED_LANES) * 2u;
            if (job_on) isaac_ahead_part1<PS_P1BLK>(job_out, warm, 8700304ULL, (u64)(rp.sampling_begin + k * rp.stride), s, t, job);
            frontier += 64;
            return true;
        }
        return false;
    };
    auto part2 = [&]() {
        if (job_on) isaac_ahead_part2<PS_NRUN, PS_NBLK, PS_P1BLK>(job_out, job);
        __builtin_amdgcn_s_waitcnt(0);
    };
    while (part1(r.G0 + 2)) part2();
    __syncthreads();
    if (P) tm = __builtin_readcyclecounter();
    for (uint64_t it = 1; it <= n_groups; it++) {
        const uint64_t g = r.G0 + it - 1;
        for (uint32_t hw = 0; hw < 2u; hw++) {
            regs.load(r.ring_wg, g, hw, sl);
            HR_STAMP(hw ? 3 : 7);
// ... 255 lines not shown
```

Baseline: 1430.

## Add wide seed producer/consumer form with governor-capped trace budget

Adds a second segmentation of the ISAAC seed pre-run (SegpCut<true>) that hands out 16/4-block runs with more pre-run columns. It instantiates wide seed kernels with a 112-VGPR ceiling, and the consumer now loads the ring after the ahead step. A host-side rule latches the wide form on when the governor's trace budget sits at or below 3x CUs, and the governor gains a budget cap that clamps budget growth while the wide form is active. The aim is to raise seed throughput when trace leaves registers free, at the cost of capping trace workgroups and adding a device-to-host governor readback on each sync.

```diff
diff --git a/hanamaru-renderer_amd/csrc/device_scene.h b/hanamaru-renderer_amd/csrc/device_scene.h
--- a/hanamaru-renderer_amd/csrc/device_scene.h
+++ b/hanamaru-renderer_amd/csrc/device_scene.h
@@ -173,6 +173,7 @@
     uint32_t budget_lo, budget_hi, budget_step;
     uint32_t budget_moves;
     float thr_down, thr_up;
+    uint32_t budget_cap, cap_hits;
 };
 HD uint32_t gov_trace_mask(int32_t level) { return level >= 4 ? 0x1fu : level == 3 ? 0xfu : 0u; }
 HD uint32_t gov_budget_next(uint32_t B, float ratio, uint32_t lo, uint32_t hi, uint32_t step, float down = 0.88f, float up = 0.97f) {
@@ -230,19 +231,41 @@
 static const int DRAWS_PER_PATH = 20;
 static const uint32_t REC_ITEM_FLOATS = 64u * REC_FLOATS;
 static const int SEG_B1 = 11, SEG_B2 = 21, SEG_NBLK = 11;
-static const int SEGP_NBLK = 8, SEGP_PNBLK = 12, SEGP_PRE = 4, SEGP_XCOLS = 32, SEGP_AHEAD_END = 24;
-HD bool segp_wants(uint32_t col, int block) {
-    return block == 0 || block == 24 || (col < (uint32_t)SEGP_XCOLS ? block == 12 : block == 8 || block == 16);
-}
-HD uint32_t segp_slot(uint32_t col, int block) {
-    if (col < (uint32_t)SEGP_XCOLS) return block == 0 ? col : block == 12 ? 32u + col : 64u + col;
-    return 96u + (uint32_t)(block >> 3) * 8u + (col - (uint32_t)SEGP_XCOLS);
-}
-HD void segp_run(uint32_t slot, uint32_t &col, uint32_t &first, uint32_t &nblk) {
-    if (slot < 64u) { col = slot & 31u; first = (slot >> 5) * (uint32_t)SEGP_PNBLK; nblk = (uint32_t)SEGP_PNBLK; }
-    else if (slot < 96u) { col = slot - 64u; first = 24u; nblk = (uint32_t)SEGP_NBLK; }
-    else { col = (uint32_t)SEGP_XCOLS + ((slot - 96u) & 7u); first = ((slot - 96u) >> 3) * (uint32_t)SEGP_NBLK; nblk = (uint32_t)SEGP_NBLK; }
-}
+template <bool WIDE> struct SegpCut;
+template <> struct SegpCut<false> {
+    static const int NBLK = 8, PNBLK = 12, PRE = 4, XCOLS = 32, AHEAD_END = 24;
+    static HD bool wants(uint32_t col, int block) {
+        return block == 0 || block == 24 || (col < (uint32_t)XCOLS ? block == 12 : block == 8 || block == 16);
+    }
+    static HD uint32_t slot(uint32_t col, int block) {
+        if (col < (uint32_t)XCOLS) return block == 0 ? col : block == 12 ? 32u + col : 64u + col;
+        return 96u + (uint32_t)(block >> 3) * 8u + (col - (uint32_t)XCOLS);
+    }
+    static HD void run(uint32_t slot, uint32_t &col, uint32_t &first, uint32_t &nblk) {
+        if (slot < 64u) { col = slot & 31u; first = (slot >> 5) * (uint32_t)PNBLK; nblk = (uint32_t)PNBLK; }
+        else if (slot < 96u) { col = slot - 64u; first = 24u; nblk = (uint32_t)NBLK; }
+        else { col = (uint32_t)XCOLS + ((slot - 96u) & 7u); first = ((slot - 96u) >> 3) * (uint32_t)NBLK; nblk = (uint32_t)NBLK; }
+    }
+};
+template <> struct SegpCut<true> {
+    static const int NBLK = 4, PNBLK = 16, PRE = 10, XCOLS = 24, AHEAD_END = 28, STEP = 4;
+    static HD bool wants(uint32_t col, int block) {
+        return block == 0 || block == 16 || (col >= (uint32_t)XCOLS && (block == 20 || block == 24 || block == 28));
+    }
+    static HD uint32_t slot(uint32_t col, int block) {
+        if (col < (uint32_t)XCOLS) return block == 0 ? col : (uint32_t)XCOLS + col;
+        return block == 0 ? 2u * (uint32_t)XCOLS + (col - (uint32_t)XCOLS) : 64u + (uint32_t)((block - 16) >> 2) * 16u + (col - (uint32_t)XCOLS);
+    }
+    static HD void run(uint32_t slot, uint32_t &col, uint32_t &first, uint32_t &nblk) {
+        if (slot < 2u * (uint32_t)XCOLS) { col = slot % (uint32_t)XCOLS; first = (slot / (uint32_t)XCOLS) * (uint32_t)PNBLK; nblk = (uint32_t)PNBLK; }
+        else if (slot < 64u) { col = slot - (uint32_t)XCOLS; first = 0u; nblk = (uint32_t)PNBLK; }
+        else { col = (uint32_t)XCOLS + ((slot - 64u) & 15u); first = 16u + ((slot - 64u) >> 4) * (uint32_t)NBLK; nblk = (uint32_t)NBLK; }
+    }
+};
+static const int SEGP_NBLK = SegpCut<false>::NBLK, SEGP_PNBLK = SegpCut<false>::PNBLK, SEGP_PRE = SegpCut<false>::PRE, SEGP_XCOLS = SegpCut<false>::XCOLS, SEGP_AHEAD_END = SegpCut<false>::AHEAD_END;
+HD bool segp_wants(uint32_t col, int block) { return SegpCut<false>::wants(col, block); }
+HD uint32_t segp_slot(uint32_t col, int block) { return SegpCut<false>::slot(col, block); }
+HD void segp_run(uint32_t slot, uint32_t &col, uint32_t &first, uint32_t &nblk) { SegpCut<false>::run(slot, col, first, nblk); }
 HD uint32_t rec_slot(uint32_t lane_base, uint32_t slot) { return lane_base + (slot >> 2) * 256u + (slot & 3u); }
 
 struct Counters {
diff --git a/hanamaru-renderer_amd/csrc/hr_api.hip b/hanamaru-renderer_amd/csrc/hr_api.hip
--- a/hanamaru-renderer_amd/csrc/hr_api.hip
+++ b/hanamaru-renderer_amd/csrc/hr_api.hip
@@ -160,6 +160,12 @@
     int seed_mode = 2;
     int seed_prof = 0;
     int seed_prerun = 1;
+    int seed_wide = 0;
+    bool wide_latched = false;
+    uint32_t wide_over = 0;
+    uint32_t wide_seen_decisions = 0, wide_seen_hits = 0;
+    bool gov_wide = false;
+    bool last_seed_wide = false;
     uint32_t seed_prio = 3;
     uint32_t nee_cull = 7;
     uint32_t rr_start = 0;
@@ -230,7 +236,8 @@
             g->decisions++;
             bool budget_moved = false;
             if (L == 0 && g->level == 0 && B == g->budget && g->budget_step) {
-                const uint32_t nb = gov_budget_next(B, trace_t / seed_t, g->budget_lo, g->budget_hi, g->budget_step, g->thr_down, g->thr_up);
+                uint32_t nb = gov_budget_next(B, trace_t / seed_t, g->budget_lo, g->budget_hi, g->budget_step, g->thr_down, g->thr_up);
+                if (g->budget_cap && (nb == 0u || nb > g->budget_cap)) { nb = g->budget_cap; g->cap_hits++; }
                 if (nb != B) {
                     budget_moved = true;
                     g->budget_moves++;
@@ -263,8 +270,13 @@
     c->precise = c->precise_opt == 1 || (c->precise_opt < 0 && has_scene && tris == 0u && !c->rr_start);
     c->trace_mode = c->trace_mode_opt >= 0 ? c->trace_mode_opt : (c->precise && tris > 0u ? 1 : 0);
 }
+static bool seed_wide_supported(const hr_ctx *c) { return c->seed_mode == 2 && c->seed_prerun != 0 && !c->counters && !c->rr_start; }
+static bool seed_wide_in_force(const hr_ctx *c) { return seed_wide_supported(c) && (c->seed_wide == 1 || (c->seed_wide < 0 && c->wide_latched)); }
 static int govern_reset(hr_ctx *c) {
     resolve_modes(c);
+    c->gov_wide = seed_wide_in_force(c);
+    c->wide_seen_decisions = c->wide_seen_hits = 0;
+    c->wide_over = 0;
     if (!c->gov) return HR_OK;
     GovDev h;
     memset(&h, 0, sizeof h);
@@ -277,6 +289,9 @@
     if (c->trace_mode == 1 && !c->rr_start && c->trace_boost < 0) {
         h.budget_step = (uint32_t)c->num_cus / 2u; h.budget_lo = (uint32_t)c->num_cus * 3u; h.budget_hi = (uint32_t)c->num_cus * 7u;
         h.thr_down = 0.96f; h.thr_up = 1.02f;
+    } else if (c->gov_wide && c->trace_boost < 0) {
+        h.budget_cap = h.budget = (uint32_t)c->num_cus * 3u;
+        h.budget_hi = std::min(h.budget_hi, h.budget_cap);
     }
     HIP_TRY(hipMemcpy(c->gov, &h, sizeof h, hipMemcpyHostToDevice));
     return HR_OK;
@@ -323,6 +338,25 @@
     c->seed_events.erase(c->seed_events.begin(), c->seed_events.begin() + (long)n);
     c->trace_events.erase(c->trace_events.begin(), c->trace_events.begin() + (long)n);
 }
+static int seed_wide_rule(hr_ctx *c) {
+    if (c->seed_wide >= 0 || !c->gov || c->trace_boost >= 0) return HR_OK;
+    GovDev h;
+    HIP_TRY(hipMemcpy(&h, c->gov, sizeof h, hipMemcpyDeviceToHost));
+    if (h.decisions == c->wide_seen_decisions) return HR_OK;
+    c->wide_seen_decisions = h.decisions;
+    const bool fits = !c->precise && c->trace_mode == 0 && c->min_waves == 5;
+    bool want;
+    if (!fits) want = false;
+    else if (!c->wide_latched) want = h.budget != 0u && h.budget <= (uint32_t)c->num_cus * 3u;
+    else {
+        c->wide_over = h.cap_hits != c->wide_seen_hits ? c->wide_over + 1u : 0u;
+        c->wide_seen_hits = h.cap_hits;
+        want = c->wide_over < 2u;
+    }
+    if (want == c->wide_latched) return HR_OK;
+    c->wide_latched = want;
+    return seed_wide_in_force(c) != c->gov_wide ? govern_reset(c) : HR_OK;
+}
 static int sync_all(hr_ctx *c) {
     HIP_TRY(hipStreamSynchronize(c->seed_stream));
     HIP_TRY(hipStreamSynchronize(c->stream));
@@ -330,7 +364,8 @@
     c->seed_pending[0] = c->seed_pending[1] = false;
     for (auto &m : c->markers) (void)hipEventDestroy(m.second);
     c->markers.clear();
-    return drain_events(c);
+    int rc = drain_events(c);
+    return rc ? rc : seed_wide_rule(c);
 }
 static void drop_pair(EventPair &ev) {
     if (ev.a) (void)hipEventDestroy(ev.a);
@@ -1012,12 +1047,18 @@
     return HR_OK;
 }
 
+static const char *seed_wide_refusal(const hr_ctx *c) {
+    if (c->seed_wide != 1) return nullptr;
+    return c->counters ? "option counters" : c->rr_start ? "option russian_roulette" : c->seed_mode != 2 ? "a seed_mode other than 2" : !c->seed_prerun ? "seed_prerun 0" : nullptr;
+}
 static int launch_seed(hr_ctx *c, const RenderParams &rp, int slot, hipStream_t st) {
     const bool list = rp.tile_list != nullptr;
     uint64_t paths = (uint64_t)(list ? rp.tile_count : rp.tiles_x * rp.tiles_y) * rp.num_k * 64u;
     uint32_t grid = (uint32_t)std::min<uint64_t>((paths + SEED_COLS - 1) / SEED_COLS, (uint64_t)c->num_cus);
-    const SeedVariant *v = select_seed_kernel(c->seed_mode, c->seed_split, c->seed_prof, rp.rec_lo_off != 0, list, c->seed_prerun != 0);
+    if (const char *why = seed_wide_refusal(c)) return fail(HR_ERR_UNSUPPORTED, "debug option seed_wide 1: the wide seed rows have no form for %s", why);
+    const SeedVariant *v = select_seed_kernel(c->seed_mode, c->seed_split, c->seed_prof, rp.rec_lo_off != 0, list, c->seed_prerun != 0, seed_wide_in_force(c));
     if (!v) return fail(HR_ERR_UNSUPPORTED, "no seed kernel instantiation for seed_mode %d, seed_split %d, seed_prof %d%s (kernel_variants.h)", c->seed_mode, c->seed_split, c->seed_prof, list ? " under a tile mask" : "");
+    c->last_seed_wide = v->wide;
     const bool skip = (c->debug_skip & 2) != 0;
     if (!skip && v->ring && !c->ring) HIP_TRY(hipMalloc((void **)&c->ring, (size_t)c->num_cus * SEED_RING_WORDS_MAX * sizeof(u64)));
     EventPair ev;
@@ -1109,6 +1150,12 @@
             if (c->buckets) c->buckets_n += total_k;
             return HR_OK;
         }
+    }
+    if (const char *why = seed_wide_refusal(c)) return fail(HR_ERR_UNSUPPORTED, "hr_render: debug option seed_wide 1: the wide seed rows have no form for %s", why);
+    if (seed_wide_in_force(c) != c->gov_wide) {
+        int grc = sync_all(c);
+        if (!grc && seed_wide_in_force(c) != c->gov_wide) grc = govern_reset(c);
+        if (grc) return grc;
     }
     LaunchPlan plan;
     int rc = plan_launch(c, s_begin, stride, 0, TRACE_IN_FORCE, plan);
@@ -2432,6 +2479,17 @@
         return HR_OK;
     }
     if (k == "nee_cull") { c->nee_cull = (uint32_t)value & 7u; return HR_OK; }
+    if (!strcmp(key, "seed_wide")) {
+        if (value != -1 && value != 0 && value != 1) return fail(HR_ERR_INVALID, "seed_wide must be -1 (the wide row of the pre-run form while the governor leaves its registers free), 0 (never) or 1 (always)");
+        int rc = sync_all(c);
+        if (rc) return rc;
+        c->seed_wide = (int)value;
+        return govern_reset(c);
+    }
+    if (!strcmp(key, "seed_wide_ran")) {
+        if (value != 0 && value != 1) return fail(HR_ERR_INVALID, "seed_wide_ran asks about form 1 (wide) or 0 (narrow)");
+        return c->last_seed_wide == (value == 1) ? HR_OK : fail(HR_ERR_UNSUPPORTED, "the last seed kernel launched took the %s form", c->last_seed_wide ? "wide" : "narrow");
+    }
     return fail(HR_ERR_INVALID, "unknown debug option '%s'", key);
 }
 
diff --git a/hanamaru-renderer_amd/csrc/isaac_core.h b/hanamaru-renderer_amd/csrc/isaac_core.h
--- a/hanamaru-renderer_amd/csrc/isaac_core.h
+++ b/hanamaru-renderer_amd/csrc/isaac_core.h
@@ -11,6 +11,16 @@
 #else
 #define HR_NOUNROLL
 #define HR_UNROLL
+#endif
+
+#if defined(__HIP_DEVICE_COMPILE__)
+#define HR_OPAQUE64(v) asm volatile("" : "+v"(v))
+#define HR_OPAQUE32(p) asm volatile("" : "+v"(p))
+#define HR_SCHED_FENCE() __builtin_amdgcn_sched_barrier(0)
+#else
+#define HR_OPAQUE64(v)
+#define HR_OPAQUE32(p)
+#define HR_SCHED_FENCE()
 #endif
 
 #define HR_ISAAC_MIX(a, b, c, d, e, f, g, h) \
@@ -132,7 +142,7 @@
     }
 }
 
-template <class Out>
+template <bool WIDE = false, class Out>
 HD void isaac_init_ahead_pre(Out &out, const IsaacWarm &w, u64 s0, u64 s1, u64 s2, u64 s3) {
     u64 A = w.r[0] + s0, B = w.r[1] + s1, C = w.r[2] + s2, D = w.r[3] + s3, E = w.r[4], F = w.r[5], G = w.r[6], H = w.r[7];
     HR_NOUNROLL
@@ -147,10 +157,18 @@
         HR_ISAAC_MIX_2(A, B, C, D, E, F, G, H)                                 \
     }                                                                          \
     if (out.wants(to)) out.state(to, a, b, c, d, e, f, g, h, A, B, C, D, E, F, G, H);
-    HR_AHEAD_TO(0, 8)
-    HR_AHEAD_TO(8, 12)
-    HR_AHEAD_TO(12, 16)
-    HR_AHEAD_TO(16, 24)
+    if constexpr (WIDE) {
+        static_assert(SegpCut<true>::AHEAD_END == 28 && SegpCut<true>::STEP == 4, "the hand-outs below");
+        HR_AHEAD_TO(0, 16)
+        HR_AHEAD_TO(16, 20)
+        HR_AHEAD_TO(20, 24)
+        HR_AHEAD_TO(24, 28)
+    } else {
+        HR_AHEAD_TO(0, 8)
+        HR_AHEAD_TO(8, 12)
+        HR_AHEAD_TO(12, 16)
+        HR_AHEAD_TO(16, 24)
+    }
 #undef HR_AHEAD_TO
 }
 template <int P>
@@ -163,6 +181,7 @@
         A += a; B += b; C += c; D += d; E += e; F += f; G += g; H += h;
         HR_ISAAC_MIX_2(A, B, C, D, E, F, G, H)
         kept[p][0] = A; kept[p][1] = B; kept[p][2] = C; kept[p][3] = D; kept[p][4] = E; kept[p][5] = F; kept[p][6] = G; kept[p][7] = H;
+        if (P > 4) { HR_SCHED_FENCE(); }
     }
     st16[0] = a; st16[1] = b; st16[2] = c; st16[3] = d; st16[4] = e; st16[5] = f; st16[6] = g; st16[7] = h;
     st16[8] = A; st16[9] = B; st16[10] = C; st16[11] = D; st16[12] = E; st16[13] = F; st16[14] = G; st16[15] = H;
@@ -221,15 +240,6 @@
     isaac_round<TAILN>(mem, tail);
 }
 
-#if defined(__HIP_DEVICE_COMPILE__)
-#define HR_OPAQUE64(v) asm volatile("" : "+v"(v))
-#define HR_OPAQUE32(p) asm volatile("" : "+v"(p))
-#define HR_SCHED_FENCE() __builtin_amdgcn_sched_barrier(0)
-#else
-#define HR_OPAQUE64(v)
-#define HR_OPAQUE32(p)
-#define HR_SCHED_FENCE()
-#endif
 
 template <int TAILN, int NG, class Mem, class Tail>
 HD void isaac_round_n(Mem *mem, Tail *tail) {
diff --git a/hanamaru-renderer_amd/csrc/kernel_variants.h b/hanamaru-renderer_amd/csrc/kernel_variants.h
--- a/hanamaru-renderer_amd/csrc/kernel_variants.h
+++ b/hanamaru-renderer_amd/csrc/kernel_variants.h
@@ -97,7 +97,7 @@
     return fn_of(find_row(TRACE_DEBUG_VARIANTS, [&](const TraceDebugVariant &r) { return r.cnt == counters && r.qn == qn; }));
 }
 
-struct SeedVariant { int mode, split, prof; bool lo; const void *fn; uint32_t threads; bool ring; bool list = false; bool pre = false; };
+struct SeedVariant { int mode, split, prof; bool lo; const void *fn; uint32_t threads; bool ring; bool list = false; bool pre = false; bool wide = false; };
 static const SeedVariant SEED_VARIANTS[] = {
     {0, 0, 0, false, (const void *)seed_isaac64_kernel, 64 * SEED_WAVES, false},
     {1, 8, 0, false, (const void *)seed_pc_kernel<8>, 256, true},
@@ -122,6 +122,13 @@
     {2, 0, 0, false, (const void *)seed_seg_kernel<false, false, true, true>, 256, true, true, true},
     {2, 0, 0, true, (const void *)seed_seg_kernel<false, true, true, true>, 256, true, true, true},
     {2, 0, 2, false, (const void *)seed_seg_kernel<2, false, false, true>, 256, true, false, true},
+    {2, 0, 0, false, (const void *)seed_seg_kernel<false, false, false, true, true>, 256, true, false, true, true},
+    {2, 0, 1, false, (const void *)seed_seg_kernel<true, false, false, true, true>, 256, true, false, true, true},
+    {2, 0, 0, true, (const void *)seed_seg_kernel<false, true, false, true, true>, 256, true, false, true, true},
+    {2, 0, 1, true, (const void *)seed_seg_kernel<true, true, false, true, true>, 256, true, false, true, true},
+    {2, 0, 0, false, (const void *)seed_seg_kernel<false, false, true, true, true>, 256, true, true, true, true},
+    {2, 0, 0, true, (const void *)seed_seg_kernel<false, true, true, true, true>, 256, true, true, true, true},
+    {2, 0, 2, false, (const void *)seed_seg_kernel<2, false, false, true, true>, 256, true, false, true, true},
 #if defined(HR_EXPERIMENTS)
     {3, 0, 0, false, (const void *)seed_ps_kernel<0>, 256, true},
     {3, 0, 1, false, (const void *)seed_ps_kernel<1>, 256, true},
@@ -131,14 +138,15 @@
     {4, 0, 1, false, (const void *)seed_w5_kernel<true>, 320, true},
 #endif
 };
-static const SeedVariant *select_seed_kernel(int seed_mode, int seed_split, int seed_prof, bool twin, bool list = false, bool prerun = false) {
+static const SeedVariant *select_seed_kernel(int seed_mode, int seed_split, int seed_prof, bool twin, bool list = false, bool prerun = false, bool wide = false) {
     int split = 0, prof = seed_prof ? 1 : 0;
     bool lo = false, pre = false;
     if (seed_mode == 2) { lo = twin; pre = prerun; if (seed_prof == 2) prof = 2; }
     else if (seed_mode == 1) split = prof ? (seed_split == 20 ? 20 : 16) : seed_split;
     else if (seed_mode == 3) prof = seed_prof >= 1 && seed_prof <= 3 ? seed_prof : 0;
     else if (seed_mode == 0) prof = 0;
-    return find_row(SEED_VARIANTS, [&](const SeedVariant &r) { return r.mode == seed_mode && r.split == split && r.prof == prof && r.lo == lo && r.list == list && r.pre == pre; });
+    wide = wide && pre;
+    return find_row(SEED_VARIANTS, [&](const SeedVariant &r) { return r.mode == seed_mode && r.split == split && r.prof == prof && r.lo == lo && r.list == list && r.pre == pre && r.wide == wide; });
 }
 
 typedef void (*AccumulateFn)(RenderParams, const float *, float *, double *, uint32_t *);
diff --git a/hanamaru-renderer_amd/csrc/seed_kernels.h b/hanamaru-renderer_amd/csrc/seed_kernels.h
--- a/hanamaru-renderer_amd/csrc/seed_kernels.h
+++ b/hanamaru-renderer_amd/csrc/seed_kernels.h
@@ -402,13 +402,18 @@
 static_assert(SEED_RING_GROUPS * SegpLayout::GROUP_WORDS <= SEED_RING_WORDS_MAX, "the ring allocation of the producer / consumer kernel holds it");
 static_assert(2 * SEGP_XCOLS == 64 && SEGP_XCOLS + 4 * (SEED_LANES - SEGP_XCOLS) == 64, "64 producer runs and 64 consumer runs per half");
 static_assert(SEGP_PNBLK == SEGP_PRE + SEGP_NBLK && 2 * SEGP_PNBLK + SEGP_NBLK == 32 && 4 * SEGP_NBLK == 32 && SEGP_AHEAD_END == 32 - SEGP_NBLK, "the runs tile the sweep");
+typedef SegpCut<true> SegwCut;
+static_assert(2 * SegwCut::XCOLS + (SEED_LANES - SegwCut::XCOLS) == 64 && 4 * (SEED_LANES - SegwCut::XCOLS) == 64, "64 producer runs and 64 consumer runs per half");
+static_assert(2 * SegwCut::PNBLK == 32 && SegwCut::PNBLK + 4 * SegwCut::NBLK == 32 && SegwCut::AHEAD_END == 32 - SegwCut::NBLK && SegwCut::PRE < SegwCut::PNBLK, "the runs tile the sweep");
+static_assert(SegwCut::PNBLK % SegwCut::STEP == 0 && SegwCut::NBLK == SegwCut::STEP, "entry blocks are multiples of the step");
+template <bool WIDE>
 struct SegpStateOut {
     u64 *half;
     uint32_t col;
-    __device__ __forceinline__ bool wants(int block) const { return segp_wants(col, block); }
+    __device__ __forceinline__ bool wants(int block) const { return SegpCut<WIDE>::wants(col, block); }
     __device__ __forceinline__ void state(int block, u64 a, u64 b, u64 c, u64 d, u64 e, u64 f, u64 g, u64 h, u64 A, u64 B, u64 C, u64 D, u64 E, u64 F, u64 G, u64 H) {
         typedef u64 u64x2 __attribute__((ext_vector_type(2)));
-        const uint32_t s = segp_slot(col, block);
+        const uint32_t s = SegpCut<WIDE>::slot(col, block);
         u64x2 *dst = reinterpret_cast<u64x2 *>(half + (size_t)(s >> 6) * SegpLayout::WAVE_WORDS + (size_t)(s & 63u) * 2u);
         const u64x2 q[8] = {{a, b}, {c, d}, {e, f}, {g, h}, {A, B}, {C, D}, {E, F}, {G, H}};
 #pragma unroll
@@ -418,14 +423,17 @@
 struct SegpLane {
     uint32_t slot, col, first;
 };
+template <bool WIDE>
 __device__ __forceinline__ SegpLane segp_lane(bool consumer, uint32_t lane) {
     SegpLane l;
     uint32_t nblk;
     l.slot = (consumer ? 64u : 0u) + lane;
-    segp_run(l.slot, l.col, l.first, nblk);
+    SegpCut<WIDE>::run(l.slot, l.col, l.first, nblk);
     return l;
 }
+template <bool WIDE>
 struct SegpRegs {
+    typedef SegpCut<WIDE> Cut;
     typedef u64 u64x2_t __attribute__((ext_vector_type(2)));
     u64x2_t v[8];
     __device__ __forceinline__ void load(const u64 *ring_wg, uint64_t g, uint32_t half, const SegpLane &l) {
@@ -438,44 +446,46 @@
 #pragma unroll
         for (int q = 0; q < 8; q++) { st16[2 * q] = v[q].x; st16[2 * q + 1] = v[q].y; }
         LdsHalfMem m{reinterpret_cast<u64 *>(lds_half) + l.col + (size_t)l.first * 8u * SEED_LANES};
-        isaac_init_run<SEGP_NBLK>(m, st16);
+        isaac_init_run<Cut::NBLK>(m, st16);
     }
     __device__ __forceinline__ void prerun(u64 (*kept)[8]) {
         u64 st16[16];
 #pragma unroll
         for (int q = 0; q < 8; q++) { st16[2 * q] = v[q].x; st16[2 * q + 1] = v[q].y; }
-        isaac_init_prerun<SEGP_PRE>(st16, kept);
+        isaac_init_prerun<Cut::PRE>(st16, kept);
 #pragma unroll
         for (int q = 0; q < 8; q++) { v[q].x = st16[2 * q]; v[q].y = st16[2 * q + 1]; }
     }
     __device__ __forceinline__ void finish(unsigned char *lds_half, const SegpLane &l, const u64 (*kept)[8]) const {
         LdsHalfMem k{reinterpret_cast<u64 *>(lds_half) + l.col + (size_t)l.first * 8u * SEED_LANES};
 #pragma unroll
-        for (int p = 0; p < SEGP_PRE; p++)
+        for (int p = 0; p < Cut::PRE; p++)
 #pragma unroll
             for (int j = 0; j < 8; j++) k.st(p * 8 + j, kept[p][j]);
+        if (WIDE) HR_SCHED_FENCE();
         u64 st16[16];
 #pragma unroll
         for (int q = 0; q < 8; q++) { st16[2 * q] = v[q].x; st16[2 * q + 1] = v[q].y; }
-        LdsHalfMem m{k.col + (size_t)SEGP_PRE * 8u * SEED_LANES};
-        isaac_init_run<SEGP_NBLK>(m, st16);
-    }
-};
-template <bool PRE> struct SegForm { typedef SegLane Lane; typedef SegRegs Regs; static __device__ __forceinline__ Lane lane(bool consumer, uint32_t l) { return seg_lane(consumer, l); } };
-template <> struct SegForm<true> { typedef SegpLane Lane; typedef SegpRegs Regs; static __device__ __forceinline__ Lane lane(bool consumer, uint32_t l) { return segp_lane(consumer, l); } };
-template <bool PROF, bool LO, bool LIST, bool PRE>
+        LdsHalfMem m{k.col + (size_t)Cut::PRE * 8u * SEED_LANES};
+        isaac_init_run<Cut::PNBLK - Cut::PRE>(m, st16);
+    }
+};
+template <bool PRE, bool WIDE> struct SegForm { typedef SegLane Lane; typedef SegRegs Regs; static __device__ __forceinline__ Lane lane(bool consumer, uint32_t l) { return seg_lane(consumer, l); } };
+template <bool WIDE> struct SegForm<true, WIDE> { typedef SegpLane Lane; typedef SegpRegs<WIDE> Regs; static __device__ __forceinline__ Lane lane(bool consumer, uint32_t l) { return segp_lane<WIDE>(consumer, l); } };
+template <bool PROF, bool LO, bool LIST, bool PRE, bool WIDE>
 __device__ __forceinline__ void seed_seg_consumer(const RenderParams &rp, int lens_shape, const PcRange &r, unsigned char *smem, uint32_t lane, uint32_t half,
                                                   float *__restrict__ recs, uint32_t *__restrict__ ovf, u64 *__restrict__ win, Counters *cnt) {
     uint32_t *ovf_list = ovf + (size_t)(blockIdx.x * 2u + half) * rp.ovf_cap;
     uint32_t ovf_count = 0;
     unsigned long long pc[8] = {0, 0, 0, 0, 0, 0, 0, 0}, tm = 0;
 #define HR_STAMP(i) do { if (PROF) { unsigned long long now_ = __builtin_readcyclecounter(); pc[i] += now_ - tm; tm = now_; } } while (0)
-    const typename SegForm<PRE>::Lane sl = SegForm<PRE>::lane(true, lane);
-    typename SegForm<PRE>::Regs regs;
+    const typename SegForm<PRE, WIDE>::Lane sl = SegForm<PRE, WIDE>::lane(true, lane);
+    typename SegForm<PRE, WIDE>::Regs regs;
     const uint32_t colr = lane < (uint32_t)SEED_LANES ? lane : 0u;
     unsigned char *lds_half = smem + (size_t)half * SEED_LDS_HALF_BYTES;
     LdsHalfMem m{reinterpret_cast<u64 *>(lds_half) + colr};
     const uint64_t n_groups = r.G1 - r.G0;
+    if (WIDE) { __syncthreads(); __syncthreads(); }
     if (PRE) __syncthreads();
     __syncthreads();
     for (uint64_t it = 1; it <= n_groups; it++) {
@@ -516,12 +526,63 @@
     seed_fixup_wave<LdsHalfMem, LO, LIST>(rp, lens_shape, m, colr, lane_on, ovf_list, ovf_count, win + (size_t)(blockIdx.x * 2u + half) * SEED_WIN_WORDS, recs, cnt);
 }
 static const uint32_t SEG_PROF_FIT = 563u * SEGP_PRE;
-template <bool LIST, bool PRE, bool PROF>
+static const uint32_t SEG_PROF_LATE = 64u;
+template <bool LIST>
+__device__ __forceinline__ void segw_ahead(const RenderParams &rp, const PcRange &r, const IsaacWarm &warm, uint32_t lane, uint32_t half, uint64_t g1, bool do1, uint64_t g2, bool do2) {
+    typedef u64 u64x2_t __attribute__((ext_vector_type(2)));
+    if ((!do1 && !do2) || (rp.pad[2] & 4u)) return;
+    const bool s1 = lane < (uint32_t)SEED_LANES, s2 = !s1 && lane < (uint32_t)(SEED_LANES + SEED_LANES - SegwCut::XCOLS);
+    const uint32_t col1 = s1 ? lane : 0u, col2 = (uint32_t)SegwCut::XCOLS + (s2 ? lane - (uint32_t)SEED_LANES : 0u);
+    SegpStateOut<true> out1{r.ring_wg + (g1 & (SEED_RING_GROUPS - 1)) * SegpLayout::GROUP_WORDS + half * SegpLayout::HALF_WORDS, col1};
+    SegpStateOut<true> out2{r.ring_wg + (g2 & (SEED_RING_GROUPS - 1)) * SegpLayout::GROUP_WORDS + half * SegpLayout::HALF_WORDS, col2};
+    AheadRegs q;
+    q.a = q.b = q.c = q.d = q.e = q.f = q.g = q.h = q.A = q.B = q.C = q.D = q.E = q.F = q.G = q.H = 0;
+    if (do1) {
+        const uint64_t pid = g1 * SEED_COLS + half * (uint32_t)SEED_LANES + col1;
+        const uint64_t ppid = pid < r.end_path ? pid : r.end_path - 1;
+        const uint32_t item = (uint32_t)(ppid >> 6), j = (uint32_t)(ppid & 63u);
+        uint32_t tile = item / rp.num_k, k = item - tile * rp.num_k;
+        uint32_t px, py, sub;
+        tile_lane_frame_pixel(rp, launch_tile<LIST>(rp, tile), j, px, py, sub);
+        bool pvalid = px < rp.width && py < rp.height;
+        u64 s, t;
+        path_seed_words(rp.width, rp.height, pvalid ? px : 0u, pvalid ? py : 0u, sub, s, t);
+        const u64 s0 = 8700304ULL, sk = (u64)(rp.sampling_begin + k * rp.stride);
+        q.A = warm.r[0] + s0; q.B = warm.r[1] + sk; q.C = warm.r[2] + s; q.D = warm.r[3] + t; q.E = warm.r[4]; q.F = warm.r[5]; q.G = warm.r[6]; q.H = warm.r[7];
+        HR_NOUNROLL
+        for (int i = 0; i < 32; i++) { HR_ISAAC_MIX_2(q.A, q.B, q.C, q.D, q.E, q.F, q.G, q.H) }
+        q.a = warm.r[0] + s0; q.b = warm.r[1] + sk; q.c = warm.r[2] + s; q.d = warm.r[3] + t; q.e = warm.r[4]; q.f = warm.r[5]; q.g = warm.r[6]; q.h = warm.r[7];
+        if (s1) out1.state(0, q.a, q.b, q.c, q.d, q.e, q.f, q.g, q.h, q.A, q.B, q.C, q.D, q.E, q.F, q.G, q.H);
+    }
+    if (do2) {
+        const uint32_t sl = SegwCut::slot(col2, 16);
+        const u64 *regs = out2.half + (size_t)(sl >> 6) * SegpLayout::WAVE_WORDS + (size_t)(sl & 63u) * 2u;
+        u64x2_t v[8];
+#pragma unroll
+        for (int p = 0; p < 8; p++) v[p] = __builtin_nontemporal_load(reinterpret_cast<const u64x2_t *>(regs + p * 128));
+        if (s2) {
+            q.a = v[0].x; q.b = v[0].y; q.c = v[1].x; q.d = v[1].y; q.e = v[2].x; q.f = v[2].y; q.g = v[3].x; q.h = v[3].y;
+            q.A = v[4].x; q.B = v[4].y; q.C = v[5].x; q.D = v[5].y; q.E = v[6].x; q.F = v[6].y; q.G = v[7].x; q.H = v[7].y;
+        }
+    }
+    static_assert(SegwCut::PNBLK == 4 * SegwCut::STEP && SegwCut::AHEAD_END - SegwCut::PNBLK == 3 * SegwCut::STEP, "stage 1 sweeps four steps, stage 2 three of them");
+    HR_NOUNROLL
+    for (int st = 0; st < (do1 ? 4 : 3); st++) {
+        HR_NOUNROLL
+        for (int i = 0; i < SegwCut::STEP; i++) { HR_AHEAD_BLOCK(q) }
+        if (do2 && s2 && st < 3) out2.state(SegwCut::PNBLK + (st + 1) * SegwCut::STEP, q.a, q.b, q.c, q.d, q.e, q.f, q.g, q.h, q.A, q.B, q.C, q.D, q.E, q.F, q.G, q.H);
+    }
+    if (do1 && s1) out1.state(SegwCut::PNBLK, q.a, q.b, q.c, q.d, q.e, q.f, q.g, q.h, q.A, q.B, q.C, q.D, q.E, q.F, q.G, q.H);
+    __builtin_amdgcn_s_waitcnt(0);
+}
+__device__ __forceinline__ uint32_t relane(uint32_t lane) { HR_OPAQUE32(lane); return lane; }
+template <bool LIST, bool PRE, bool PROF, bool WIDE>
 __device__ __forceinline__ void seed_seg_producer(const RenderParams &rp, const PcRange &r, unsigned char *smem, uint32_t lane, uint32_t half, const uint32_t pprio, Counters *cnt) {
     const IsaacWarm warm = isaac_warm();
-    const typename SegForm<PRE>::Lane sl = SegForm<PRE>::lane(false, lane);
-    typename SegForm<PRE>::Regs regs;
-    u64 kept[PRE ? SEGP_PRE : 1][8];
+    static_assert(PRE || !WIDE, "the wide row is a pre-run form");
+    const typename SegForm<PRE, WIDE>::Lane sl = SegForm<PRE, WIDE>::lane(false, lane);
+    typename SegForm<PRE, WIDE>::Regs regs;
+    u64 kept[PRE ? SegpCut<WIDE>::PRE : 1][8];
     uint32_t pc[8] = {0, 0, 0, 0, 0, 0, 0, 0}, tm = 0, chunks = 0;
 #define HR_NOW() __builtin_amdgcn_readfirstlane((uint32_t)__builtin_readcyclecounter())
 #define HR_STAMP(i) do { if (PROF) { const uint32_t now_ = HR_NOW(); pc[i] = __builtin_amdgcn_readfirstlane(pc[i] + (now_ - tm)); tm = now_; } } while (0)
@@ -545,7 +606,7 @@
             const uint64_t g = ppid / SEED_COLS;
             const uint32_t c80 = (uint32_t)(ppid - g * SEED_COLS), hh = c80 >= (uint32_t)SEED_LANES ? 1u : 0u;
             if constexpr (PRE) {
-                SegpStateOut out{r.ring_wg + (g & (SEED_RING_GROUPS - 1)) * SegpLayout::GROUP_WORDS + hh * SegpLayout::HALF_WORDS, c80 - hh * (uint32_t)SEED_LANES};
+                SegpStateOut<false> out{r.ring_wg + (g & (SEED_RING_GROUPS - 1)) * SegpLayout::GROUP_WORDS + hh * SegpLayout::HALF_WORDS, c80 - hh * (uint32_t)SEED_LANES};
                 if (on) isaac_init_ahead_pre(out, warm, 8700304ULL, (u64)(rp.sampling_begin + k * rp.stride), s, t);
             } else {
                 SegStateOut out{r.ring_wg + (g & (SEED_RING_GROUPS - 1)) * SegLayout::GROUP_WORDS + hh * SegLayout::HALF_WORDS + (size_t)(c80 - hh * (uint32_t)SEED_LANES) * 2u};
@@ -555,7 +616,13 @@
         }
         __builtin_amdgcn_s_waitcnt(0);
     };
-    ahead(r.G0 + 2);
+    if constexpr (WIDE) {
+        segw_ahead<LIST>(rp, r, warm, lane, half, r.G0, true, 0, false);
+        __syncthreads();
+        segw_ahead<LIST>(rp, r, warm, lane, half, r.G0 + 1, r.G0 + 1 < r.G1, r.G0, true);
+        __syncthreads();
+        segw_ahead<LIST>(rp, r, warm, lane, half, r.G0 + 2, r.G0 + 2 < r.G1, r.G0 + 1, r.G0 + 1 < r.G1);
+    } else ahead(r.G0 + 2);
     if constexpr (PRE) {
         __syncthreads();
         regs.load(r.ring_wg, r.G0, half, sl);
@@ -567,28 +634,32 @@
     }
     for (uint64_t it = 1; it <= n_groups; it++) {
         if (PROF) { tm = HR_NOW(); chunks = 0; }
-        if constexpr (PRE) regs.finish(lds_half, sl, kept);
+        if constexpr (WIDE) regs.finish(lds_half, SegForm<PRE, WIDE>::lane(false, relane(lane)), kept);
+        else if constexpr (PRE) regs.finish(lds_half, sl, kept);
         else regs.run(lds_half, sl);
         HR_STAMP(0);
         __syncthreads();
         HR_STAMP(1);
-        if (it < n_groups) regs.load(r.ring_wg, r.G0 + it, half, sl);
+        if (!WIDE && it < n_groups) regs.load(r.ring_wg, r.G0 + it, half, sl);
         if (((pprio >> 2) & 3u) != (pprio & 3u)) {
             const uint32_t pr = (it & 1u) ? (pprio >> 2) & 3u : pprio & 3u;
             if (pr == 0u) __builtin_amdgcn_s_setprio(0); else if (pr == 1u) __builtin_amdgcn_s_setprio(1); else if (pr == 2u) __builtin_amdgcn_s_setprio(2); else __builtin_amdgcn_s_setprio(3);
         }
-        ahead(r.G0 + it + 2);
+        if constexpr (WIDE) {
+            segw_ahead<LIST>(rp, r, warm, relane(lane), half, r.G0 + it + 2, r.G0 + it + 2 < r.G1, r.G0 + it + 1, r.G0 + it + 1 < r.G1);
+            if (it < n_groups) regs.load(r.ring_wg, r.G0 + it, half, SegForm<PRE, WIDE>::lane(false, relane(lane)));
+        } else ahead(r.G0 + it + 2);
         if constexpr (PRE) regs.prerun(kept);
         HR_STAMP(2);
         __syncthreads();
         if (PROF) {
             const uint32_t now_ = HR_NOW(), wait = now_ - tm;
             tm = now_;
-            const bool busy = chunks != 0;
+            const bool busy = WIDE || chunks != 0;
             pc[3] = __builtin_amdgcn_readfirstlane(pc[3] + (busy ? wait : 0u));
             pc[4] = __builtin_amdgcn_readfirstlane(pc[4] + (busy ? 0u : wait));
             pc[5] = __builtin_amdgcn_readfirstlane(pc[5] + (busy ? 1u : 0u));
-            pc[6] = __builtin_amdgcn_readfirstlane(pc[6] + (busy && wait < SEG_PROF_FIT ? 1u : 0u));
+            pc[6] = __builtin_amdgcn_readfirstlane(pc[6] + (busy && wait < (WIDE ? SEG_PROF_LATE : SEG_PROF_FIT) ? 1u : 0u));
             pc[7] = __builtin_amdgcn_readfirstlane(pc[7] + 1u);
         }
     }
@@ -597,32 +668,52 @@
     if (PROF && lane == 0)
         for (int i = 0; i < 8; i++) atomicAdd(&cnt->seed_phase[i], (unsigned long long)pc[i]);
 }
-template <int PROF = 0, bool LO = false, bool LIST = false, bool PRE = false>
+#define HR_SEED_SEG_BODY(PROF, LO, LIST, PRE, WIDE) \
+    extern __shared__ __align__(16) unsigned char smem[];                                                                        \
+    const uint32_t lane = threadIdx.x & 63u, wave = threadIdx.x >> 6, half = wave & 1u;                                          \
+    const bool consumer = wave < 2u;                                                                                             \
+    const uint32_t pprio = consumer ? 0u : seed_gov_begin(rp, wave == 2u && lane == 0u);                                         \
+    const uint32_t prio = consumer ? rp.pad[0] : pprio & 3u;                                                                     \
+    switch (prio) {                                                                                                              \
+        case 0: break;                                                                                                           \
+        case 1: __builtin_amdgcn_s_setprio(1); break;                                                                            \
+        case 2: __builtin_amdgcn_s_setprio(2); break;                                                                            \
+        default: __builtin_amdgcn_s_setprio(3); break;                                                                           \
+    }                                                                                                                            \
+    PcRange r;                                                                                                                   \
+    r.paths = (uint64_t)launch_tiles<LIST>(rp) * rp.num_k * 64u;                                                                 \
+    const uint64_t groups = (r.paths + SEED_COLS - 1) / SEED_COLS;                                                               \
+    r.G0 = groups * blockIdx.x / gridDim.x; r.G1 = groups * (blockIdx.x + 1) / gridDim.x;                                        \
+    r.first_path = r.G0 * SEED_COLS; r.end_path = r.G1 * SEED_COLS < r.paths ? r.G1 * SEED_COLS : r.paths;                       \
+    r.ring_wg = ring + (size_t)blockIdx.x * SEED_RING_WORDS_MAX;                                                                 \
+    if (consumer) seed_seg_consumer<PROF == 1, LO, LIST, PRE, WIDE>(rp, lens_shape, r, smem, lane, half, recs, ovf, win, cnt);   \
+    else {                                                                                                                       \
+        seed_seg_producer<LIST, PRE, PROF == 2, WIDE>(rp, r, smem, lane, half, pprio, cnt);                                      \
+        seed_gov_end(rp, wave == 2u && lane == 0u);                                                                              \
+    }                                                                                                                           
+template <int PROF = 0, bool LO = false, bool LIST = false, bool PRE = false, bool WIDE = false>
 __global__ __launch_bounds__(256) void seed_seg_kernel(RenderParams rp, int lens_shape, u64 *__restrict__ ring, float *__restrict__ recs,
                                                        uint32_t *__restrict__ ovf, u64 *__restrict__ win, Counters *cnt) {
-    extern __shared__ __align__(16) unsigned char smem[];
-    const uint32_t lane = threadIdx.x & 63u, wave = threadIdx.x >> 6, half = wave & 1u;
-    const bool consumer = wave < 2u;
-    const uint32_t pprio = consumer ? 0u : seed_gov_begin(rp, wave == 2u && lane == 0u);
-    const uint32_t prio = consumer ? rp.pad[0] : pprio & 3u;
-    switch (prio) {
-        case 0: break;
-        case 1: __builtin_amdgcn_s_setprio(1); break;
-        case 2: __builtin_amdgcn_s_setprio(2); break;
-        default: __builtin_amdgcn_s_setprio(3); break;
-    }
-    PcRange r;
-    r.paths = (uint64_t)launch_tiles<LIST>(rp) * rp.num_k * 64u;
-    const uint64_t groups = (r.paths + SEED_COLS - 1) / SEED_COLS;
-    r.G0 = groups * blockIdx.x / gridDim.x; r.G1 = groups * (blockIdx.x + 1) / gridDim.x;
-    r.first_path = r.G0 * SEED_COLS; r.end_path = r.G1 * SEED_COLS < r.paths ? r.G1 * SEED_COLS : r.paths;
-    r.ring_wg = ring + (size_t)blockIdx.x * SEED_RING_WORDS_MAX;
-    if (consumer) seed_seg_consumer<PROF == 1, LO, LIST, PRE>(rp, lens_shape, r, smem, lane, half, recs, ovf, win, cnt);
-    else {
-        seed_seg_producer<LIST, PRE, PROF == 2>(rp, r, smem, lane, half, pprio, cnt);
-        seed_gov_end(rp, wave == 2u && lane == 0u);
-    }
-}
+    static_assert(!WIDE, "the wide rows are the specialisations below: each carries the register ceiling");
+    HR_SEED_SEG_BODY(PROF, LO, LIST, PRE, false)
+}
+static const int SEED_WIDE_VGPRS = 224;
+#define HR_SEED_WIDE_ROW(PROF, LO, LIST)                                                                                                                            \
+    template <>                                                                                                                                                     \
+    __global__ __launch_bounds__(256) __attribute__((amdgpu_num_vgpr(112))) void seed_seg_kernel<PROF, LO, LIST, true, true>(                                       \
+        RenderParams rp, int lens_shape, u64 *__restrict__ ring, float *__restrict__ recs, uint32_t *__restrict__ ovf, u64 *__restrict__ win, Counters *cnt) {      \
+        HR_SEED_SEG_BODY(PROF, LO, LIST, true, true)                                                                                                                \
+    }
+HR_SEED_WIDE_ROW(0, false, false)
+HR_SEED_WIDE_ROW(1, false, false)
+HR_SEED_WIDE_ROW(0, true, false)
+HR_SEED_WIDE_ROW(1, true, false)
+HR_SEED_WIDE_ROW(0, false, true)
+HR_SEED_WIDE_ROW(0, true, true)
+HR_SEED_WIDE_ROW(2, false, false)
+#undef HR_SEED_WIDE_ROW
+#undef HR_SEED_SEG_BODY
+static_assert(SEED_WIDE_VGPRS == 2 * 112, "the rows' attribute above");
 
 #if defined(HR_EXPERIMENTS)
 static const int PS_NRUN = 4, PS_NBLK = 8, PS_P1BLK = 4;
```

New measurement: 1429. No clear change (-0.0%).
